# matthewhoung/inference-arena

Measured on AMD Instinct MI355X. Metric: req/sec (whole node) + P50/P99 e2e latency, YOLOv5n→MobileNetV2 at 1/2/4/8 GPU, higher is better.
Workload: dtype fp32

## Files before the change

csrc/bindings.cpp:

```cpp
#include <pybind11/numpy.h>
#include <pybind11/pybind11.h>
#include <pybind11/stl.h>

#include <cstring>
#include <malloc.h>
#include <map>
#include <mutex>

#include "kernels/launch.h"
#include "runtime/executor.h"
#include "runtime/echo_instance.h"
#include "runtime/http_front.h"
#include "runtime/http_loadgen.h"
#include "runtime/ipc_buffer.h"
#include "runtime/peer.h"
#include "runtime/jpeg_decode.h"
#include "runtime/jpeg_ingest.h"
#include "runtime/batcher.h"
#include "runtime/split.h"
#include "runtime/crash_trace.h"

namespace py = pybind11;
using namespace arena;

namespace arena {
void bind_jpeg(py::module& m);
}

namespace {

template <typename T>
T get(const py::dict& d, const char* k, T dflt) {
  if (!d.contains(k)) return dflt;
  py::object o = d[k];
  if (o.is_none()) return dflt;
  return o.cast<T>();
}
template <typename T>
T req(const py::dict& d, const char* k) {
  if (!d.contains(k)) throw std::runtime_error(std::string("missing kernel parameter '") + k + "'");
  return d[k].cast<T>();
}
template <typename P>
P ptr(const py::dict& d, const char* k) {
  return reinterpret_cast<P>(get<uintptr_t>(d, k, 0));
}
hipStream_t stream_of(const py::dict& d) { return reinterpret_cast<hipStream_t>(get<uintptr_t>(d, "stream", 0)); }

void py_conv2d(const py::dict& d) {
  ConvParams p{};
  p.x = ptr<const void*>(d, "x");
  p.B = req<int>(d, "B");
  p.H = req<int>(d, "H");
  p.W = req<int>(d, "W");
  p.xs = req<int>(d, "xs");
  p.Cin = req<int>(d, "Cin");
  p.w = ptr<const void*>(d, "w");
  p.Kpad = req<int>(d, "Kpad");
  p.bias = ptr<const float*>(d, "bias");
  p.y = ptr<void*>(d, "y");
  p.Ho = req<int>(d, "Ho");
  p.Wo = req<int>(d, "Wo");
  p.ys = req<int>(d, "ys");
  p.Cout = req<int>(d, "Cout");
  p.Cout_pad = req<int>(d, "Cout_pad");
  p.KH = req<int>(d, "KH");
  p.KW = req<int>(d, "KW");
  p.stride = get<int>(d, "stride", 1);
  p.pad_t = get<int>(d, "pad_t", 0);
  p.pad_l = get<int>(d, "pad_l", 0);
  p.res = ptr<const void*>(d, "res");
  p.rs = get<int>(d, "rs", 0);
  p.y2 = ptr<void*>(d, "y2");
  p.y2s = get<int>(d, "y2s", 0);
  p.act = get<int>(d, "act", 0);
  p.f32out = get<int>(d, "f32out", 0);
  p.bdev = ptr<const int*>(d, "bdev");
  p.impl = get<int>(d, "impl", 0);
  p.pw_w = ptr<const void*>(d, "pw_w");
  p.pw_bias = ptr<const float*>(d, "pw_bias");
  p.pw_y = ptr<void*>(d, "pw_y");
  p.pw_ys = get<int>(d, "pw_ys", 0);
  p.pw_cout = get<int>(d, "pw_cout", 0);
  p.pw_kpad = get<int>(d, "pw_kpad", 0);
  p.pw_act = get<int>(d, "pw_act", 0);
  p.gate = ptr<const float*>(d, "gate");
  p.gate_n = get<int>(d, "gate_n", 0);
  p.gate_min = get<float>(d, "gate_min", 0.f);
  p.w3 = ptr<const void*>(d, "w3");
  p.sk_ws = ptr<float*>(d, "sk_ws");
  p.sk_ws_bytes = get<int64_t>(d, "sk_ws_bytes", 0);
  prepare_kernels();
  if (get<int>(d, "f32", 0))
    conv2d_f32(p, stream_of(d));
  else
    conv2d(p, stream_of(d));
}

void py_dwconv(const py::dict& d) {
  DwParams p{};
  p.x = ptr<const void*>(d, "x");
  p.B = req<int>(d, "B");
  p.H = req<int>(d, "H");
  p.W = req<int>(d, "W");
  p.xs = req<int>(d, "xs");
  p.C = req<int>(d, "C");
  p.w = ptr<const void*>(d, "w");
  p.bias = ptr<const float*>(d, "bias");
  p.y = ptr<void*>(d, "y");
  p.Ho = req<int>(d, "Ho");
  p.Wo = req<int>(d, "Wo");
  p.ys = req<int>(d, "ys");
  p.stride = get<int>(d, "stride", 1);
  p.act = get<int>(d, "act", 0);
  p.bdev = ptr<const int*>(d, "bdev");
  if (get<int>(d, "f32", 0))
    dwconv3x3_f32(p, stream_of(d));
  else
    dwconv3x3(p, stream_of(d));
}

void py_ir_block(const py::dict& d) {
  IrParams p{};
  p.x = ptr<const void*>(d, "x");
  p.x_cs = req<int>(d, "x_cs");
  p.H = req<int>(d, "H");
  p.W = req<int>(d, "W");
  p.inp = req<int>(d, "inp");
  p.inp_pad = req<int>(d, "inp_pad");
  p.hid_pad = req<int>(d, "hid_pad");
  p.oup = req<int>(d, "oup");
  p.oup_pad = req<int>(d, "oup_pad");
  p.stride = req<int>(d, "stride");
  p.expand = req<int>(d, "expand");
  p.res = get<int>(d, "res", 0);
  p.we = ptr<const void*>(d, "we");
  p.be = ptr<const float*>(d, "be");
  p.wd = ptr<const void*>(d, "wd");
  p.bd = ptr<const float*>(d, "bd");
  p.wp = ptr<const void*>(d, "wp");
  p.bp = ptr<const float*>(d, "bp");
  p.y = ptr<void*>(d, "y");
  p.y_cs = req<int>(d, "y_cs");
  p.Ho = req<int>(d, "Ho");
  p.Wo = req<int>(d, "Wo");
  p.B = req<int>(d, "B");
  p.bdev = ptr<const int*>(d, "bdev");
  p.x3w = get<int>(d, "x3w", 0);
  p.x_parts = get<int>(d, "x_parts", 0);
  p.y_parts = get<int>(d, "y_parts", 0);
  prepare_kernels();
  if (get<int>(d, "f32", 0))
    ir_block_f32(p, stream_of(d));
  else
    ir_block(p, stream_of(d));
}

void py_c3_block(const py::dict& d) {
  C3Params p{};
  p.x = ptr<const void*>(d, "x");
  p.xs = req<int>(d, "xs");
  p.B = req<int>(d, "B");
  p.H = req<int>(d, "H");
  p.W = req<int>(d, "W");
  p.bdev = ptr<const int*>(d, "bdev");
  p.C1 = req<int>(d, "C1");
  p.CH = req<int>(d, "CH");
  p.NB = req<int>(d, "NB");
  p.res = req<int>(d, "res");
  p.w12 = ptr<const void*>(d, "w12");
  p.b12 = ptr<const float*>(d, "b12");
  p.wb1[0] = p.wb1[1] = ptr<const void*>(d, "wb1");
  p.bb1[0] = p.bb1[1] = ptr<const float*>(d, "bb1");
  p.wb2[0] = p.wb2[1] = ptr<const void*>(d, "wb2");
  p.bb2[0] = p.bb2[1] = ptr<const float*>(d, "bb2");
  p.w3 = ptr<const void*>(d, "w3");
  p.b3 = ptr<const float*>(d, "b3");
  p.y = ptr<void*>(d, "y");
  p.ys = req<int>(d, "ys");
  prepare_kernels();
  if (get<int>(d, "f32", 0))
    c3_x3(p, stream_of(d));
  else
    c3_fused(p, stream_of(d));
}

void py_sppf(const py::dict& d) {
  SppfParams p{};
  p.buf = ptr<void*>(d, "buf");
  p.B = req<int>(d, "B");
  p.H = req<int>(d, "H");
  p.W = req<int>(d, "W");
  p.xs = req<int>(d, "xs");
  p.C = req<int>(d, "C");
  p.bdev = ptr<const int*>(d, "bdev");
  if (get<int>(d, "f32", 0))
    sppf_pool_f32(p, stream_of(d));
  else
    sppf_pool(p, stream_of(d));
}

void py_letterbox(const py::dict& d) {
  LetterboxParams p{};
  p.pool = ptr<const uint8_t*>(d, "pool");
  p.meta = ptr<const ImageMeta*>(d, "meta");
  p.ctrl = ptr<const Ctrl*>(d, "ctrl");
  p.out = ptr<void*>(d, "out");
  p.B = req<int>(d, "B");
  p.T = req<int>(d, "T");
  p.f32 = get<int>(d, "f32", 0);
  letterbox_s2d(p, stream_of(d));
}

void py_decode(const py::dict& d) {
  DecodeParams p{};
  auto heads = req<std::vector<uintptr_t>>(d, "head");
  auto hw = req<std::vector<int>>(d, "hw");
  auto xs = req<std::vector<int>>(d, "xs");
  auto st = req<std::vector<float>>(d, "strides");
  for (int l = 0; l < 3; ++l) {
    p.head[l] = (const void*)heads.at(l);
    p.hw[l] = hw.at(l);
    p.xs[l] = xs.at(l);
    p.stride[l] = st.at(l);
  }
  p.B = req<int>(d, "B");
  p.conf_thr = req<float>(d, "conf_thr");
  p.cand = ptr<Candidate*>(d, "cand");
  p.cand_count = ptr<int*>(d, "cand_count");
  p.cand_cap = req<int>(d, "cand_cap");
  p.ctrl = ptr<const Ctrl*>(d, "ctrl");
  p.f32 = get<int>(d, "f32", 0);
  detect_decode(p, stream_of(d));
}

void py_yolo_raw(const py::dict& d) {
  YoloRawParams p{};
  auto heads = req<std::vector<uintptr_t>>(d, "head");
  auto hw = req<std::vector<int>>(d, "hw");
  auto xs = req<std::vector<int>>(d, "xs");
  auto st = req<std::vector<float>>(d, "strides");
  for (int l = 0; l < 3; ++l) {
    p.head[l] = (const void*)heads.at(l);
    p.hw[l] = hw.at(l);
    p.xs[l] = xs.at(l);
    p.stride[l] = st.at(l);
  }
  p.B = req<int>(d, "B");
  p.out = ptr<void*>(d, "out");
// ... 216 lines not shown
      p = std::malloc(bytes);
      if (p == nullptr) throw std::bad_alloc();
    }
    it->coef = (int16_t*)p;
    st = compact ? jpeg_decode_compact((const uint8_t*)data.data(), data.size(), it->info, (uint8_t*)it->coef, err)
                 : jpeg_decode_coefs((const uint8_t*)data.data(), data.size(), it->info, it->coef, err);
    if (st != JpegStatus::Ok) throw py::value_error("JpegSet: entropy decode failed: " + err);
    set->items.push_back(it);
  }
  return set;
}

std::vector<InputImage> images_from(const py::list& imgs, std::vector<py::array>& keep, JpegKeep* jkeep = nullptr) {
  std::vector<InputImage> v;
  v.reserve(imgs.size());
  for (auto h : imgs) {
    if (py::isinstance<py::bytes>(h)) {
      if (jkeep == nullptr) throw std::runtime_error("JPEG inputs are not accepted here");
      const std::string data = h.cast<std::string>();
      auto jh = std::make_shared<JpegHolder>();
      std::string err;
      JpegStatus st = jpeg_parse((const uint8_t*)data.data(), data.size(), jh->info, err);
      if (st == JpegStatus::Ok) {
        jh->coef.assign((size_t)jh->info.coef_count, 0);
        st = jpeg_decode_coefs((const uint8_t*)data.data(), data.size(), jh->info, jh->coef.data(), err);
      }
      if (st != JpegStatus::Ok) throw py::value_error("JPEG input not decodable by the split decoder: " + err);
      InputImage im{(const uint8_t*)jh->coef.data(), jh->info.out_height, jh->info.out_width};
      im.jpeg = &jh->info;
      jkeep->push_back(jh);
      v.push_back(im);
      continue;
    }
    py::array a = py::array::ensure(h, py::array::c_style);
    if (!a) throw std::runtime_error("inputs must be numpy arrays");
    InputImage im;
    if (a.ndim() == 3 && a.shape(2) == 3 && a.itemsize() == 1) {
      im.h = (int)a.shape(0);
      im.w = (int)a.shape(1);
    } else if (a.ndim() == 3 && a.shape(0) == 3 && a.itemsize() == 4 && a.shape(1) == a.shape(2)) {
      im.h = im.w = (int)a.shape(1);
      im.bytes = (int64_t)a.nbytes();
    } else {
      throw std::runtime_error("inputs must be uint8 HxWx3 images or float32 [3,S,S] tensors");
    }
    keep.push_back(a);
    im.data = (const uint8_t*)a.data();
    v.push_back(im);
  }
  return v;
}

py::dict result_to_py(const BatchResult& r, int max_det) {
  py::dict out;
  const int n = r.n_images;
  py::array_t<int32_t> cnt(n);
  std::memcpy(cnt.mutable_data(), r.det_count.data(), sizeof(int) * n);
  py::array_t<float> det({n, max_det, 8});
  static_assert(sizeof(Detection) == 32, "Detection layout");
  if (n) std::memcpy(det.mutable_data(), r.det.data(), sizeof(Detection) * (size_t)n * max_det);
  py::array_t<int32_t> offs(n + 1);
  std::memcpy(offs.mutable_data(), r.crop_offset.data(), sizeof(int) * (n + 1));
  static_assert(sizeof(TopkResult) == 64, "TopkResult layout");
  py::array_t<int32_t> tk_idx({(int)r.topk.size(), 5});
  py::array_t<float> tk_logit({(int)r.topk.size(), 5});
  py::array_t<float> tk_prob({(int)r.topk.size(), 5});
  for (size_t i = 0; i < r.topk.size(); ++i)
    for (int k = 0; k < 5; ++k) {
      tk_idx.mutable_at(i, k) = r.topk[i].idx[k];
      tk_logit.mutable_at(i, k) = r.topk[i].logit[k];
      tk_prob.mutable_at(i, k) = r.topk[i].prob[k];
    }
  out["det_count"] = cnt;
  out["det"] = det;
  out["crop_offset"] = offs;
  out["topk_idx"] = tk_idx;
  out["topk_logit"] = tk_logit;
  out["topk_prob"] = tk_prob;
  out["gpu_ms"] = r.gpu_ms;
  out["detection_ms"] = r.det_ms;
  out["classification_ms"] = r.cls_ms;
  out["bucket"] = r.bucket;
  out["total_crops"] = r.total_crops;
  if (!r.raw.empty()) {
    py::array_t<uint8_t> raw((py::ssize_t)r.raw.size());
    std::memcpy(raw.mutable_data(), r.raw.data(), r.raw.size());
    out["raw"] = raw;
  }
  return out;
}

}

PYBIND11_MODULE(_C, m) {
  m.doc() = "MI355X-native kernels and runtime of inference_arena_amd (gfx950)";
  {
    const char* e = std::getenv("ARENA_CRASH_TRACE");
    if (e == nullptr || std::strcmp(e, "0") != 0) arena::install_crash_trace();
  }
  m.def("install_crash_trace", &arena::install_crash_trace);
  m.def("crash_trace_installed", &arena::crash_trace_installed);
  m.def("dump_thread_stack", &arena::dump_thread_stack, py::arg("tid"));
  m.def("malloc_trim", []() {
    py::gil_scoped_release nogil;
    return malloc_trim(0) != 0;
  });
  m.def("malloc_info", []() {
    const struct mallinfo2 mi = mallinfo2();
    py::dict d;
    d["arena"] = (uint64_t)mi.arena;
    d["mmapped"] = (uint64_t)mi.hblkhd;
    d["in_use"] = (uint64_t)mi.uordblks;
    d["free"] = (uint64_t)mi.fordblks;
    d["releasable"] = (uint64_t)mi.keepcost;
    return d;
  });
  bind_jpeg(m);
  m.def("conv2d", &py_conv2d);
  m.def("set_conv_impl", &set_conv_impl);
  m.def("get_conv_impl", &get_conv_impl);
  m.def("dwconv3x3", &py_dwconv);
  m.def("sppf_pool", &py_sppf);
  m.def("ir_block", &py_ir_block);
  m.def("c3_block", &py_c3_block);
  m.def("set_conv_pw", &set_conv_pw);
  m.def("set_conv_v3", &set_conv_v3);
  m.def("set_ir_wave", &set_ir_wave);
  m.def("set_irx_parts", &set_irx_parts);
  m.def("set_irx_slices_big", &set_irx_slices_big);
  m.def("set_ir_t14", &set_ir_t14);
  m.def("set_ir_crop", &set_ir_crop);
  m.def("set_ir_s2k16", &set_ir_s2k16);
  m.def("set_ir_crop_split", &set_ir_crop_split);
  m.def("set_head_gate", &set_head_gate);
  m.def("get_head_gate", &get_head_gate);
  m.def(
      "head_gate_min",
      [](float conf_thr) -> py::object {
        float g;
        if (!head_gate_min(conf_thr, &g)) return py::none();
        return py::float_(g);
      },
      py::arg("conf_thr"), "the gate's logit threshold for a confidence threshold (float32); None: the gate is off");
  m.def(
      "head_gate_pairs",
      [](py::array_t<int64_t, py::array::c_style> ops) {
        if (ops.ndim() != 2 || ops.shape(1) != kOpFields) throw std::runtime_error("ops must be int64 [n, OP_FIELDS]");
        py::list out;
        for (const HeadGatePair& gp : head_gate_pairs(ops.data(), (int)ops.shape(0), kOpFields))
          out.append(py::make_tuple(gp.box, gp.cls, gp.level));
        return out;
      },
      py::arg("ops"), "[(box conv op, class conv op, level)] of a program's records");
  m.attr("HEAD_BOX_CHANNELS") = kHeadBoxChannels;
  m.attr("HEAD_CLS_CHANNELS") = kHeadClsChannels;
  m.def("letterbox_s2d", &py_letterbox);
  m.def("detect_decode", &py_decode);
  m.def("yolo_raw", &py_yolo_raw);
  m.def("tensor_in_s2d", &py_tensor_in);
  m.def("nms", &py_nms);
  m.def("crop_plan", &py_crop_plan);
  m.def("crop_gather_s2d", &py_crop_gather);
  m.def("global_avgpool", &py_avgpool);
  m.def("head_pool", &py_head_pool);
  m.def("topk_softmax", &py_topk);
  m.attr("SIZEOF_IMAGE_META") = (int)sizeof(ImageMeta);
  m.attr("SIZEOF_CTRL") = (int)sizeof(Ctrl);
  m.attr("SIZEOF_CANDIDATE") = (int)sizeof(Candidate);
  m.attr("SIZEOF_DETECTION") = (int)sizeof(Detection);
  m.attr("SIZEOF_CROPREF") = (int)sizeof(CropRef);
  m.attr("SIZEOF_TOPK") = (int)sizeof(TopkResult);
  m.attr("OP_FIELDS") = kOpFields;

  py::class_<Executor, std::shared_ptr<Executor>>(m, "Executor")
      .def(py::init([](const py::dict& cfg) { return std::make_shared<Executor>(config_from(cfg)); }))
      .def("set_weights",
           [](Executor& e, py::array_t<uint8_t, py::array::c_style> blob) { e.set_weights(blob.data(), blob.size()); })
      .def("set_weights_device",
           [](Executor& e, uintptr_t ptr, size_t bytes) {
             py::gil_scoped_release nogil;
             e.set_weights_device((const void*)ptr, bytes);
           })
      .def("weights_host",
           [](Executor& e) {
             std::vector<uint8_t> v;
             {
               py::gil_scoped_release nogil;
               v = e.weights_host();
             }
             return py::bytes((const char*)v.data(), v.size());
           })
      .def("set_program",
           [](Executor& e, py::array_t<int64_t, py::array::c_style> ops, py::array_t<int64_t, py::array::c_style> cls) {
             if (ops.ndim() != 2 || ops.shape(1) != kOpFields || cls.ndim() != 2 || cls.shape(1) != kOpFields)
               throw std::runtime_error("programs must be int64 [n, OP_FIELDS]");
             e.set_program(ops.data(), (int)ops.shape(0), cls.data(), (int)cls.shape(0));
           })
      .def("add_bucket",
           [](Executor& e, int B, py::array_t<int64_t, py::array::c_style> offs, int64_t arena_bytes,
              py::object impl) {
             if (impl.is_none()) {
               e.add_bucket(B, offs.data(), (int)offs.size(), arena_bytes);
             } else {
               const std::vector<int> v = impl.cast<std::vector<int>>();
               e.add_bucket(B, offs.data(), (int)offs.size(), arena_bytes, &v);
             }
           },
           py::arg("B"), py::arg("offsets"), py::arg("arena_bytes"), py::arg("impl") = py::none())
      .def("buckets", &Executor::buckets)
      .def("crop_cap_for", &Executor::crop_cap_for)
      .def("submit",
           [](Executor& e, const py::list& imgs) {
             std::vector<py::array> keep;
             JpegKeep jkeep;
             auto v = images_from(imgs, keep, &jkeep);
             int slot;
             {
               py::gil_scoped_release nogil;
               slot = e.submit(v);
             }
             if (!jkeep.empty()) {
               std::lock_guard<std::mutex> lk(g_jkeep_mu);
               g_jkeep[{(const void*)&e, slot}] = std::move(jkeep);
             }
             return slot;
           })
      .def("submit_jpeg_set",
           [](Executor& e, std::shared_ptr<JpegSet> set, const std::vector<int>& idx) {
             std::vector<InputImage> v;
             v.reserve(idx.size());
             for (int i : idx) {
               if (i < 0 || i >= (int)set->items.size()) throw py::index_error("submit_jpeg_set: index out of range");
               const auto& it = set->items[i];
               InputImage im{(const uint8_t*)it->coef, it->info.out_height, it->info.out_width};
               im.jpeg = &it->info;
               v.push_back(im);
             }
             int slot;
             {
               py::gil_scoped_release nogil;
               slot = e.submit(v);
             }
             std::lock_guard<std::mutex> lk(g_jkeep_mu);
             g_jset_keep[{(const void*)&e, slot}] = set;
             return slot;
           })
      .def("collect",
           [](Executor& e, int slot) {
             BatchResult r;
             {
               py::gil_scoped_release nogil;
               r = e.collect(slot);
             }
             {
               std::lock_guard<std::mutex> lk(g_jkeep_mu);
               g_jkeep.erase({(const void*)&e, slot});
               g_jset_keep.erase({(const void*)&e, slot});
             }
             return result_to_py(r, e.config().max_det);
           })
      .def("run",
           [](Executor& e, const py::list& imgs) {
             std::vector<py::array> keep;
             JpegKeep jkeep;
             auto v = images_from(imgs, keep, &jkeep);
             BatchResult r;
             {
               py::gil_scoped_release nogil;
               r = e.run(v);
             }
             return result_to_py(r, e.config().max_det);
           })
      .def("replay",
           [](Executor& e, int B, int slot, int iters) {
             py::gil_scoped_release nogil;
             e.replay(B, slot, iters);
           })
      .def("num_slots", &Executor::num_slots)
      .def("synchronize",
           [](Executor& e) {
             py::gil_scoped_release nogil;
             e.synchronize();
           })
      .def("arena_ptr", &Executor::arena_ptr)
      .def("read_arena",
           [](Executor& e, int B, int64_t offset, size_t bytes) {
             py::array_t<uint8_t> out(bytes);
             {
               py::gil_scoped_release nogil;
               e.read_arena(B, offset, out.mutable_data(), bytes);
             }
             return out;
           })
      .def("weights_ptr", &Executor::weights_ptr)
      .def("set_peer_stage", &Executor::set_peer_stage)
      .def("device", &Executor::device)
      .def("submit_peer",
           [](Executor& e, Executor& src, int slot) {
             py::gil_scoped_release nogil;
             return e.submit_peer(src, slot);
           })
      .def("submit_device",
           [](Executor& e, const std::vector<std::tuple<uintptr_t, int, int, int>>& images,
              const std::vector<py::array_t<float, py::array::c_style | py::array::forcecast>>& boxes) {
             if (images.size() != boxes.size()) throw std::runtime_error("submit_device: one box array per image");
             std::vector<Executor::DeviceImage> imgs;
             std::vector<std::vector<Detection>> dets(images.size());
             for (size_t i = 0; i < images.size(); ++i) {
               Executor::DeviceImage d;
               d.ptr = std::get<0>(images[i]);
               d.h = std::get<1>(images[i]);
               d.w = std::get<2>(images[i]);
               d.device = std::get<3>(images[i]);
               imgs.push_back(d);
               const auto& b = boxes[i];
               if (b.size() == 0) continue;
               if (b.ndim() != 2 || b.shape(1) != 6) throw std::runtime_error("submit_device: boxes must be [k, 6]");
               const float* q = b.data();
               for (ssize_t k = 0; k < b.shape(0); ++k, q += 6) {
                 Detection dd{};
                 dd.x1 = q[0];
                 dd.y1 = q[1];
                 dd.x2 = q[2];
                 dd.y2 = q[3];
                 dd.conf = q[4];
                 dd.cls = (int)q[5];
                 dets[i].push_back(dd);
               }
             }
             py::gil_scoped_release nogil;
             return e.submit_device(imgs, dets);
           })
      .def("conv_choices", &Executor::conv_choices)
      .def("exec_order", &Executor::exec_order, py::arg("B"),
           "program op indices in the order bucket B's graphs launch them")
      .def("gated_ops", &Executor::gated_ops, py::arg("B"), "ops of bucket B that run with a tile gate")
      .def("stream", &Executor::stream);

  py::class_<SplitInstance, std::shared_ptr<SplitInstance>>(m, "SplitInstance")
      .def(py::init([](std::shared_ptr<Executor> det, std::shared_ptr<Executor> cls) {
        return std::make_shared<SplitInstance>(det, cls);
      }))
      .def("submit",
           [](SplitInstance& s, const py::list& imgs) {
             std::vector<py::array> keep;
             auto v = images_from(imgs, keep);
             py::gil_scoped_release nogil;
             return s.submit(v);
           })
      .def("collect",
           [](SplitInstance& s, int slot) {
             BatchResult r;
             {
               py::gil_scoped_release nogil;
               r = s.collect(slot);
             }
             return result_to_py(r, s.max_det());
           })
      .def("num_slots", &SplitInstance::num_slots)
      .def("buckets", &SplitInstance::buckets);

  py::class_<JpegSet, std::shared_ptr<JpegSet>>(m, "JpegSet")
      .def(py::init(&make_jpeg_set), py::arg("uploads"), py::arg("pinned") = true,
           "JPEG uploads entropy-decoded once into (pinned) host buffers, for Executor.submit_jpeg_set")
      .def("__len__", [](const JpegSet& s) { return s.items.size(); })
      .def("coef_bytes", [](const JpegSet& s, int i) { return (int64_t)jpeg_payload_bytes(s.items.at(i)->info); })
      .def_property_readonly("pinned", [](const JpegSet& s) {
        for (const auto& it : s.items)
          if (!it->pinned) return false;
        return true;
      });

  py::class_<EchoInstance, std::shared_ptr<EchoInstance>>(m, "EchoInstance")
      .def(py::init<int, int, int, int, int64_t>(), py::arg("slots") = 2, py::arg("max_batch") = 32,
           py::arg("max_det") = 4, py::arg("latency_us") = 0, py::arg("staging_cap") = 0);

  py::class_<DynamicBatcher>(m, "DynamicBatcher")
      .def(py::init([](py::list executors, const py::dict& cfg) {
             std::vector<std::shared_ptr<BatchInstance>> inst;
             for (auto h : executors) {
               if (py::isinstance<SplitInstance>(h))
                 inst.push_back(h.cast<std::shared_ptr<SplitInstance>>());
               else if (py::isinstance<EchoInstance>(h))
                 inst.push_back(h.cast<std::shared_ptr<EchoInstance>>());
               else
                 inst.push_back(h.cast<std::shared_ptr<Executor>>());
             }
             BatcherConfig c;
             c.max_batch = get<int>(cfg, "max_batch", c.max_batch);
             c.preferred = get<std::vector<int>>(cfg, "preferred", {});
             c.max_queue_delay_us = get<int64_t>(cfg, "max_queue_delay_us", c.max_queue_delay_us);
             c.idle_queue_delay_us = get<int64_t>(cfg, "idle_queue_delay_us", c.idle_queue_delay_us);
             c.max_queue_size = get<int64_t>(cfg, "max_queue_size", c.max_queue_size);
             c.overlap = get<int>(cfg, "overlap", c.overlap);
             return new DynamicBatcher(inst, c);
           }),
           py::keep_alive<1, 2>())
      .def("enqueue",
           [](DynamicBatcher& b, py::array img_in, py::function cb, uintptr_t export_to) {
             py::array img = py::array::ensure(img_in, py::array::c_style);
             int h = 0, w = 0;
             int64_t bytes = 0;
             if (img && img.ndim() == 3 && img.shape(2) == 3 && img.itemsize() == 1) {
               h = (int)img.shape(0);
               w = (int)img.shape(1);
             } else if (img && img.ndim() == 3 && img.shape(0) == 3 && img.itemsize() == 4 &&
                        img.shape(1) == img.shape(2)) {
               h = w = (int)img.shape(1);
               bytes = (int64_t)img.nbytes();
             } else {
               throw std::runtime_error("input must be a uint8 HxWx3 image or a float32 [3,S,S] tensor");
             }
             ResultCallback f = py_result_cb(std::move(cb));
             const uint8_t* data = (const uint8_t*)img.data();
             py::gil_scoped_release nogil;
             return b.enqueue(data, h, w, std::move(f), bytes, (uint8_t*)export_to);
           },
           py::arg("img"), py::arg("cb"), py::arg("export_to") = 0)
      .def("stats",
           [](DynamicBatcher& b) {
             BatcherStats s = b.stats();
             py::dict d;
             d["requests"] = s.requests;
             d["batches"] = s.batches;
             d["rejected"] = s.rejected;
             d["failed"] = s.failed;
             d["queue_depth"] = s.queue_depth;
             d["mean_batch"] = s.batches ? s.sum_batch / s.batches : 0.0;
             d["mean_queue_us"] = s.requests ? s.sum_queue_us / s.requests : 0.0;
             d["mean_compute_us"] = s.batches ? s.sum_compute_us / s.batches : 0.0;
             d["batch_hist"] = s.batch_hist;
             d["device_faults"] = s.device_faults;
             d["last_error"] = s.last_error;
             return d;
           })
      .def("shutdown", [](DynamicBatcher& b) {
        py::gil_scoped_release nogil;
        b.shutdown();
      });

  py::class_<JpegIngest>(m, "JpegIngest")
      .def(py::init([](DynamicBatcher& batcher, const py::dict& cfg) {
             IngestConfig c;
             c.threads = get<int>(cfg, "threads", c.threads);
             c.jpeg_device = get<bool>(cfg, "jpeg_device", c.jpeg_device);
             c.max_image_pixels = get<int64_t>(cfg, "max_image_pixels", c.max_image_pixels);
             c.buffer_cap = get<int64_t>(cfg, "buffer_cap", c.buffer_cap);
             int ndev = 0;
             const bool gpu = hipGetDeviceCount(&ndev) == hipSuccess && ndev > 0;
             (void)hipGetLastError();
             if (get<bool>(cfg, "pinned", gpu)) {
               c.host_alloc = [](size_t n) -> void* {
                 void* p = nullptr;
                 if (hipHostMalloc(&p, n, hipHostMallocPortable) != hipSuccess) {
                   (void)hipGetLastError();
                   return nullptr;
                 }
                 return p;
               };
               c.host_free = [](void* p) { (void)hipHostFree(p); };
             }
             py::gil_scoped_release nogil;
             return new JpegIngest(&batcher, c);
           }),
           py::keep_alive<1, 2>())
      .def(
          "submit",
          [](JpegIngest& g, py::bytes upload, py::function done, py::function fallback, uintptr_t export_to) {
            std::string u = upload;
            std::shared_ptr<py::function> fb(new py::function(std::move(fallback)), [](py::function* fn) {
              py::gil_scoped_acquire gil;
              delete fn;
            });
            ResultCallback cb = py_result_cb(std::move(done));
            py::gil_scoped_release nogil;
            g.submit(std::move(u), std::move(cb), [fb](std::string&&) {
              py::gil_scoped_acquire gil;
              try {
                (*fb)();
              } catch (py::error_already_set& e) {
                e.discard_as_unraisable("JpegIngest fallback");
              }
            }, (uint8_t*)export_to);
          },
          py::arg("upload"), py::arg("done"), py::arg("fallback"), py::arg("export_to") = 0,
          "Split-decode `upload` into the batcher: done(result dict) after its batch; fallback() (no arguments) "
          "when the split decoder does not cover the format (the caller decodes and enqueues it itself).")
      .def("stats",
           [](JpegIngest& g) {
// ... 323 lines not shown
```

csrc/kernels/conv_f32.hip:

```cpp
#include <algorithm>
#include <cstdlib>
#include <stdexcept>
#include <string>

#include "common.h"
#include "launch.h"
#include "letterbox.h"

namespace arena {

__device__ __forceinline__ float4 load_f4_or_zero(const float* p, const float* safe, bool ok) {
  const float4 v = *(const float4*)(ok ? p : safe);
  return ok ? v : make_float4(0.f, 0.f, 0.f, 0.f);
}

__device__ __forceinline__ float f4_get(const float4& v, int s) {
  return s == 0 ? v.x : s == 1 ? v.y : s == 2 ? v.z : v.w;
}

__device__ __forceinline__ int xcd_remap(int bx, int nx) {
  const int q = nx / 8, r = nx % 8, x = bx % 8, y = bx / 8;
  return (x < r ? x * (q + 1) : r * (q + 1) + (x - r) * q) + y;
}

// ... 1236 lines not shown
  const int HWo = p.Ho * p.Wo;
  const int M = live_batch(p.B, p.bdev) * HWo;
  const int tiles = (M + 15) / 16;
  int t = blockIdx.x * 4 + wave;
  if (blockIdx.x * 4 >= tiles) return;

  const float* __restrict__ w = (const float*)p.w;
  for (int i = tid; i < BN * K / 4; i += STR_THREADS) {
    const int row = i / (K / 4), k = 4 * (i - row * (K / 4));
    const bool ok = n0 + row < p.Cout_pad && k < p.Kpad;
    *(float4*)&sW[row * WPF + k] = load_f4_or_zero(w + (size_t)(n0 + row) * p.Kpad + k, w, ok);
  }
  float4 bias[NF];
#pragma unroll
  for (int j = 0; j < NF; ++j) {
    const int cb = n0 + j * 16 + 4 * kq;
    bias[j] = cb < p.Cout ? *(const float4*)(p.bias + cb) : make_float4(0.f, 0.f, 0.f, 0.f);
  }
  __syncthreads();

  const float* __restrict__ x = (const float*)p.x;
  const int tstride = gridDim.x * 4;
  int tdy[KC], tdx[KC], tci[KC];
#pragma unroll
  for (int c = 0; c < KC; ++c) {
    const int k0 = c * 16 + kq * 4, tap = k0 / p.Cin;
    const int kh = tap / p.KW;
    tci[c] = k0 - tap * p.Cin;
    tdy[c] = (tap < p.KH * p.KW && k0 < p.Kpad) ? kh - p.pad_t : -(1 << 20);
    tdx[c] = tap - kh * p.KW - p.pad_l;
  }
  float4 bnext[KC];
  auto load_b = [&](int tt) {
    const int pix = tt * 16 + col;
    const int b = pix / HWo, r = pix - b * HWo;
    const int oy = r / p.Wo, ox = r - (r / p.Wo) * p.Wo;
    const float* xb = x + (size_t)b * p.H * p.W * p.xs;
#pragma unroll
    for (int c = 0; c < KC; ++c) {
      const int iy = oy * p.stride + tdy[c], ix = ox * p.stride + tdx[c];
      const bool ok = pix < M && (unsigned)iy < (unsigned)p.H && (unsigned)ix < (unsigned)p.W;
      bnext[c] = load_f4_or_zero(xb + ((size_t)iy * p.W + ix) * p.xs + tci[c], x, ok);
    }
  };
  if (t < tiles) load_b(t);
  for (; t < tiles; t += tstride) {
    float4 bc[KC];
#pragma unroll
    for (int c = 0; c < KC; ++c) bc[c] = bnext[c];
    if (t + tstride < tiles) load_b(t + tstride);
    f32x4 acc[NF];
#pragma unroll
    for (int j = 0; j < NF; ++j) acc[j] = f32x4{0.f, 0.f, 0.f, 0.f};
#pragma unroll
    for (int c = 0; c < KC; ++c) {
#pragma unroll
      for (int j = 0; j < NF; ++j) {
        const float4 a = *(const float4*)&sW[(j * 16 + col) * WPF + c * 16 + kq * 4];
#pragma unroll
        for (int s4 = 0; s4 < 4; ++s4)
          acc[j] = __builtin_amdgcn_mfma_f32_16x16x4f32(f4_get(a, s4), f4_get(bc[c], s4), acc[j], 0, 0, 0);
      }
    }
    const int pix = t * 16 + col;
    if (pix >= M) continue;
#pragma unroll
    for (int j = 0; j < NF; ++j) {
      const int cb = n0 + j * 16 + kq * 4;
      if (cb >= p.Cout) continue;
      float v[4] = {acc[j][0] + bias[j].x, acc[j][1] + bias[j].y, acc[j][2] + bias[j].z, acc[j][3] + bias[j].w};
#pragma unroll
      for (int r = 0; r < 4; ++r) v[r] = apply_act(v[r], p.act);
      if (p.res != nullptr) {
        const float4 rv = *(const float4*)((const float*)p.res + (size_t)pix * p.rs + cb);
        v[0] += rv.x; v[1] += rv.y; v[2] += rv.z; v[3] += rv.w;
      }
      const float4 o = make_float4(v[0], v[1], v[2], v[3]);
      *(float4*)((float*)p.y + (size_t)pix * p.ys + cb) = o;
      if (p.y2 != nullptr) {
        const int b = pix / HWo;
        const int r = pix - b * HWo;
        const int oy = r / p.Wo, ox = r - (r / p.Wo) * p.Wo;
        const int W2 = 2 * p.Wo;
        float* y2 = (float*)p.y2;
        const size_t base = ((size_t)(b * 2 * p.Ho + 2 * oy) * W2 + 2 * ox);
        *(float4*)(y2 + base * p.y2s + cb) = o;
        *(float4*)(y2 + (base + 1) * p.y2s + cb) = o;
        *(float4*)(y2 + (base + W2) * p.y2s + cb) = o;
        *(float4*)(y2 + (base + W2 + 1) * p.y2s + cb) = o;
      }
    }
  }
}

template <int NF, int KC>
static void launch_stream_exact(const ConvParams& p, hipStream_t s) {
  constexpr int BN = NF * 16;
  const int ny = (p.Cout_pad + BN - 1) / BN;
  const long tiles = ((long)p.B * p.Ho * p.Wo + 15) / 16;
  const long gx = std::max(1L, std::min((tiles + 3) / 4, (long)std::max(1, 1024 / ny)));
  hipLaunchKernelGGL((conv_f32_stream_kernel<NF, KC>), dim3((unsigned)gx, (unsigned)ny), dim3(STR_THREADS), 0, s, p);
}

template <int NF>
static bool launch_stream_exact_k(const ConvParams& p, hipStream_t s) {
  const int kc = p.Kpad / 16;
  if (kc <= 1) launch_stream_exact<NF, 1>(p, s);
  else if (kc <= 2) launch_stream_exact<NF, 2>(p, s);
  else if (kc <= 4) launch_stream_exact<NF, 4>(p, s);
  else if (kc <= 6) launch_stream_exact<NF, 6>(p, s);
  else if (kc <= 8) launch_stream_exact<NF, 8>(p, s);
  else if (kc <= 10) launch_stream_exact<NF, 10>(p, s);
  else if (kc <= 12) launch_stream_exact<NF, 12>(p, s);
  else return false;
  return true;
}

static bool f32_stream(const ConvParams& p, hipStream_t s) {
  if (p.Cin % 4 != 0 || p.Kpad > 192 || p.Kpad % 16 != 0 || p.Kpad < p.KH * p.KW * p.Cin || p.xs % 4 != 0)
    return false;
  const int ncf = p.Cout_pad / 16;
  const int nf = ncf <= 5 ? ncf : ncf % 4 == 0 ? 4 : ncf % 3 == 0 ? 3 : ncf % 5 == 0 ? 5 : ncf % 2 == 0 ? 2 : 1;
  switch (nf) {
    case 1: return launch_stream_exact_k<1>(p, s);
    case 2: return launch_stream_exact_k<2>(p, s);
    case 3: return launch_stream_exact_k<3>(p, s);
    case 4: return launch_stream_exact_k<4>(p, s);
    case 5: return launch_stream_exact_k<5>(p, s);
    default: return false;
  }
}

static bool x3_stream(const ConvParams& p, hipStream_t s, int nf_force) {
  if (p.Cin % 8 != 0 || p.Kpad > 192 || p.Kpad < p.KH * p.KW * p.Cin || p.xs % 4 != 0) return false;
  const int ncf = p.Cout_pad / 16;
  const int nf = nf_force ? nf_force
                          : ncf <= 5 ? ncf : ncf % 4 == 0 ? 4 : ncf % 3 == 0 ? 3 : ncf % 5 == 0 ? 5 : ncf % 2 == 0 ? 2 : 1;
  switch (nf) {
    case 1: return launch_stream_k<1>(p, s);
    case 2: return launch_stream_k<2>(p, s);
    case 3: return launch_stream_k<3>(p, s);
    case 4: return launch_stream_k<4>(p, s);
    case 5: return launch_stream_k<5>(p, s);
    default: return false;
  }
}

void conv2d_f32(const ConvParams& p, hipStream_t s) {
  if (p.Cin % 4 != 0 || p.xs % 4 != 0 || p.Kpad % 16 != 0 || p.Cout_pad % 16 != 0 || p.Cout % 4 != 0 ||
      p.Cout > p.Cout_pad || p.ys % 4 != 0)
    throw std::runtime_error("conv2d_f32: unsupported geometry (Cin/xs/ys %4, Kpad %16, Cout_pad %16, Cout %4)");
  if (p.Cin < 16) throw std::runtime_error("conv2d_f32: Cin must be >= 16");
  if (p.Kpad < p.KH * p.KW * p.Cin) throw std::runtime_error("conv2d_f32: Kpad < KH*KW*Cin");
  if (p.pw_w != nullptr) {
    if (p.impl >= kF32X3HRPw && p.impl < kF32X3HRPw + kF32X3HRPwVariants) {
      if (!conv_x3hr_pw(p, s, p.impl - kF32X3HRPw))
        throw std::runtime_error("conv2d_f32: a fused pointwise epilogue needs an x3hr-pw variant that fits the conv");
      return;
    }
    const int v = p.impl >= kF32X3HGPw && p.impl < kF32X3HGPw + kF32X3HGPwVariants ? p.impl - kF32X3HGPw
                  : p.impl >= kF32X3HGPwSmall && p.impl < kF32X3HGPwSmall + kF32X3HGPwSmallVariants
                      ? kF32X3HGPwVariants + p.impl - kF32X3HGPwSmall
                  : p.impl == 0 ? (p.Cout_pad <= 64 ? 0 : 2)
                                : -1;
    if (v < 0 || !conv_x3hg_pw(p, s, v))
      throw std::runtime_error("conv2d_f32: a fused pointwise epilogue needs an x3hg-pw variant that fits the conv");
    return;
  }
  if (p.res != nullptr && p.rs % 4 != 0) throw std::runtime_error("conv2d_f32: residual stride % 4");
  if (p.y2 != nullptr && p.y2s % 4 != 0) throw std::runtime_error("conv2d_f32: upsampled stride % 4");
  const long M = (long)p.B * p.Ho * p.Wo;
  if (M <= 0) return;
  if (M > 0x7fffffffL || (long)p.B * p.H * p.W * p.xs > 0x7fffffffL) throw std::runtime_error("conv2d_f32: too large");
  const int ncf = p.Cout_pad / 16;
  if (p.lb_meta != nullptr) {
    if (p.lb_pool == nullptr || !x3_h16(p, s))
      throw std::runtime_error("conv2d_f32: a letterbox-source conv must be a 3x3 s1 pad-1 conv over 16 channels");
    return;
  }
  if (p.impl >= 10) {
    if (p.impl >= kF32X3G && p.impl < kF32X3G + kF32X3GVariants) {
      if (!conv_x3g(p, s, p.impl - kF32X3G))
        throw std::runtime_error("conv2d_f32: not an x3g-eligible conv (needs pre-split weights)");
      return;
    }
    if (p.impl >= kF32X3GSK && p.impl < kF32X3GSK + kF32X3GSKVariants) {
      if (!conv_x3g_sk(p, s, p.impl - kF32X3GSK))
        throw std::runtime_error("conv2d_f32: not a split-K x3g-eligible conv (pre-split weights, workspace)");
      return;
    }
    if (p.impl >= kF32X3HG && p.impl < kF32X3HG + kF32X3HGVariants) {
      if (!conv_x3hg(p, s, p.impl - kF32X3HG))
        throw std::runtime_error("conv2d_f32: not an x3hg-eligible conv (3x3 s1 with pre-split weights)");
      return;
    }
    if (p.impl >= kF32X3HR && p.impl < kF32X3HR + kF32X3HRVariants) {
      if (!conv_x3hr(p, s, p.impl - kF32X3HR))
        throw std::runtime_error("conv2d_f32: not an x3hr-eligible conv (3x3 s1 with pre-split weights)");
      return;
    }
    if (p.impl >= kF32X3HP && p.impl < kF32X3HP + kF32X3HPVariants) {
      if (!conv_x3hp(p, s, p.impl - kF32X3HP))
        throw std::runtime_error("conv2d_f32: not an x3hp-eligible conv (3x3 s1 with pre-split weights)");
      return;
    }
    if (p.impl == kF32X3H16) {
      if (!x3_h16(p, s)) throw std::runtime_error("conv2d_f32: not an x3-h16-eligible conv (3x3 s1 over 16 channels)");
      return;
    }
    if (p.impl == kF32Fc) {
      if (!conv_fc_f32(p, s)) throw std::runtime_error("conv2d_f32: not an FC-eligible conv (1x1 map, Kpad 1280)");
      return;
    }
    if (p.impl == kF32StreamExact) {
      if (!f32_stream(p, s)) throw std::runtime_error("conv2d_f32: not a stream-eligible conv (Cin % 4, Kpad <= 192)");
      return;
    }
    if (p.impl == kF32Stream || p.impl == kF32StreamN2) {
      if (!x3_stream(p, s, p.impl == kF32StreamN2 ? 2 : 0))
        throw std::runtime_error("conv2d_f32: not a stream-eligible conv (Cin % 8, Kpad <= 192)");
      return;
    }
    if (p.impl == kF32X3Halo || p.impl == kF32X3HaloN3 || p.impl == kF32X3HaloN2 || p.impl == kF32X3Halo16 ||
        p.impl == kF32X3Halo16N3) {
      const int nf = (p.impl == kF32X3HaloN3 || p.impl == kF32X3Halo16N3) ? 3 : p.impl == kF32X3HaloN2 ? 2 : 0;
      const int th = (p.impl == kF32X3Halo16 || p.impl == kF32X3Halo16N3) ? 16 : 8;
      if (!x3_halo(p, s, nf, th)) throw std::runtime_error("conv2d_f32: not an x3-halo-eligible conv");
      return;
    }
    if (p.impl == kF32Halo) {
      if (!halo_f32(p, s, true)) throw std::runtime_error("conv2d_f32: not a halo-eligible conv");
      return;
    }
    if (p.impl >= kF32X3) {
      if (p.impl >= kF32X3 + kF32X3Variants || !launch_x3_variant(p, s, M, p.impl - kF32X3))
        throw std::runtime_error("conv2d_f32: unknown x3 variant");
      return;
    }
    if (p.impl >= 10 + kF32Variants || !launch_lds_variant(p, s, M, p.impl - 10)) throw std::runtime_error("conv2d_f32: unknown variant");
    return;
  }
  if (p.impl == 0 && conv_fc_f32(p, s)) return;
  const int impl = p.impl == 1 ? 1 : p.impl >= 2 ? 2 : f32_conv_family();
  if (impl == 2 && halo_f32(p, s)) return;
  if (impl == 2) {
    if (ncf == 1)
      launch_lds_m<1, 4, 1>(p, s, M);
    else if (ncf == 2)
      launch_lds_m<2, 4, 1>(p, s, M);
    else if (ncf == 3 || ncf == 9)
      launch_lds_m<3, 4, 1>(p, s, M);
    else if (ncf == 5)
      launch_lds_m<5, 4, 1>(p, s, M);
    else if (ncf == 6)
      launch_lds_m<3, 2, 2>(p, s, M);
    else
      launch_lds_m<2, 2, 2>(p, s, M);
    return;
  }
  if (ncf % 4 == 0 || ncf > 12)
    launch_f32_wc<4>(p, s, M);
  else if (ncf % 3 == 0)
    launch_f32_wc<3>(p, s, M);
  else if (ncf % 2 == 0)
    launch_f32_wc<2>(p, s, M);
  else if (ncf == 5)
    launch_f32_wc<5>(p, s, M);
  else
    launch_f32_wc<1>(p, s, M);
}

template <int R, int S, int CX>
__global__ __launch_bounds__(256) void dwconv_f32_kernel(const DwParams p) {
  const int B = live_batch(p.B, p.bdev);
  const int cg = p.C >> 2;
  const int strips = (p.Ho + R - 1) / R;
  const int colb = (p.Wo + CX - 1) / CX;
  const int total = B * strips * colb * cg;
  const int tid = blockIdx.x * blockDim.x + threadIdx.x;
  if (tid >= total) return;
  const int g = tid % cg;
  int t = tid / cg;
  const int ox0 = (t % colb) * CX;
  t /= colb;
  const int st = t % strips;
  const int b = t / strips;
  const int c0 = g * 4;
  const int oy0 = st * R;
  const float* x = (const float*)p.x + (size_t)b * p.H * p.W * p.xs + c0;
  const float* w = (const float*)p.w + c0;
  float4 wt[9];
#pragma unroll
  for (int k = 0; k < 9; ++k) wt[k] = *(const float4*)(w + k * p.C);
  const float4 bias = *(const float4*)(p.bias + c0);
  float4 acc[R][CX];
#pragma unroll
  for (int r = 0; r < R; ++r)
#pragma unroll
    for (int c = 0; c < CX; ++c) acc[r][c] = bias;
  constexpr int NIN = (R - 1) * S + 3, NCOL = (CX - 1) * S + 3;
  const int iy0 = oy0 * S - 1, ix0 = ox0 * S - 1;
#pragma unroll
  for (int ri = 0; ri < NIN; ++ri) {
    const int iy = iy0 + ri;
    if ((unsigned)iy >= (unsigned)p.H) continue;
    const float* row = x + (size_t)iy * p.W * p.xs;
    float4 v[NCOL];
#pragma unroll
    for (int q = 0; q < NCOL; ++q)
      v[q] = load_f4_or_zero(row + (ix0 + q) * p.xs, x, (unsigned)(ix0 + q) < (unsigned)p.W);
#pragma unroll
    for (int r = 0; r < R; ++r) {
      const int ky = ri - r * S;
      if (ky < 0 || ky > 2) continue;
#pragma unroll
      for (int c = 0; c < CX; ++c)
#pragma unroll
// ... 120 lines not shown
```

csrc/kernels/halo_x3g.hip:

```cpp
#include <stdexcept>
#include <string>

#include "common.h"
#include "launch.h"

namespace arena {

namespace {

typedef float f32x16 __attribute__((ext_vector_type(16)));
typedef unsigned u32x4 __attribute__((ext_vector_type(4)));

constexpr int HG_P = 56;
constexpr int HG_GATE_MAX_N = 80;

__host__ __device__ constexpr int hg_th(int TW, int WM, int TM) { return WM * TM * (32 / TW); }
__host__ __device__ constexpr int hg_lds_bytes(int TW, int WM, int WN, int TM, int TN) {
  return ((hg_th(TW, WM, TM) + 2) * (TW + 2) + 2 * WN * TN * 32) * HG_P * 2;
}
__host__ __device__ constexpr int hr_lds_bytes(int TW, int WM, int TM) {
  return (hg_th(TW, WM, TM) + 2) * (TW + 2) * HG_P * 2;
}

__device__ __forceinline__ int hg_xcd_remap(int bx, int nx) {
// ... 404 lines not shown
#pragma unroll
      for (int pl = 0; pl < 3; ++pl) w[tn][pl] = __builtin_amdgcn_raw_buffer_load_b128(wr, w_off[tn], step + 64 * pl, 0);
  };

  f32x16 acc[TM][TN];
#pragma unroll
  for (int a = 0; a < TM; ++a)
#pragma unroll
    for (int c = 0; c < TN; ++c)
#pragma unroll
      for (int r = 0; r < 16; ++r) acc[a][c][r] = 0.f;

  int xpix[TM];
#pragma unroll
  for (int tm = 0; tm < TM; ++tm) {
    const int r = (wm * TM + tm) * RF + fr / TW, c = fr % TW;
    xpix[tm] = r * HC + c;
  }
  auto compute = [&](const u32x4 (&w)[TN][3], int tap) {
    const int ky = tap / 3, kx = tap - ky * 3;
    const int toff = ky * HC + kx;
    bf16x8 xh[TM], xm[TM], xl[TM];
#pragma unroll
    for (int tm = 0; tm < TM; ++tm) {
      const bf16* r = sX + (xpix[tm] + toff) * HG_P + fk;
      xh[tm] = *(const bf16x8*)r;
      xm[tm] = *(const bf16x8*)(r + 16);
      xl[tm] = *(const bf16x8*)(r + 32);
    }
#pragma unroll
    for (int tn = 0; tn < TN; ++tn) {
      const bf16x8 wh = __builtin_bit_cast(bf16x8, w[tn][0]), wmid = __builtin_bit_cast(bf16x8, w[tn][1]),
                   wl = __builtin_bit_cast(bf16x8, w[tn][2]);
#pragma unroll
      for (int tm = 0; tm < TM; ++tm) acc[tm][tn] = hg_mfma_x3(wh, wmid, wl, xh[tm], xm[tm], xl[tm], acc[tm][tn]);
    }
  };

  const int nc = (Cin + 15) >> 4;
  u32x4 wa[TN][3], wb[TN][3];
#pragma unroll
  for (int piece = 0; piece < 8; ++piece) load_x_piece(0, piece);
  load_w(0, wa);
  store_x();
  __syncthreads();
  auto chunk = [&](int cc, u32x4 (&w0)[TN][3], u32x4 (&w1)[TN][3]) {
    const bool more = cc + 1 < nc;
#pragma unroll
    for (int tap = 0; tap < 9; ++tap) {
      const int st = cc * 9 + tap;
      if (tap % 2 == 0) load_w(st + 1, w1);
      else load_w(st + 1, w0);
      if (more && tap < 8) load_x_piece(cc + 1, tap);
      if (tap % 2 == 0) compute(w0, tap);
      else compute(w1, tap);
    }
    if (more) {
      __syncthreads();
      store_x();
      __syncthreads();
    }
  };
  for (int cc = 0; cc < nc; ++cc) {
    if ((cc & 1) == 0) chunk(cc, wa, wb);
    else chunk(cc, wb, wa);
  }

  hg_epilogue<TW, WM, WN, TM, TN, PWN>(p, acc, b, oy0, ox0, n0, wm, wn, lane);
}

namespace {

template <int TW, int WM, int WN, int TM, int TN, int PWN = 0>
void hg_launch(const ConvParams& p, hipStream_t s) {
  constexpr int TH = hg_th(TW, WM, TM), BN = WN * TN * 32;
  const long tiles = (long)p.B * ((p.Ho + TH - 1) / TH) * ((p.Wo + TW - 1) / TW) * ((p.Cout_pad + BN - 1) / BN);
  hipLaunchKernelGGL((conv_x3hg_kernel<TW, WM, WN, TM, TN, PWN>), dim3((unsigned)tiles), dim3(WM * WN * 64),
                     hg_lds_bytes(TW, WM, WN, TM, TN), s, p);
}

template <int TW, int WM, int WN, int TM, int TN, int PWN = 0>
void hr_launch(const ConvParams& p, hipStream_t s) {
  constexpr int TH = hg_th(TW, WM, TM), BN = WN * TN * 32;
  const long tiles = (long)p.B * ((p.Ho + TH - 1) / TH) * ((p.Wo + TW - 1) / TW) * ((p.Cout_pad + BN - 1) / BN);
  hipLaunchKernelGGL((conv_x3hr_kernel<TW, WM, WN, TM, TN, PWN>), dim3((unsigned)tiles), dim3(WM * WN * 64),
                     hr_lds_bytes(TW, WM, TM), s, p);
}

#define HG_VARIANTS(X) \
  X(0, 16, 4, 1, 2, 2)   \
  X(1, 16, 4, 1, 1, 2)   \
  X(2, 16, 2, 2, 2, 1)   \
  X(3, 16, 4, 1, 2, 3)   \
  X(4, 16, 4, 1, 1, 3)   \
  X(5, 16, 4, 1, 2, 5)   \
  X(6, 16, 4, 1, 1, 5)   \
  X(7, 8, 2, 2, 1, 1)    \
  X(8, 8, 4, 1, 1, 2)    \
  X(9, 8, 4, 1, 1, 5)    \
  X(10, 8, 4, 1, 1, 3)   \
  X(11, 16, 8, 1, 1, 5)  \
  X(12, 8, 2, 2, 1, 2)   \
  X(13, 8, 2, 1, 1, 5)

#define HG_PW_VARIANTS(X) \
  X(0, 16, 4, 1, 2, 2)   \
  X(1, 16, 4, 2, 2, 2)   \
  X(2, 16, 4, 1, 3, 3)   \
  X(3, 16, 4, 2, 3, 3)   \
  X(4, 8, 4, 1, 2, 2)    \
  X(5, 8, 4, 1, 3, 3)    \
  X(6, 8, 2, 1, 2, 2)    \
  X(7, 8, 2, 1, 3, 3)

#define HR_VARIANTS(X) \
  X(0, 16, 4, 1, 2, 2)   \
  X(1, 16, 4, 1, 1, 2)   \
  X(2, 16, 4, 1, 2, 3)   \
  X(3, 16, 4, 1, 1, 3)   \
  X(4, 16, 4, 1, 1, 5)   \
  X(5, 16, 8, 1, 1, 5)   \
  X(6, 8, 4, 1, 1, 2)    \
  X(7, 8, 4, 1, 1, 5)    \
  X(8, 16, 2, 2, 2, 1)   \
  X(9, 8, 4, 1, 1, 3)

#define HR_PW_VARIANTS(X) \
  X(0, 16, 4, 1, 2, 2)  \
  X(1, 16, 4, 2, 2, 2)  \
  X(2, 16, 4, 1, 3, 3)  \
  X(3, 16, 4, 2, 3, 3)  \
  X(4, 8, 4, 1, 2, 2)   \
  X(5, 8, 4, 1, 3, 3)

}

bool x3hg_supported(const ConvParams& p) {
  const size_t x_bytes = (size_t)p.B * p.H * p.W * p.xs * 4;
  const size_t w_bytes = (size_t)9 * ((p.Cin + 31) / 32) * p.Cout_pad * 192;
  return p.w3 != nullptr && p.KH == 3 && p.KW == 3 && p.stride == 1 && p.Cin % 4 == 0 && p.xs % 4 == 0 &&
         x_bytes < (1u << 31) - (1u << 20) && w_bytes < (1u << 31) - (1u << 20) && p.Cout % 4 == 0 &&
         p.ys % 4 == 0 && (p.res == nullptr || p.rs % 4 == 0) && (p.y2 == nullptr || p.y2s % 4 == 0) &&
         p.lb_meta == nullptr && p.pw_w == nullptr;
}

bool x3hg_pw_supported(const ConvParams& p, int bn, int pwn) {
  return p.w3 != nullptr && p.KH == 3 && p.KW == 3 && p.stride == 1 && p.Cin % 4 == 0 && p.xs % 4 == 0 &&
         (size_t)p.B * p.H * p.W * p.xs * 4 < (1u << 31) - (1u << 20) && p.Cout % 4 == 0 && p.Cout_pad <= bn &&
         p.res == nullptr && p.y2 == nullptr && p.lb_meta == nullptr && p.pw_w != nullptr && p.pw_y != nullptr &&
         p.pw_kpad == bn && p.pw_cout % 4 == 0 && p.pw_cout <= 32 * pwn && p.pw_ys % 4 == 0 &&
         (p.gate == nullptr ||
          (p.gate_n > 0 && p.gate_n <= HG_GATE_MAX_N && p.gate_n % 4 == 0 && p.gate_n <= p.pw_ys &&
           (uintptr_t)p.gate % 16 == 0));
}

bool conv_x3hg_pw(const ConvParams& p, hipStream_t s, int v) {
  switch (v) {
#define HG_PW_CASE(V, TW, WM, TM, TN, PWN) \
  case V:                                 \
    if (!x3hg_pw_supported(p, TN * 32, PWN)) return false; \
    hg_launch<TW, WM, 1, TM, TN, PWN>(p, s);                \
    return true;
    HG_PW_VARIANTS(HG_PW_CASE)
#undef HG_PW_CASE
    default: return false;
  }
}

bool conv_x3hg(const ConvParams& p, hipStream_t s, int v) {
  if (!x3hg_supported(p)) return false;
  switch (v) {
#define HG_CASE(V, TW, WM, WN, TM, TN) \
  case V: hg_launch<TW, WM, WN, TM, TN>(p, s); return true;
    HG_VARIANTS(HG_CASE)
#undef HG_CASE
    default: return false;
  }
}

bool conv_x3hr(const ConvParams& p, hipStream_t s, int v) {
  if (!x3hg_supported(p)) return false;
  switch (v) {
#define HR_CASE(V, TW, WM, WN, TM, TN) \
  case V: hr_launch<TW, WM, WN, TM, TN>(p, s); return true;
    HR_VARIANTS(HR_CASE)
#undef HR_CASE
    default: return false;
  }
}

bool conv_x3hr_pw(const ConvParams& p, hipStream_t s, int v) {
  switch (v) {
#define HR_PW_CASE(V, TW, WM, TM, TN, PWN) \
  case V:                                 \
    if (!x3hg_pw_supported(p, TN * 32, PWN)) return false; \
    hr_launch<TW, WM, 1, TM, TN, PWN>(p, s);                \
    return true;
    HR_PW_VARIANTS(HR_PW_CASE)
#undef HR_PW_CASE
    default: return false;
  }
}

void x3hg_prepare() {
#define HG_ATTR(V, TW, WM, WN, TM, TN)                                                            \
  ARENA_HIP_CHECK(hipFuncSetAttribute((const void*)conv_x3hg_kernel<TW, WM, WN, TM, TN>,           \
                                      hipFuncAttributeMaxDynamicSharedMemorySize,                  \
                                      hg_lds_bytes(TW, WM, WN, TM, TN)));
  HG_VARIANTS(HG_ATTR)
#undef HG_ATTR
#define HG_PW_ATTR(V, TW, WM, TM, TN, PWN)                                                         \
  ARENA_HIP_CHECK(hipFuncSetAttribute((const void*)conv_x3hg_kernel<TW, WM, 1, TM, TN, PWN>,         \
                                      hipFuncAttributeMaxDynamicSharedMemorySize,                  \
                                      hg_lds_bytes(TW, WM, 1, TM, TN)));
  HG_PW_VARIANTS(HG_PW_ATTR)
#undef HG_PW_ATTR
#define HR_ATTR(V, TW, WM, WN, TM, TN)                                                            \
  ARENA_HIP_CHECK(hipFuncSetAttribute((const void*)conv_x3hr_kernel<TW, WM, WN, TM, TN>,           \
                                      hipFuncAttributeMaxDynamicSharedMemorySize, hr_lds_bytes(TW, WM, TM)));
  HR_VARIANTS(HR_ATTR)
#undef HR_ATTR
#define HR_PW_ATTR(V, TW, WM, TM, TN, PWN)                                                         \
  ARENA_HIP_CHECK(hipFuncSetAttribute((const void*)conv_x3hr_kernel<TW, WM, 1, TM, TN, PWN>,         \
                                      hipFuncAttributeMaxDynamicSharedMemorySize, hr_lds_bytes(TW, WM, TM)));
  HR_PW_VARIANTS(HR_PW_ATTR)
#undef HR_PW_ATTR
}

}
```

csrc/kernels/halo_x3p.hip:

```cpp
#include <stdexcept>
#include <string>

#include "common.h"
#include "launch.h"

namespace arena {

namespace {

typedef unsigned u32x4 __attribute__((ext_vector_type(4)));

constexpr int HP_TW = 16, HP_HC = HP_TW + 2;
constexpr int HP_XP = 3 * 32 + 16;
__host__ __device__ constexpr int hp_wp(int TS) { return TS * 96 + 16; }
__host__ __device__ constexpr int hp_lds_bytes(int NF, int TH, int TS) {
  return ((TH + 2) * HP_HC * HP_XP + NF * 16 * hp_wp(TS)) * 2;
}

__device__ __forceinline__ int hp_xcd_remap(int bx, int nx) {
  const int q = nx / 8, r = nx % 8, x = bx % 8, y = bx / 8;
  return (x < r ? x * (q + 1) : r * (q + 1) + (x - r) * q) + y;
}

}

template <int NF, int TH, int TS>
__global__ __launch_bounds__(TH * 32) void conv_x3hp_kernel(const ConvParams p) {
  static_assert(TS == 1 || TS == 3, "a weight stage is one tap or one kernel row");
  constexpr int NT = TH * 32, NW = TH / 2;
  constexpr int HR = TH + 2, HPIX = HR * HP_HC;
  constexpr int XI = (HPIX * 8 + NT - 1) / NT;
  constexpr int BN = NF * 16, MF = 2;
  constexpr int WP = hp_wp(TS);
  constexpr int WPC = TS * BN * 12;
  constexpr int WI = (WPC + NT - 1) / NT;
  constexpr int SPC = 9 / TS;
  extern __shared__ __attribute__((aligned(16))) bf16 hp_lds[];
  bf16* sX = hp_lds;
  bf16* sW = hp_lds + HPIX * HP_XP;

  const int tid = threadIdx.x, lane = tid & 63, wave = tid >> 6;
  const int col = lane & 15, kq = lane >> 4;
  const int tiles_x = (p.Wo + HP_TW - 1) / HP_TW, tiles_y = (p.Ho + TH - 1) / TH;
  const int tiles = tiles_x * tiles_y;
  const int bx = hp_xcd_remap(blockIdx.x, gridDim.x);
  const int b = bx / tiles;
  if (b >= live_batch(p.B, p.bdev)) return;
  const int t = bx - b * tiles;
  const int ty = t / tiles_x, tx = t - ty * tiles_x;
  const int oy0 = ty * TH, ox0 = tx * HP_TW;
  const int iy0 = oy0 - p.pad_t, ix0 = ox0 - p.pad_l;
  const int n0 = blockIdx.y * BN;
  const int H = p.H, W = p.W, Cin = p.Cin;

  const __amdgpu_buffer_rsrc_t xr = __builtin_amdgcn_make_buffer_rsrc(
      const_cast<void*>(p.x), (short)0, (int)((size_t)p.B * H * W * p.xs * 4), 0x00020000);
  const int cin32 = (Cin + 31) >> 5;
  const __amdgpu_buffer_rsrc_t wr = __builtin_amdgcn_make_buffer_rsrc(
      const_cast<void*>(p.w3), (short)0, (int)((size_t)9 * cin32 * p.Cout_pad * 192), 0x00020000);
  constexpr int kOob = 0x7fffffff & ~15;

  int x_off[XI];
  const size_t img = (size_t)b * H * W;
#pragma unroll
  for (int j = 0; j < XI; ++j) {
    const int i = tid + NT * j;
    const int px = i >> 3, g = i & 7;
    const int hy = px / HP_HC, hx = px - hy * HP_HC;
    const int iy = iy0 + hy, ix = ix0 + hx;
    const bool in = i < HPIX * 8 && (unsigned)iy < (unsigned)H && (unsigned)ix < (unsigned)W;
    x_off[j] = in ? (int)(((img + (size_t)iy * W + ix) * p.xs + 4 * g) * 4) : kOob;
  }
  int w_off[WI], w_dst[WI];
  const int tap_bytes = cin32 * p.Cout_pad * 192;
#pragma unroll
  for (int j = 0; j < WI; ++j) {
    const int i = tid + NT * j;
    const int kxl = i / (BN * 12), r = i - kxl * (BN * 12);
    const int row = r / 12, piece = r - row * 12;
    const int n = n0 + row;
    w_off[j] = (i < WPC && n < p.Cout_pad) ? kxl * tap_bytes + n * 192 + piece * 16 : kOob;
    w_dst[j] = row * WP + kxl * 96 + piece * 8;
  }

  f32x4 rx[XI];
  u32x4 rw[WI];
  auto load_x = [&](int c0) {
#pragma unroll
    for (int j = 0; j < XI; ++j) {
      const int c = c0 + 4 * ((tid + NT * j) & 7);
      const int o = (x_off[j] != kOob && c < Cin) ? x_off[j] + 4 * c0 : kOob;
      rx[j] = __builtin_bit_cast(f32x4, __builtin_amdgcn_raw_buffer_load_b128(xr, o, 0, 0));
    }
  };
  auto store_x = [&]() {
#pragma unroll
    for (int j = 0; j < XI; ++j) {
      const int i = tid + NT * j;
      if (HPIX * 8 % NT == 0 || i < HPIX * 8) {
        bf16x2 h0, m0, l0, h1, m1, l1;
        split_bf16x3_pair(f32x2{rx[j][0], rx[j][1]}, h0, m0, l0);
        split_bf16x3_pair(f32x2{rx[j][2], rx[j][3]}, h1, m1, l1);
        bf16* d = sX + (i >> 3) * HP_XP + 4 * (i & 7);
        *(bf16x4*)d = __builtin_shufflevector(h0, h1, 0, 1, 2, 3);
        *(bf16x4*)(d + 32) = __builtin_shufflevector(m0, m1, 0, 1, 2, 3);
        *(bf16x4*)(d + 64) = __builtin_shufflevector(l0, l1, 0, 1, 2, 3);
      }
    }
  };
  auto load_w = [&](int st) {
    const int chunk = st / SPC, s = st - chunk * SPC;
    const int step = (s * TS * cin32 + chunk) * p.Cout_pad * 192;
#pragma unroll
    for (int j = 0; j < WI; ++j) rw[j] = __builtin_amdgcn_raw_buffer_load_b128(wr, w_off[j], step, 0);
  };
  auto store_w = [&]() {
#pragma unroll
    for (int j = 0; j < WI; ++j)
      if (WPC % NT == 0 || tid + NT * j < WPC) *(u32x4*)(sW + w_dst[j]) = rw[j];
  };

  f32x4 acc[MF][NF];
#pragma unroll
  for (int f = 0; f < MF; ++f)
#pragma unroll
    for (int j = 0; j < NF; ++j) acc[f][j] = f32x4{0.f, 0.f, 0.f, 0.f};

  const int nstage = cin32 * SPC;
  load_x(0);
  load_w(0);
  for (int st = 0; st < nstage; ++st) {
    const int chunk = st / SPC, s = st - chunk * SPC;
    if (s == 0) store_x();
    store_w();
    __syncthreads();
    if (st + 1 < nstage) {
      if (s == SPC - 1) load_x((chunk + 1) * 32);
      load_w(st + 1);
    }
    const int ky = TS == 3 ? s : s / 3;
#pragma unroll
    for (int kxl = 0; kxl < TS; ++kxl) {
      const int kx = TS == 3 ? kxl : s - ky * 3;
      bf16x8 bh[MF], bm[MF], bl[MF];
#pragma unroll
      for (int f = 0; f < MF; ++f) {
        const int oy = wave + NW * f;
        const bf16* r = &sX[((oy + ky) * HP_HC + col + kx) * HP_XP + 8 * kq];
        bh[f] = *(const bf16x8*)r;
        bm[f] = *(const bf16x8*)(r + 32);
        bl[f] = *(const bf16x8*)(r + 64);
      }
#pragma unroll
      for (int j = 0; j < NF; ++j) {
        const bf16* r = &sW[(j * 16 + col) * WP + kxl * 96 + 8 * kq];
        const bf16x8 ah = *(const bf16x8*)r;
        const bf16x8 am = *(const bf16x8*)(r + 32);
        const bf16x8 al = *(const bf16x8*)(r + 64);
#pragma unroll
        for (int f = 0; f < MF; ++f) {
          f32x4 c = acc[f][j];
          c = __builtin_amdgcn_mfma_f32_16x16x32_bf16(am, bm[f], c, 0, 0, 0);
          c = __builtin_amdgcn_mfma_f32_16x16x32_bf16(al, bh[f], c, 0, 0, 0);
          c = __builtin_amdgcn_mfma_f32_16x16x32_bf16(ah, bl[f], c, 0, 0, 0);
          c = __builtin_amdgcn_mfma_f32_16x16x32_bf16(am, bh[f], c, 0, 0, 0);
          c = __builtin_amdgcn_mfma_f32_16x16x32_bf16(ah, bm[f], c, 0, 0, 0);
          acc[f][j] = __builtin_amdgcn_mfma_f32_16x16x32_bf16(ah, bh[f], c, 0, 0, 0);
        }
      }
    }
    __syncthreads();
  }

  const int HWo = p.Ho * p.Wo;
#pragma unroll
  for (int j = 0; j < NF; ++j) {
    const int cb = n0 + j * 16 + kq * 4;
    if (cb >= p.Cout) continue;
    const float4 bias = *(const float4*)(p.bias + cb);
#pragma unroll
    for (int f = 0; f < MF; ++f) {
      const int oy = oy0 + wave + NW * f, ox = ox0 + col;
      if (oy >= p.Ho || ox >= p.Wo) continue;
      const size_t pix = (size_t)b * HWo + (size_t)oy * p.Wo + ox;
      float v[4] = {acc[f][j][0] + bias.x, acc[f][j][1] + bias.y, acc[f][j][2] + bias.z, acc[f][j][3] + bias.w};
#pragma unroll
      for (int r = 0; r < 4; ++r) v[r] = apply_act(v[r], p.act);
      if (p.res != nullptr) {
        const float4 rv = *(const float4*)((const float*)p.res + pix * p.rs + cb);
        v[0] += rv.x; v[1] += rv.y; v[2] += rv.z; v[3] += rv.w;
      }
      const float4 o = make_float4(v[0], v[1], v[2], v[3]);
      *(float4*)((float*)p.y + pix * p.ys + cb) = o;
      if (p.y2 != nullptr) {
        const int W2 = 2 * p.Wo;
        float* y2 = (float*)p.y2;
        const size_t base = ((size_t)(b * 2 * p.Ho + 2 * oy) * W2 + 2 * ox);
        *(float4*)(y2 + base * p.y2s + cb) = o;
        *(float4*)(y2 + (base + 1) * p.y2s + cb) = o;
        *(float4*)(y2 + (base + W2) * p.y2s + cb) = o;
        *(float4*)(y2 + (base + W2 + 1) * p.y2s + cb) = o;
      }
    }
  }
}

namespace {

template <int NF, int TH, int TS>
void hp_launch(const ConvParams& p, hipStream_t s) {
  constexpr int BN = NF * 16;
  const int tiles = ((p.Wo + HP_TW - 1) / HP_TW) * ((p.Ho + TH - 1) / TH);
  dim3 grid((unsigned)(p.B * tiles), (unsigned)((p.Cout_pad + BN - 1) / BN));
  hipLaunchKernelGGL((conv_x3hp_kernel<NF, TH, TS>), grid, dim3(TH * 32), hp_lds_bytes(NF, TH, TS), s, p);
}

#define HP_VARIANTS(X) \
  X(0, 2, 8, 3)    \
  X(1, 3, 8, 3)    \
  X(2, 4, 8, 3)    \
  X(3, 5, 8, 3)    \
  X(4, 2, 16, 3)   \
  X(5, 3, 16, 3)   \
  X(6, 4, 16, 3)   \
  X(7, 9, 8, 1)    \
  X(8, 9, 16, 1)

}

bool x3hp_supported(const ConvParams& p) {
  const size_t x_bytes = (size_t)p.B * p.H * p.W * p.xs * 4;
  const size_t w_bytes = (size_t)9 * ((p.Cin + 31) / 32) * p.Cout_pad * 192;
  return p.w3 != nullptr && p.KH == 3 && p.KW == 3 && p.stride == 1 && p.Cin % 4 == 0 && p.xs % 4 == 0 &&
         x_bytes < (1u << 31) - (1u << 20) && w_bytes < (1u << 31) - (1u << 20) && p.Cout % 4 == 0 &&
         p.Cout_pad % 16 == 0 && p.ys % 4 == 0 && (p.res == nullptr || p.rs % 4 == 0) &&
         (p.y2 == nullptr || p.y2s % 4 == 0) && p.lb_meta == nullptr && p.pw_w == nullptr;
}

bool conv_x3hp(const ConvParams& p, hipStream_t s, int v) {
  if (!x3hp_supported(p)) return false;
  switch (v) {
#define HP_CASE(V, NF, TH, TS) \
  case V: hp_launch<NF, TH, TS>(p, s); return true;
    HP_VARIANTS(HP_CASE)
#undef HP_CASE
    default: return false;
  }
}

void x3hp_prepare() {
#define HP_ATTR(V, NF, TH, TS)                                                                      \
  ARENA_HIP_CHECK(hipFuncSetAttribute((const void*)conv_x3hp_kernel<NF, TH, TS>,                     \
                                      hipFuncAttributeMaxDynamicSharedMemorySize, hp_lds_bytes(NF, TH, TS)));
  HP_VARIANTS(HP_ATTR)
#undef HP_ATTR
}

}
```

csrc/kernels/launch.h:

```cpp
#pragma once
#include <hip/hip_runtime.h>
#include <stdint.h>
#include <stdexcept>
#include <string>

namespace arena {

struct ImageMeta;
struct CropRef;
struct Ctrl;
struct ConvParams {
  const void* x;
  int B, H, W;
  int xs;
  int Cin;
  const void* w;
  int Kpad;
  const float* bias;
  void* y;
  int Ho, Wo, ys;
  int Cout;
  int Cout_pad;
  int KH, KW, stride, pad_t, pad_l;
  const void* res;
  int rs;
  void* y2;
  int y2s;
  int act;
  int f32out;
  const int* bdev;
  int impl;
  const void* pw_w;
  const float* pw_bias;
  void* pw_y;
  int pw_ys, pw_cout, pw_kpad, pw_act;
  const float* gate;
  int gate_n;
  float gate_min;
  const uint8_t* lb_pool;
  const ImageMeta* lb_meta;
  const void* w3;
  float* sk_ws;
  int64_t sk_ws_bytes;
  int sk_splits;
};
void conv2d(const ConvParams& p, hipStream_t s);
void conv_igemm(const ConvParams& p, hipStream_t s);
bool conv_pw(const ConvParams& p, hipStream_t s);
void set_conv_pw(bool v);
bool conv3x3_v3(const ConvParams& p, hipStream_t s);
bool conv_fc(const ConvParams& p, hipStream_t s);
void set_conv_v3(bool v);
void set_conv_impl(int v);
int get_conv_impl();

constexpr int kF32Variants = 16;
constexpr int kF32X3 = 40;
constexpr int kF32X3Variants = 12;
constexpr int kF32Halo = 100;
constexpr int kF32X3Halo = 101;
constexpr int kF32X3HaloN3 = 102;
constexpr int kF32X3HaloN2 = 103;
constexpr int kF32Stream = 104;
constexpr int kF32StreamN2 = 105;
constexpr int kF32Fc = 106;
constexpr int kF32StreamExact = 107;
constexpr int kF32X3Halo16 = 108;
constexpr int kF32X3Halo16N3 = 109;
constexpr int kF32X3H16 = 110;
constexpr int kF32X3G = 111;
constexpr int kF32X3GVariants = 20;
void x3_halo_prepare();
bool x3g_supported(const ConvParams& p);
bool conv_x3g(const ConvParams& p, hipStream_t s, int v);
constexpr int kF32X3GSK = 171;
constexpr int kF32X3GSKVariants = 9;
bool conv_x3g_sk(const ConvParams& p, hipStream_t s, int v);
void x3g_prepare();
constexpr int kF32X3HG = 131;
constexpr int kF32X3HGVariants = 14;
bool x3hg_supported(const ConvParams& p);
bool conv_x3hg(const ConvParams& p, hipStream_t s, int v);
void x3hg_prepare();
constexpr int kF32X3HGPw = 145;
constexpr int kF32X3HGPwVariants = 6;
constexpr int kF32X3HGPwSmall = 181;
constexpr int kF32X3HGPwSmallVariants = 2;
bool conv_x3hg_pw(const ConvParams& p, hipStream_t s, int v);
constexpr int kF32X3HR = 151;
constexpr int kF32X3HRVariants = 10;
constexpr int kF32X3HRPw = 161;
constexpr int kF32X3HRPwVariants = 6;
constexpr int kF32X3HP = 191;
constexpr int kF32X3HPVariants = 9;
bool x3hp_supported(const ConvParams& p);
bool conv_x3hp(const ConvParams& p, hipStream_t s, int v);
void x3hp_prepare();
bool conv_x3hr(const ConvParams& p, hipStream_t s, int v);
bool conv_x3hr_pw(const ConvParams& p, hipStream_t s, int v);
bool conv_fc_f32(const ConvParams& p, hipStream_t s);
void conv2d_f32(const ConvParams& p, hipStream_t s);

struct DwParams {
  const void* x;
  int B, H, W, xs, C;
  const void* w;
  const float* bias;
  void* y;
  int Ho, Wo, ys, stride, act;
  const int* bdev;
};
void dwconv3x3(const DwParams& p, hipStream_t s);
void dwconv3x3_f32(const DwParams& p, hipStream_t s);

struct IrParams {
  const void* x;
  int x_cs, H, W;
  int inp, inp_pad;
  int hid_pad;
  int oup, oup_pad;
  int stride, expand, res;
  const void* we;
  const float* be;
  const void* wd;
  const float* bd;
  const void* wp;
  const float* bp;
  void* y;
  int y_cs, Ho, Wo;
  int B;
  const int* bdev;
  int x3w;
  int x_parts, y_parts;
  int stem;
  const uint8_t* st_pool;
  const ImageMeta* st_meta;
  const CropRef* st_crops;
  const Ctrl* st_ctrl;
  int st_S;
  float st_mean[3], st_inv_std[3];
  const float* st_w;
  const float* st_b;
};
void ir_block(const IrParams& p, hipStream_t s);
void ir_block_f32(const IrParams& p, hipStream_t s);
bool ir_block_f32_supported(int stride, int inp_pad, int hid_pad, int oup_pad, int expand);
bool ir_block_crop_f32(const IrParams& p, hipStream_t s);
bool ir_block_crop_f32_supported(int H, int stride, int inp_pad, int hid_pad, int oup_pad, int expand);
bool ir_tile_x3(const IrParams& p, hipStream_t s);
bool ir_tile_x3_supported(int stride, int inp_pad, int hid_pad, int oup_pad, int expand);
void ir_tile_x3_prepare();
bool ir_stem_x3(const IrParams& p, hipStream_t s);
bool ir_s2k16_x3(const IrParams& p, hipStream_t s);
void set_ir_s2k16(bool v);
void ir_prepare();
void set_ir_t14(bool v);
void set_ir_crop(bool v);
void set_ir_crop_split(int v);
void set_ir_wave(bool v);
void set_irx_slices_big(int n);
void set_irx_parts(int n);

struct C3Params {
  const void* x;
  int xs;
  int B, H, W;
  const int* bdev;
  int C1, CH, NB, res;
  const void* w12;
  const float* b12;
  const void* wb1[2];
  const float* bb1[2];
  const void* wb2[2];
  const float* bb2[2];
  const void* w3;
  const float* b3;
  void* y;
  int ys;
};
bool c3_fused_supported(int C1, int CH, int NB, bool res, int H, int W);
bool c3_x3_supported(int C1, int CH, int NB, bool res, int H, int W);
void c3_x3(const C3Params& p, hipStream_t s);
void c3_x3_prepare();
void c3_fused(const C3Params& p, hipStream_t s);

struct SppfParams {
  void* buf;
  int B, H, W, xs, C;
  const int* bdev;
};
void sppf_pool(const SppfParams& p, hipStream_t s);
void sppf_pool_f32(const SppfParams& p, hipStream_t s);

struct ImageMeta {
  int64_t offset;
  int h, w;
  int new_w, new_h;
  int pad_w, pad_h;
  float scale;
  float pad_[3];
};
static_assert(sizeof(ImageMeta) == 48, "ImageMeta layout");

struct Ctrl {
  int n_images;
  int n_crops;
  int crop_base;
  int total_crops;
  int pad_[12];
};

struct LetterboxParams {
  const uint8_t* pool;
  const ImageMeta* meta;
  const Ctrl* ctrl;
  void* out;
  int B, T;
  int f32;
};
void letterbox_s2d(const LetterboxParams& p, hipStream_t s);

struct TensorInParams {
  const uint8_t* pool;
  const ImageMeta* meta;
  const Ctrl* ctrl;
  void* out;
  int B, S;
  int f32;
};
void tensor_in_s2d(const TensorInParams& p, hipStream_t s);

struct Candidate {
  float x1, y1, x2, y2;
  float score;
  int cls;
  int anchor;
  int pad_;
};
struct DecodeParams {
  const void* head[3];
  int hw[3];
  int xs[3];
  float stride[3];
  int B;
  float conf_thr;
  Candidate* cand;
  int* cand_count;
  int cand_cap;
  const Ctrl* ctrl;
  int f32;
// ... 157 lines not shown
```

csrc/runtime/executor.cpp:

```cpp
#include "executor.h"
#include "peer.h"

#include <pthread.h>
#include <sys/prctl.h>

#include <algorithm>
#include <chrono>
#include <cmath>
#include <cstdio>
#include <cstdlib>
#include <cstring>
#include <thread>
#include <stdexcept>
#include <string>

#include "../kernels/common.h"
#include "../kernels/jpeg_desc.h"
#include "jpeg_decode.h"
#include "trace.h"

namespace arena {

namespace {
float bits_to_float(int64_t v) {
  uint32_t u = (uint32_t)v;
  float f;
  std::memcpy(&f, &u, 4);
  return f;
}
size_t align_up(size_t v, size_t a) { return (v + a - 1) / a * a; }
constexpr size_t kCtrlBytes = 256;
static_assert(kHgOpConv == OP_CONV && kHgOpDecode == OP_DECODE && kHgDtypeField == kDtypeField &&
                  sizeof(OpRecord) == sizeof(int64_t) * kOpFields,
              "head_gate.h reads the executor's op records");
bool g_head_gate = [] {
  const char* e = std::getenv("ARENA_HEAD_GATE");
  return e == nullptr || std::atoi(e) != 0;
}();
}

void set_head_gate(bool v) { g_head_gate = v; }
bool get_head_gate() { return g_head_gate; }

Executor::Executor(const ExecutorConfig& cfg) : cfg_(cfg) {
  if (cfg_.max_batch <= 0 || cfg_.max_batch > 1024) throw std::runtime_error("Executor: max_batch out of range");
  if (cfg_.cand_cap > 16384) throw std::runtime_error("Executor: cand_cap > 16384");
  ARENA_HIP_CHECK(hipSetDevice(cfg_.device));
  prepare_kernels();
  max_B_ = cfg_.max_batch;
  {
    int khz = 0;
    if (hipDeviceGetAttribute(&khz, hipDeviceAttributeWallClockRate, cfg_.device) == hipSuccess && khz > 0)
      wall_khz_ = (double)khz;
  }
  {
    const char* e = std::getenv("ARENA_DEBUG_SYNC");
    debug_sync_ = e != nullptr ? std::atoi(e) : 0;
    const char* at = std::getenv("ARENA_AUTOTUNE");
    autotune_ = at != nullptr ? std::atoi(at) : 1;
    const char* c = std::getenv("ARENA_COPY_MODE");
    copy_mode_ = c != nullptr && std::atoi(c) == 2 ? 2 : 0;
    const char* cc = std::getenv("ARENA_CONCURRENT");
    concurrent_ = cc != nullptr ? std::atoi(cc) : 1;
    if (debug_sync_) concurrent_ = 0;
    const char* ns = std::getenv("ARENA_SLOTS");
    n_slots_ = concurrent_ ? std::min(kMaxSlots, std::max(2, ns != nullptr ? std::atoi(ns) : 4)) : 2;
    const char* nc = std::getenv("ARENA_CONCURRENCY");
    n_streams_ = concurrent_ ? std::min(n_slots_, std::max(1, nc != nullptr ? std::atoi(nc) : 3)) : 1;
    const char* sg = std::getenv("ARENA_STAGGER");
    if (concurrent_ && n_streams_ > 1) {
      std::string spec = sg != nullptr ? sg : "0.25";
      for (size_t a = 0; a < spec.size();) {
        size_t e = spec.find(',', a);
        if (e == std::string::npos) e = spec.size();
        const double f = std::atof(spec.substr(a, e - a).c_str());
        if (f > 0.0 && f < 1.0 && (int)stagger_.size() < kMaxStaggerParts - 1) stagger_.push_back(f);
        a = e + 1;
      }
      std::sort(stagger_.begin(), stagger_.end());
    }
    const char* sm = std::getenv("ARENA_STAGGER_MIN_BATCH");
    stagger_min_batch_ = sm != nullptr ? std::max(1, std::atoi(sm)) : 32;
  }
  ARENA_HIP_CHECK(hipStreamCreateWithFlags(&compute_, hipStreamNonBlocking));
  ARENA_HIP_CHECK(hipStreamCreateWithFlags(&copy_, hipStreamNonBlocking));
  streams_[0] = compute_;
  for (int i = 1; i < n_streams_; ++i) ARENA_HIP_CHECK(hipStreamCreateWithFlags(&streams_[i], hipStreamNonBlocking));
  for (int s = 0; s < n_slots_; ++s) {
    slots_[s].idx = s;
    slots_[s].stream = streams_[s % n_streams_];
  }
  alloc_slots();
  const int nthreads = std::max(1, cfg_.host_threads);
  for (int t = 0; t < nthreads; ++t) {
    workers_.emplace_back([this]() {
      pthread_setname_np(pthread_self(), "arena-pack");
      uint64_t seen = 0;
      for (;;) {
        std::vector<std::function<void()>>* jobs;
        {
          std::unique_lock<std::mutex> lk(pool_mu_);
          pool_cv_.wait(lk, [&] { return pool_stop_ || pool_gen_ != seen; });
          if (pool_stop_) return;
          seen = pool_gen_;
          jobs = pool_jobs_;
          if (jobs == nullptr) continue;
          ++pool_active_;
        }
        for (;;) {
          const int i = pool_next_.fetch_add(1);
          if (i >= (int)jobs->size()) break;
          (*jobs)[i]();
        }
        std::lock_guard<std::mutex> lk(pool_mu_);
        if (--pool_active_ == 0) pool_done_cv_.notify_all();
      }
    });
  }
}

Executor::~Executor() {
  {
    std::lock_guard<std::mutex> lk(pool_mu_);
    pool_stop_ = true;
  }
  pool_cv_.notify_all();
  for (auto& t : workers_) t.join();
  hipSetDevice(cfg_.device);
  for (int i = 0; i < n_streams_; ++i)
    if (streams_[i]) hipStreamSynchronize(streams_[i]);
  if (copy_) hipStreamSynchronize(copy_);
  for (auto& kv : buckets_) {
    for (int s = 0; s < n_slots_; ++s) destroy_graphs(kv.second, s);
    free_arenas(kv.second);
  }
  for (int i = 1; i < n_streams_; ++i)
    if (streams_[i]) hipStreamDestroy(streams_[i]);
  for (int s = 0; s < n_slots_; ++s) {
    Slot& sl = slots_[s];
    if (sl.d_in) hipFree(sl.d_in);
    if (sl.d_out) hipFree(sl.d_out);
    if (sl.sk_ws) hipFree(sl.sk_ws);
    if (sl.h_in) hipHostFree(sl.h_in);
    if (sl.h_out) hipHostFree(sl.h_out);
  }
  for (uint8_t* p : retired_h_in_) hipHostFree(p);
  retired_h_in_.clear();
  for (int s = 0; s < n_slots_; ++s) {
    Slot& sl = slots_[s];
    if (sl.copied) hipEventDestroy(sl.copied);
    if (sl.started) hipEventDestroy(sl.started);
    if (sl.done) hipEventDestroy(sl.done);
    if (sl.fork_ev) hipEventDestroy(sl.fork_ev);
    for (hipEvent_t& e : sl.phase)
      if (e) hipEventDestroy(e);
    for (int l = 0; l < kMaxLanes; ++l) {
      if (sl.lane_ev[l]) hipEventDestroy(sl.lane_ev[l]);
      if (sl.lane_stream[l]) hipStreamDestroy(sl.lane_stream[l]);
    }
  }
  if (d_weights_) hipFree(d_weights_);
  if (compute_) hipStreamDestroy(compute_);
  if (copy_) hipStreamDestroy(copy_);
}

size_t Executor::jpeg_desc_off() const { return kCtrlBytes + align_up(sizeof(ImageMeta) * (size_t)max_B_, 256); }
size_t Executor::in_bytes_meta() const { return jpeg_desc_off() + align_up(sizeof(JpegDesc) * (size_t)max_B_, 256); }
size_t Executor::pool_cap() const {
  return align_up((size_t)cfg_.pool_bytes_per_image * (size_t)std::max(1, cfg_.pool_factor) * max_B_, 256);
}
size_t Executor::in_bytes_total() const { return in_bytes_meta() + pool_cap(); }
size_t Executor::out_off_det() const { return align_up(sizeof(int) * (size_t)max_B_, 256); }
size_t Executor::out_off_topk() const {
  return out_off_det() + align_up(sizeof(Detection) * (size_t)max_B_ * cfg_.max_det, 256);
}
size_t Executor::out_off_raw() const {
  return align_up(out_off_topk() + sizeof(TopkResult) * (size_t)max_B_ * cfg_.max_det, 256);
}
size_t Executor::out_off_xcrops() const { return align_up(out_off_raw() + (size_t)cfg_.raw_out_bytes * max_B_, 256); }
size_t Executor::out_off_stamps() const {
  return align_up(out_off_xcrops() + sizeof(CropRef) * (size_t)max_B_ * cfg_.max_det, 256);
}
size_t Executor::out_bytes_total() const { return out_off_stamps() + 4 * sizeof(uint64_t); }

void Executor::sync_slots() {
  for (int i = 0; i < n_streams_; ++i) ARENA_HIP_CHECK(hipStreamSynchronize(streams_[i]));
}

void Executor::free_arenas(Bucket& bk) {
  for (int s = 0; s < n_slots_; ++s) {
    if (bk.d_arena[s] == nullptr) continue;
    bool first = true;
    for (int t = 0; t < s; ++t) first &= bk.d_arena[t] != bk.d_arena[s];
    if (first) hipFree(bk.d_arena[s]);
  }
  for (int s = 0; s < kMaxSlots; ++s) bk.d_arena[s] = nullptr;
}

void Executor::alloc_slots() {
  for (int s = 0; s < n_slots_; ++s) {
    Slot& sl = slots_[s];
    ARENA_HIP_CHECK(hipMalloc(&sl.d_in, in_bytes_total() + 256));
    ARENA_HIP_CHECK(hipMalloc(&sl.d_out, out_bytes_total()));
    ARENA_HIP_CHECK(hipMalloc(&sl.sk_ws, (size_t)sk_lane_bytes() * (kMaxLanes + 1)));
    sl.h_cap = in_bytes_meta() + align_up((size_t)cfg_.pool_bytes_per_image * max_B_, 256);
    ARENA_HIP_CHECK(hipHostMalloc(&sl.h_in, sl.h_cap, hipHostMallocDefault));
    ARENA_HIP_CHECK(hipHostMalloc(&sl.h_out, out_bytes_total(), hipHostMallocDefault));
    ARENA_HIP_CHECK(hipMemset(sl.d_in, 0, in_bytes_total()));
    ARENA_HIP_CHECK(hipMemset(sl.d_out, 0, out_bytes_total()));
    std::memset(sl.h_in, 0, in_bytes_meta());
    ARENA_HIP_CHECK(hipEventCreateWithFlags(&sl.copied, hipEventDisableTiming));
    for (hipEvent_t& e : sl.phase) ARENA_HIP_CHECK(hipEventCreateWithFlags(&e, hipEventDisableTiming));
    ARENA_HIP_CHECK(hipEventCreate(&sl.started));
    static const bool blocking = [] {
      const char* e = std::getenv("ARENA_SYNC");
      return e != nullptr && std::string(e) == "blocking";
    }();
    ARENA_HIP_CHECK(hipEventCreateWithFlags(&sl.done, blocking ? hipEventBlockingSync : hipEventDefault));
  }
}

void Executor::ensure_lanes(Slot& sl) {
  if (sl.fork_ev != nullptr) return;
  bool lanes = false;
  for (const OpRecord& r : prog_) lanes |= r[kLaneField] > 0;
  if (!lanes) return;
  for (int l = 0; l < kMaxLanes; ++l) {
    ARENA_HIP_CHECK(hipStreamCreateWithFlags(&sl.lane_stream[l], hipStreamNonBlocking));
    ARENA_HIP_CHECK(hipEventCreateWithFlags(&sl.lane_ev[l], hipEventDisableTiming));
  }
  ARENA_HIP_CHECK(hipEventCreateWithFlags(&sl.fork_ev, hipEventDisableTiming));
}

void Executor::set_weights(const void* host, size_t bytes) {
  ARENA_HIP_CHECK(hipSetDevice(cfg_.device));
  if (d_weights_ != nullptr && bytes != weights_bytes_) {
    if (!buckets_.empty()) throw std::runtime_error("set_weights: size change after buckets were captured");
    ARENA_HIP_CHECK(hipFree(d_weights_));
    d_weights_ = nullptr;
  }
  if (d_weights_ == nullptr) ARENA_HIP_CHECK(hipMalloc(&d_weights_, bytes));
  sync_slots();
  ARENA_HIP_CHECK(hipMemcpy(d_weights_, host, bytes, hipMemcpyHostToDevice));
  weights_bytes_ = bytes;
}

void Executor::set_weights_device(const void* dev, size_t bytes) {
  ARENA_HIP_CHECK(hipSetDevice(cfg_.device));
  if (d_weights_ == nullptr || bytes != weights_bytes_)
    throw std::runtime_error("set_weights_device: only a same-size update of uploaded weights is supported");
  sync_slots();
  ARENA_HIP_CHECK(hipMemcpy(d_weights_, dev, bytes, hipMemcpyDeviceToDevice));
}

std::vector<uint8_t> Executor::weights_host() {
  std::vector<uint8_t> out(weights_bytes_);
  if (d_weights_ == nullptr || weights_bytes_ == 0) return out;
  ARENA_HIP_CHECK(hipSetDevice(cfg_.device));
  sync_slots();
  ARENA_HIP_CHECK(hipMemcpy(out.data(), d_weights_, weights_bytes_, hipMemcpyDeviceToHost));
  return out;
}

void Executor::set_program(const int64_t* ops, int n_ops, const int64_t* cls_ops, int n_cls_ops) {
  prog_.resize(n_ops);
  for (int i = 0; i < n_ops; ++i) std::memcpy(prog_[i].data(), ops + (size_t)i * kOpFields, sizeof(OpRecord));
  cls_prog_.resize(n_cls_ops);
  for (int i = 0; i < n_cls_ops; ++i)
    std::memcpy(cls_prog_[i].data(), cls_ops + (size_t)i * kOpFields, sizeof(OpRecord));
  has_topk_ = has_det_ = has_raw_ = has_stamps_ = false;
  for (const auto& r : prog_) {
    has_topk_ |= r[0] == OP_TOPK;
    has_stamps_ |= r[0] == OP_STAMP;
    has_det_ |= r[0] == OP_NMS || r[0] == OP_CROPPLAN;
    for (int f = 1; f < kOpFields; ++f) has_raw_ |= r[f] == BUF_RAWOUT && (r[0] == OP_YOLORAW || r[0] == OP_CONV);
  }
  if (has_raw_ && cfg_.raw_out_bytes <= 0) throw std::runtime_error("program exports raw outputs: raw_out_bytes = 0");
  gate_pairs_ = head_gate_pairs(prog_.empty() ? nullptr : prog_[0].data(), n_ops, kOpFields);
}

int Executor::crop_cap_for(int B) const { return std::max(cfg_.min_crop_cap, B * cfg_.crop_cap_per_image); }

std::vector<int> Executor::buckets() const {
  std::vector<int> r;
  for (auto& kv : buckets_) r.push_back(kv.first);
  return r;
}

uintptr_t Executor::arena_ptr(int B) const {
  auto it = buckets_.find(B);
  return it == buckets_.end() ? 0 : (uintptr_t)it->second.d_arena[0];
}

void Executor::read_arena(int B, int64_t offset, void* dst, size_t bytes) {
  auto it = buckets_.find(B);
  if (it == buckets_.end()) throw std::runtime_error("read_arena: unknown bucket");
  if (offset < 0 || offset + (int64_t)bytes > it->second.info.arena_bytes)
    throw std::runtime_error("read_arena: range outside the arena");
  ARENA_HIP_CHECK(hipSetDevice(cfg_.device));
  sync_slots();
  ARENA_HIP_CHECK(hipMemcpy(dst, it->second.d_arena[it->second.last_slot] + offset, bytes, hipMemcpyDeviceToHost));
}

void Executor::add_bucket(int B, const int64_t* offsets, int n_buffers, int64_t arena_bytes,
                          const std::vector<int>* impl) {
  if (B <= 0 || B > max_B_) throw std::runtime_error("add_bucket: B outside (0, max_batch]");
  if (prog_.empty()) throw std::runtime_error("add_bucket: set_program first");
  if (d_weights_ == nullptr) throw std::runtime_error("add_bucket: set_weights first");
  ARENA_HIP_CHECK(hipSetDevice(cfg_.device));
  Bucket& bk = buckets_[B];
  bk.info.B = B;
  bk.info.crop_cap = crop_cap_for(B);
  bk.info.offsets.assign(offsets, offsets + n_buffers);
  bk.info.arena_bytes = arena_bytes;
  sync_slots();
  free_arenas(bk);
  const size_t abytes = (size_t)std::max<int64_t>(arena_bytes, 256);
  for (int s = 0; s < n_slots_; ++s) {
    ARENA_HIP_CHECK(hipMalloc(&bk.d_arena[s], abytes));
    ARENA_HIP_CHECK(hipMemset(bk.d_arena[s], 0, abytes));
  }
  bk.impl.assign(prog_.size(), 0);
  if (impl != nullptr) {
    if (impl->size() != prog_.size()) throw std::runtime_error("add_bucket: tuning table does not match the program");
    for (size_t i = 0; i < prog_.size(); ++i) {
      const int v = (*impl)[i];
      const bool f32 = prog_[i][kDtypeField] == 1;
      const bool ok = f32 ? (v >= 0 && v <= 2) || (v >= 10 && v < 10 + kF32Variants) ||
                                (v >= kF32X3 && v < kF32X3 + kF32X3Variants) || v == kF32Halo || v == kF32X3Halo ||
                                v == kF32X3HaloN3 || v == kF32X3HaloN2 || v == kF32Stream || v == kF32StreamN2 ||
                                v == kF32Fc || v == kF32StreamExact || v == kF32X3Halo16 || v == kF32X3Halo16N3 ||
                                v == kF32X3H16 || (v >= kF32X3G && v < kF32X3G + kF32X3GVariants) ||
                                (v >= kF32X3HG && v < kF32X3HG + kF32X3HGVariants) ||
                                (v >= kF32X3HGPw && v < kF32X3HGPw + kF32X3HGPwVariants) ||
                                (v >= kF32X3HGPwSmall && v < kF32X3HGPwSmall + kF32X3HGPwSmallVariants) ||
                                (v >= kF32X3HR && v < kF32X3HR + kF32X3HRVariants) ||
                                (v >= kF32X3HRPw && v < kF32X3HRPw + kF32X3HRPwVariants) ||
                                (v >= kF32X3HP && v < kF32X3HP + kF32X3HPVariants) ||
                                (v >= kF32X3GSK && v < kF32X3GSK + kF32X3GSKVariants)
                          : v >= 0 && v <= 3;
      if (!ok || (v != 0 && prog_[i][0] != OP_CONV)) throw std::runtime_error("add_bucket: bad tuning entry");
      bk.impl[i] = (int16_t)v;
    }
  } else if (autotune_) {
    autotune(bk);
  }
  for (int s = 0; s < n_slots_; ++s) capture(bk, s);
  if (debug_sync_ || std::getenv("ARENA_DEBUG_ALLOC")) {
    fprintf(stderr, "[arena alloc] bucket %d arena %p..%p (%lld B)\n", B, (void*)bk.d_arena[0],
            (void*)(bk.d_arena[0] + arena_bytes), (long long)arena_bytes);
    for (int s = 0; s < n_slots_; ++s)
      fprintf(stderr, "[arena alloc] slot %d in %p..%p out %p..%p\n", s, (void*)slots_[s].d_in,
              (void*)(slots_[s].d_in + in_bytes_total()), (void*)slots_[s].d_out,
              (void*)(slots_[s].d_out + out_bytes_total()));
    fprintf(stderr, "[arena alloc] weights %p..%p\n", (void*)d_weights_, (void*)(d_weights_ + weights_bytes_));
  }
}

void Executor::autotune(Bucket& bk) {
  Slot& sl = slots_[0];
  Ctrl c{};
  c.n_images = bk.info.B;
  c.n_crops = bk.info.crop_cap;
  ARENA_HIP_CHECK(hipStreamSynchronize(compute_));
  ARENA_HIP_CHECK(hipMemcpy(sl.d_in, &c, sizeof(Ctrl), hipMemcpyHostToDevice));
  hipEvent_t e0, e1;
  ARENA_HIP_CHECK(hipEventCreate(&e0));
  ARENA_HIP_CHECK(hipEventCreate(&e1));
  static const int kF32Candidates[] = {0,      12,     13,     14,     17,     19,     20,         21,
                                       23,     24,     kF32Halo, kF32X3, kF32X3 + 1, kF32X3 + 4, kF32X3 + 5,
                                       kF32X3 + 6, kF32X3 + 7, kF32X3 + 8, kF32X3Halo, kF32X3HaloN3,
                                       kF32X3HaloN2, kF32Stream, kF32StreamN2, kF32Fc, kF32StreamExact,
                                       kF32X3Halo16, kF32X3Halo16N3, kF32X3H16,
                                       kF32X3G + 5, kF32X3G + 6, kF32X3G + 7, kF32X3G + 9, kF32X3G + 15,
                                       kF32X3G + 16, kF32X3G + 17, kF32X3G + 19,
                                       kF32X3HG + 0, kF32X3HG + 1, kF32X3HG + 2, kF32X3HG + 4, kF32X3HG + 6,
                                       kF32X3HG + 7, kF32X3HG + 8, kF32X3HG + 9, kF32X3HG + 10,
                                       kF32X3HGPw + 0, kF32X3HGPw + 1, kF32X3HGPw + 2, kF32X3HGPw + 3,
                                       kF32X3HGPw + 4, kF32X3HGPw + 5, kF32X3HGPwSmall + 0, kF32X3HGPwSmall + 1,
                                       kF32X3HR + 0, kF32X3HR + 1, kF32X3HR + 2, kF32X3HR + 3, kF32X3HR + 4,
                                       kF32X3HR + 5, kF32X3HR + 6, kF32X3HR + 7, kF32X3HR + 8, kF32X3HR + 9,
                                       kF32X3HRPw + 0, kF32X3HRPw + 1, kF32X3HRPw + 2, kF32X3HRPw + 3,
                                       kF32X3HRPw + 4, kF32X3HRPw + 5,
                                       kF32X3HP + 0, kF32X3HP + 1, kF32X3HP + 2, kF32X3HP + 3, kF32X3HP + 4,
                                       kF32X3HP + 5, kF32X3HP + 6, kF32X3HP + 7, kF32X3HP + 8,
                                       kF32X3GSK + 0, kF32X3GSK + 1, kF32X3GSK + 2, kF32X3GSK + 3, kF32X3GSK + 4,
                                       kF32X3GSK + 5, kF32X3GSK + 6, kF32X3GSK + 7, kF32X3GSK + 8};
  static const int kBf16Candidates[] = {1, 2, 3};
  for (size_t i = 0; i < prog_.size(); ++i) {
    if (prog_[i][0] != OP_CONV) continue;
    const bool f32 = prog_[i][kDtypeField] == 1;
    if (prog_[i][1] == BUF_POOL) {
      bk.impl[i] = kF32X3H16;
      continue;
    }
    if (!f32 && prog_[i][34] > 0) {
      bk.impl[i] = 2;
      continue;
    }
    const int reps = f32 ? 5 : 3;
    std::vector<OpRecord> one(1, prog_[i]);
    float best = 1e30f;
    int best_impl = -1;
    const int* cand = f32 ? kF32Candidates : kBf16Candidates;
    const int n_cand = f32 ? (int)(sizeof(kF32Candidates) / sizeof(int)) : 3;
    for (int ci = 0; ci < n_cand; ++ci) {
      const int impl = cand[ci];
      try {
        enqueue_program(one, bk, sl, compute_, (int)i, impl);
      } catch (const std::runtime_error&) {
        continue;
      }
      ARENA_HIP_CHECK(hipEventRecord(e0, compute_));
      for (int k = 0; k < reps; ++k) enqueue_program(one, bk, sl, compute_, (int)i, impl);
      ARENA_HIP_CHECK(hipEventRecord(e1, compute_));
      ARENA_HIP_CHECK(hipEventSynchronize(e1));
      float ms = 0.f;
      ARENA_HIP_CHECK(hipEventElapsedTime(&ms, e0, e1));
      if (best_impl < 0 || ms < best * 0.97f) {
        best = ms;
        best_impl = impl;
      }
    }
    bk.impl[i] = (int16_t)std::max(best_impl, 0);
    if (autotune_ > 1)
      fprintf(stderr, "[arena autotune] B=%d op %zu -> impl %d (%.1f us)\n", bk.info.B, i, best_impl,
              best * 1e3f / reps);
  }
  ARENA_HIP_CHECK(hipEventDestroy(e0));
  ARENA_HIP_CHECK(hipEventDestroy(e1));
  ARENA_HIP_CHECK(hipMemset(bk.d_arena[0], 0, std::max<int64_t>(bk.info.arena_bytes, 256)));
}

static int lanes_max_batch() {
  static const int v = [] {
    const char* e = std::getenv("ARENA_LANES_MAX_BATCH");
    return e != nullptr ? std::atoi(e) : 2;
  }();
  return v;
}

bool Executor::lanes_for(const Bucket& bk) const {
  if (bk.info.B > lanes_max_batch()) return false;
  for (const OpRecord& r : prog_)
    if (r[kLaneField] >= 1 && r[kLaneField] <= kMaxLanes) return true;
  return false;
}

int64_t Executor::sk_lane_bytes() {
  static const int64_t v = [] {
    const char* e = std::getenv("ARENA_SPLITK_WS_MB");
    return (int64_t)std::max(1, e != nullptr ? std::atoi(e) : 16) << 20;
  }();
  return v;
}

void Executor::destroy_graphs(Bucket& bk, int s) {
  if (bk.graph[s]) hipGraphExecDestroy(bk.graph[s]);
  bk.graph[s] = nullptr;
  for (hipGraphExec_t g : bk.parts[s])
    if (g) hipGraphExecDestroy(g);
  bk.parts[s].clear();
  for (auto& sg : bk.segs[s])
    if (sg.g) hipGraphExecDestroy(sg.g);
  bk.segs[s].clear();
}

void Executor::capture(Bucket& bk, int s) {
  Slot& sl = slots_[s];
  hipStream_t st = sl.stream;
  ARENA_HIP_CHECK(hipStreamSynchronize(st));
  destroy_graphs(bk, s);
  if (s == 0) {
    bk.exec_order.clear();
    bk.gated.clear();
  }
  auto capture_range = [&](size_t a, size_t b) {
    std::vector<OpRecord> part(prog_.begin() + a, prog_.begin() + b);
    if (s == 0) {
      std::vector<const HeadGatePair*> gate;
      const std::vector<size_t> order = exec_plan(part, bk, (int)a, 0, gate);
      for (size_t k = 0; k < order.size(); ++k) {
        bk.exec_order.push_back((int)(a + order[k]));
        if (gate[k] != nullptr) bk.gated.push_back((int)(a + order[k]));
      }
    }
    hipGraph_t g = nullptr;
    hipGraphExec_t ge = nullptr;
    ARENA_HIP_CHECK(hipStreamBeginCapture(st, hipStreamCaptureModeThreadLocal));
    try {
      enqueue_program(part, bk, sl, st, (int)a);
    } catch (...) {
      hipStreamEndCapture(st, &g);
      if (g) hipGraphDestroy(g);
      throw;
    }
    ARENA_HIP_CHECK(hipStreamEndCapture(st, &g));
    ARENA_HIP_CHECK(hipGraphInstantiate(&ge, g, nullptr, nullptr, 0));
    ARENA_HIP_CHECK(hipGraphDestroy(g));
    return ge;
  };
  if (!lanes_for(bk)) {
    std::vector<size_t> cuts{0};
    if (bk.info.B >= 16)
      for (double f : stagger_) {
        const size_t k = (size_t)std::lround(f * (double)prog_.size());
        if (k > cuts.back() && k < prog_.size()) cuts.push_back(k);
      }
    if (cuts.size() > 1) {
      cuts.push_back(prog_.size());
      for (size_t i = 0; i + 1 < cuts.size(); ++i) bk.parts[s].push_back(capture_range(cuts[i], cuts[i + 1]));
    } else {
      bk.graph[s] = capture_range(0, prog_.size());
    }
    return;
  }
  ensure_lanes(sl);
  auto lane_of = [&](size_t i) {
    const int64_t l = prog_[i][kLaneField];
    return l >= 1 && l <= kMaxLanes ? (int)l : 0;
  };
  for (size_t a = 0; a < prog_.size();) {
    size_t b = a + 1;
    while (b < prog_.size() && lane_of(b) == lane_of(a)) ++b;
    Bucket::Seg sg;
    sg.lane = lane_of(a);
    sg.g = capture_range(a, b);
    bk.segs[s].push_back(sg);
    a = b;
  }
}

void Executor::launch_graph(Bucket& bk, int s, hipStream_t st, int n_live) {
  if (bk.segs[s].empty()) {
    if (!bk.parts[s].empty()) {
      int others = 0;
      for (int k = 0; k < n_slots_; ++k) others += k != s && slots_[k].busy ? 1 : 0;
      const bool gate = n_live < 0 || (n_live >= std::min(stagger_min_batch_, bk.info.B) && others >= 2);
      const Slot* prev = gate && last_launched_ >= 0 && last_launched_ != s ? &slots_[last_launched_] : nullptr;
      const size_t np = bk.parts[s].size();
      for (size_t i = 0; i < np; ++i) {
        if (prev && i + 1 < np) ARENA_HIP_CHECK(hipStreamWaitEvent(st, prev->phase[i], 0));
        ARENA_HIP_CHECK(hipGraphLaunch(bk.parts[s][i], st));
        ARENA_HIP_CHECK(hipEventRecord(slots_[s].phase[i], st));
      }
      last_launched_ = s;
      return;
    }
    ARENA_HIP_CHECK(hipGraphLaunch(bk.graph[s], st));
    return;
  }
  Slot& sl = slots_[s];
  bool forked[kMaxLanes] = {};
  bool fork_recorded = false;
  auto join = [&]() {
    for (int l = 0; l < kMaxLanes; ++l)
      if (forked[l]) {
        ARENA_HIP_CHECK(hipEventRecord(sl.lane_ev[l], sl.lane_stream[l]));
        ARENA_HIP_CHECK(hipStreamWaitEvent(st, sl.lane_ev[l], 0));
        forked[l] = false;
      }
    fork_recorded = false;
  };
  for (const Bucket::Seg& sg : bk.segs[s]) {
    if (sg.lane == 0) {
      join();
      ARENA_HIP_CHECK(hipGraphLaunch(sg.g, st));
      continue;
    }
    const int l = sg.lane - 1;
    if (!forked[l]) {
      if (!fork_recorded) {
        ARENA_HIP_CHECK(hipEventRecord(sl.fork_ev, st));
        fork_recorded = true;
      }
      ARENA_HIP_CHECK(hipStreamWaitEvent(sl.lane_stream[l], sl.fork_ev, 0));
      forked[l] = true;
    }
    ARENA_HIP_CHECK(hipGraphLaunch(sg.g, sl.lane_stream[l]));
  }
  join();
}

uint8_t* Executor::resolve(Bucket& bk, Slot& sl, int64_t buf, int64_t coff, int eb) {
  uint8_t* base = nullptr;
  switch (buf) {
    case BUF_NONE: return nullptr;
    case BUF_CTRL: base = sl.d_in; break;
    case BUF_META: base = sl.d_in + kCtrlBytes; break;
    case BUF_POOL: base = sl.d_in + in_bytes_meta(); break;
    case BUF_DETCOUNT: base = sl.d_out; break;
    case BUF_DET: base = sl.d_out + out_off_det(); break;
    case BUF_TOPK: base = sl.d_out + out_off_topk(); break;
    case BUF_RAWOUT: base = sl.d_out + out_off_raw(); break;
    case BUF_XCROPS: base = sl.d_out + out_off_xcrops(); break;
    default:
      if (buf < 0 || buf >= (int64_t)bk.info.offsets.size())
        throw std::runtime_error("program references unknown buffer " + std::to_string(buf));
      base = bk.d_arena[sl.idx] + bk.info.offsets[buf];
  }
  return base + coff * eb;
}

std::vector<size_t> Executor::exec_plan(const std::vector<OpRecord>& prog, const Bucket& bk, int op_offset,
                                        int force_impl, std::vector<const HeadGatePair*>& gate) const {
  std::vector<size_t> order(prog.size());
  for (size_t k = 0; k < order.size(); ++k) order[k] = k;
  gate.assign(prog.size(), nullptr);
  if (!g_head_gate || force_impl != 0) return order;
  for (const HeadGatePair& gp : gate_pairs_) {
    const long li = (long)gp.box - op_offset;
    float gm;
    if (li < 0 || li + 1 >= (long)prog.size() || gp.cls >= (int)prog_.size()) continue;
    if (!head_gate_min(gp.conf_thr, &gm)) continue;
    if (prog[li] != prog_[gp.box] || prog[li + 1] != prog_[gp.cls]) continue;
    const int impl = gp.box < (int)bk.impl.size() ? bk.impl[gp.box] : 0;
    const bool x3hg_pw = impl == 0 || (impl >= kF32X3HGPw && impl < kF32X3HGPw + kF32X3HGPwVariants) ||
                         (impl >= kF32X3HGPwSmall && impl < kF32X3HGPwSmall + kF32X3HGPwSmallVariants);
    if (!x3hg_pw) continue;
    order[li] = (size_t)li + 1;
    order[li + 1] = (size_t)li;
    gate[li + 1] = &gp;
  }
  return order;
}

void Executor::enqueue_program(const std::vector<OpRecord>& prog, Bucket& bk, Slot& sl, hipStream_t s_main,
                               int op_offset, int force_impl) {
  Ctrl* ctrl = (Ctrl*)resolve(bk, sl, BUF_CTRL, 0, 1);
  const ImageMeta* meta = (const ImageMeta*)resolve(bk, sl, BUF_META, 0, 1);
  const uint8_t* pool = resolve(bk, sl, BUF_POOL, 0, 1);
  const int B = bk.info.B, CC = bk.info.crop_cap;
  auto batch = [&](int64_t kind) { return kind == BATCH_CROPS ? CC : B; };
  auto bdev = [&](int64_t kind) -> const int* { return kind == BATCH_CROPS ? &ctrl->n_crops : &ctrl->n_images; };
  const uint8_t* W = d_weights_;

  std::vector<const HeadGatePair*> gate;
  const std::vector<size_t> order = exec_plan(prog, bk, op_offset, force_impl, gate);
  for (size_t k = 0; k < prog.size(); ++k) {
    const size_t oi = order[k];
    const OpRecord& r = prog[oi];
    hipStream_t s = s_main;
    const bool f32 = r[kDtypeField] == 1;
    const int eb = f32 ? 4 : 2;
    switch (r[0]) {
      case OP_CONV: {
        ConvParams p{};
        const size_t gi = (size_t)op_offset + oi;
        p.impl = force_impl ? force_impl : (gi < bk.impl.size() ? bk.impl[gi] : 0);
        p.x = resolve(bk, sl, r[1], r[2], eb);
        p.xs = (int)r[3];
        p.H = (int)r[4];
        p.W = (int)r[5];
        p.Cin = (int)r[6];
        p.w = W + r[7];
        p.Kpad = (int)r[8];
        p.bias = (const float*)(W + r[9]);
        p.f32out = (int)r[29];
        p.y = resolve(bk, sl, r[10], r[11], p.f32out ? 4 : eb);
        p.ys = (int)r[12];
        p.Ho = (int)r[13];
        p.Wo = (int)r[14];
        p.Cout = (int)r[15];
        p.Cout_pad = (int)r[16];
        p.KH = (int)r[17];
        p.KW = (int)r[18];
        p.stride = (int)r[19];
        p.pad_t = (int)r[20];
        p.pad_l = (int)r[21];
        p.res = resolve(bk, sl, r[22], r[23], eb);
        p.rs = (int)r[24];
        p.y2 = resolve(bk, sl, r[25], r[26], eb);
        p.y2s = (int)r[27];
        p.act = (int)r[28];
        p.B = batch(r[30]);
        p.bdev = bdev(r[30]);
        if (r[41] != 0) p.w3 = W + r[40];
        {
          const int64_t ln = r[kLaneField];
          const int li = ln >= 1 && ln <= kMaxLanes ? (int)ln : 0;
          p.sk_ws = (float*)((uint8_t*)sl.sk_ws + (size_t)li * sk_lane_bytes());
          p.sk_ws_bytes = sk_lane_bytes();
        }
        if (r[1] == BUF_POOL) {
          if (!f32 || r[30] != 0) throw std::runtime_error("executor: letterbox-source conv must be fp32 over images");
          p.x = nullptr;
          p.lb_pool = pool;
          p.lb_meta = meta;
          p.impl = kF32X3H16;
        }
        if (r[34] > 0) {
          p.pw_w = W + r[31];
          p.pw_kpad = (int)r[32];
          p.pw_bias = (const float*)(W + r[33]);
          p.pw_cout = (int)r[34];
          p.pw_y = resolve(bk, sl, r[36], r[37], eb);
          p.pw_ys = (int)r[38];
          p.pw_act = (int)r[39];
          if (!f32) p.impl = 2;
          if (gate[k] != nullptr) {
            p.gate = (const float*)resolve(bk, sl, r[36], r[37] + kHeadBoxChannels, eb);
            p.gate_n = kHeadClsChannels;
            head_gate_min(gate[k]->conf_thr, &p.gate_min);
          }
        }
        if (f32)
          conv2d_f32(p, s);
        else
          conv2d(p, s);
        break;
      }
      case OP_DWCONV: {
        DwParams p{};
        p.x = resolve(bk, sl, r[1], r[2], eb);
        p.xs = (int)r[3];
        p.H = (int)r[4];
        p.W = (int)r[5];
        p.C = (int)r[6];
        p.w = W + r[7];
        p.bias = (const float*)(W + r[8]);
        p.y = resolve(bk, sl, r[9], r[10], eb);
        p.ys = (int)r[11];
        p.Ho = (int)r[12];
        p.Wo = (int)r[13];
        p.stride = (int)r[14];
        p.act = (int)r[15];
        p.B = batch(r[16]);
        p.bdev = bdev(r[16]);
        if (f32)
          dwconv3x3_f32(p, s);
        else
          dwconv3x3(p, s);
        break;
      }
      case OP_IRBLOCK: {
        IrParams p{};
        p.x = resolve(bk, sl, r[1], r[2], eb);
        p.x_cs = (int)r[3];
        p.H = (int)r[4];
        p.W = (int)r[5];
        p.inp = (int)r[6];
        p.inp_pad = (int)r[7];
        p.hid_pad = (int)r[8];
        p.oup = (int)r[9];
        p.oup_pad = (int)r[10];
        p.stride = (int)r[11];
        p.expand = (int)r[12];
        p.res = (int)r[13];
        p.we = W + r[14];
        p.be = (const float*)(W + r[15]);
        p.wd = W + r[16];
        p.bd = (const float*)(W + r[17]);
        p.wp = W + r[18];
        p.bp = (const float*)(W + r[19]);
        p.y = resolve(bk, sl, r[20], r[21], eb);
        p.y_cs = (int)r[22];
        p.Ho = (int)r[23];
        p.Wo = (int)r[24];
        p.B = batch(r[25]);
        p.bdev = bdev(r[25]);
        p.x3w = (int)r[26];
        p.x_parts = (int)r[27];
        p.y_parts = (int)r[28];
        if (!f32 && (p.x_parts > 1 || p.y_parts > 1))
          throw std::runtime_error("executor: partial-sum ir_block tensors are fp32-only");
        p.stem = (int)r[31];
        if (p.stem) {
          p.st_pool = pool;
          p.st_meta = meta;
          p.st_crops = (const CropRef*)resolve(bk, sl, r[32], 0, 1);
          p.st_ctrl = ctrl;
          p.st_S = (int)r[33];
          for (int c = 0; c < 3; ++c) {
            p.st_mean[c] = bits_to_float(r[34 + c]);
            p.st_inv_std[c] = bits_to_float(r[37 + c]);
          }
          p.st_w = (const float*)(W + r[40]);
          p.st_b = (const float*)(W + r[41]);
        }
        if (f32)
          ir_block_f32(p, s);
        else
          ir_block(p, s);
        break;
      }
      case OP_SPPF: {
        SppfParams p{};
        p.buf = resolve(bk, sl, r[1], r[2], eb);
        p.xs = (int)r[3];
        p.H = (int)r[4];
        p.W = (int)r[5];
        p.C = (int)r[6];
        p.B = batch(r[7]);
        p.bdev = bdev(r[7]);
        if (f32)
          sppf_pool_f32(p, s);
        else
          sppf_pool(p, s);
        break;
      }
      case OP_LETTERBOX: {
        LetterboxParams p{};
        p.pool = pool;
        p.meta = meta;
        p.ctrl = ctrl;
        p.out = resolve(bk, sl, r[1], 0, eb);
        p.B = B;
        p.T = (int)r[2];
        p.f32 = f32;
        letterbox_s2d(p, s);
        break;
      }
      case OP_STAMP: {
        if (r[1] < 0 || r[1] >= 4) throw std::runtime_error("OP_STAMP: stamp index out of range");
        stamp(sl.d_out + out_off_stamps() + sizeof(uint64_t) * (size_t)r[1], s);
        break;
      }
      case OP_ZERO: {
        uint8_t* ptr = resolve(bk, sl, r[1], 0, 1);
        const size_t bytes = (size_t)r[2] * batch(r[3]);
        zero_fill(ptr, bytes, s);
        break;
      }
      case OP_DECODE: {
        DecodeParams p{};
        for (int l = 0; l < 3; ++l) {
          p.head[l] = resolve(bk, sl, r[1 + 4 * l], r[2 + 4 * l], eb);
          p.xs[l] = (int)r[3 + 4 * l];
          p.hw[l] = (int)r[4 + 4 * l];
          p.stride[l] = (float)r[13 + l];
        }
        p.cand = (Candidate*)resolve(bk, sl, r[16], 0, 1);
        p.cand_count = (int*)resolve(bk, sl, r[17], 0, 1);
        p.conf_thr = bits_to_float(r[18]);
        p.cand_cap = cfg_.cand_cap;
        p.B = B;
        p.ctrl = ctrl;
        p.f32 = f32;
        detect_decode(p, s);
        break;
      }
      case OP_NMS: {
        NmsParams p{};
        p.cand = (const Candidate*)resolve(bk, sl, r[1], 0, 1);
        p.cand_count = (const int*)resolve(bk, sl, r[2], 0, 1);
        p.cand_cap = cfg_.cand_cap;
        p.meta = meta;
        p.B = B;
        p.det = (Detection*)resolve(bk, sl, r[3], 0, 1);
        p.det_count = (int*)resolve(bk, sl, r[4], 0, 1);
        p.max_det = cfg_.max_det;
        p.iou_thr = bits_to_float(r[5]);
        p.ctrl = ctrl;
        nms(p, s);
        break;
      }
      case OP_CROPPLAN: {
// ... 748 lines not shown
```

csrc/runtime/executor.h:

```cpp
#pragma once
#include <chrono>
#include <hip/hip_runtime.h>

#include <array>
#include <atomic>
#include <condition_variable>
#include <cstdint>
#include <functional>
#include <map>
#include <mutex>
#include <thread>
#include <vector>

#include "../kernels/launch.h"
#include "head_gate.h"
#include "instance.h"

namespace arena {

constexpr int kOpFields = 48;
constexpr int kDtypeField = 47;
constexpr int kLaneField = 46;
constexpr int kMaxLanes = 3;
constexpr int kMaxSlots = 6;
constexpr int kMaxStaggerParts = 5;
constexpr int kMaxEstBuckets = 257;
using OpRecord = std::array<int64_t, kOpFields>;

void set_head_gate(bool v);
bool get_head_gate();

enum OpType : int64_t {
  OP_CONV = 1,
  OP_DWCONV = 2,
  OP_SPPF = 3,
  OP_LETTERBOX = 4,
  OP_ZERO = 5,
  OP_DECODE = 6,
  OP_NMS = 7,
  OP_CROPPLAN = 8,
  OP_CROPGATHER = 9,
  OP_AVGPOOL = 10,
  OP_TOPK = 11,
  OP_TENSORIN = 12,
  OP_YOLORAW = 13,
  OP_IRBLOCK = 14,
  OP_STEMFUSED = 15,
  OP_C3FUSED = 16,
  OP_HEADPOOL = 17,
  OP_STAMP = 18,
};

enum ReservedBuf : int64_t {
  BUF_NONE = -1,
  BUF_CTRL = -10,
  BUF_META = -11,
  BUF_POOL = -12,
  BUF_DET = -13,
  BUF_DETCOUNT = -14,
  BUF_TOPK = -15,
  BUF_RAWOUT = -16,
  BUF_XCROPS = -17,
};

enum BatchKind : int64_t { BATCH_IMAGES = 0, BATCH_CROPS = 1 };

struct ExecutorConfig {
  int device = 0;
  int max_batch = 32;
  int max_det = 300;
  int cand_cap = 8400;
  int crop_cap_per_image = 6;
  int min_crop_cap = 16;
  int64_t pool_bytes_per_image = 640LL * 640 * 3;
  int pool_factor = 3;
  int det_size = 640;
  int cls_size = 224;
  int host_threads = 8;
  int64_t raw_out_bytes = 0;
};

struct BucketInfo {
  int B = 0;
  int crop_cap = 0;
  std::vector<int64_t> offsets;
  int64_t arena_bytes = 0;
};

class Executor : public BatchInstance {
 public:
  explicit Executor(const ExecutorConfig& cfg);
  ~Executor() override;
  Executor(const Executor&) = delete;
  Executor& operator=(const Executor&) = delete;

  void set_weights(const void* host, size_t bytes);
  void set_weights_device(const void* dev, size_t bytes);
  std::vector<uint8_t> weights_host();
  void set_program(const int64_t* ops, int n_ops, const int64_t* cls_ops, int n_cls_ops);
  void add_bucket(int B, const int64_t* offsets, int n_buffers, int64_t arena_bytes,
                  const std::vector<int>* impl = nullptr);
  std::vector<int> buckets() const override;
  int crop_cap_for(int B) const;
  const ExecutorConfig& config() const { return cfg_; }
  int max_det() const override { return cfg_.max_det; }
  int64_t raw_out_bytes() const override { return cfg_.raw_out_bytes; }
  int64_t staging_bytes() const override { return (int64_t)pool_cap(); }

  int submit(const std::vector<InputImage>& imgs) override;
  BatchResult collect(int slot) override;
  int ready(int slot) override;
  double remaining_us(int slot) override;
  BatchResult run(const std::vector<InputImage>& imgs);

  int submit_peer(Executor& src, int src_slot);
  struct DeviceImage {
    uintptr_t ptr = 0;
    int h = 0, w = 0;
    int device = -1;
  };
  int submit_device(const std::vector<DeviceImage>& imgs, const std::vector<std::vector<Detection>>& dets);
  void set_peer_stage(bool v) { peer_stage_ = v; }
  bool peer_stage() const { return peer_stage_; }
  int device() const { return cfg_.device; }

  void replay(int B, int slot, int iters);
  void synchronize();
  int num_slots() const override { return n_slots_; }

  uintptr_t arena_ptr(int B) const;
  void read_arena(int B, int64_t offset, void* dst, size_t bytes);
  uintptr_t weights_ptr() const { return (uintptr_t)d_weights_; }
  uintptr_t stream() const { return (uintptr_t)compute_; }

 private:
  std::vector<uint8_t*> retired_h_in_;
  int64_t staging_growths_ = 0;

 public:
  int64_t staging_growths() const { return staging_growths_; }

 private:
  struct Slot {
    uint8_t* d_in = nullptr;
    uint8_t* d_out = nullptr;
    float* sk_ws = nullptr;
    uint8_t* h_in = nullptr;
    size_t h_cap = 0;
    uint8_t* h_out = nullptr;
    hipEvent_t copied = nullptr, started = nullptr, done = nullptr;
    hipEvent_t phase[kMaxStaggerParts] = {};
    hipStream_t stream = nullptr;
    hipStream_t lane_stream[kMaxLanes] = {};
    hipEvent_t fork_ev = nullptr, lane_ev[kMaxLanes] = {};
    int idx = 0;
    std::chrono::steady_clock::time_point t_submit{};
    bool polled = false;
    std::chrono::steady_clock::time_point t_poll{};
    bool busy = false;
    int bucket = 0;
    int n_images = 0;
    size_t in_used = 0;
  };
  struct Bucket {
    BucketInfo info;
    uint8_t* d_arena[kMaxSlots] = {};
    int last_slot = 0;
    hipGraphExec_t graph[kMaxSlots] = {};
    std::vector<hipGraphExec_t> parts[kMaxSlots];
    struct Seg {
      int lane = 0;
      hipGraphExec_t g = nullptr;
    };
    std::vector<Seg> segs[kMaxSlots];
    std::vector<int16_t> impl;
    std::vector<int> exec_order, gated;
  };

  void alloc_slots();
  void ensure_lanes(Slot& sl);
  void sync_slots();
  void free_arenas(Bucket& bk);
  void capture(Bucket& bk, int slot);
  void wait_done(Slot& sl);
  void note_done(Slot& sl);
  void release_copy(Slot& sl);
  static int64_t sk_lane_bytes();
  uint64_t copy_release_n_ = 0;
  void launch_graph(Bucket& bk, int slot, hipStream_t st, int n_live = -1);
  void destroy_graphs(Bucket& bk, int slot);
  bool lanes_for(const Bucket& bk) const;
  void enqueue_program(const std::vector<OpRecord>& prog, Bucket& bk, Slot& sl, hipStream_t s,
                       int op_offset = 0, int force_impl = 0);
  void autotune(Bucket& bk);
  std::vector<size_t> exec_plan(const std::vector<OpRecord>& prog, const Bucket& bk, int op_offset, int force_impl,
                                std::vector<const HeadGatePair*>& gate) const;

 public:
  std::vector<int> exec_order(int B) const {
    auto it = buckets_.find(B);
    return it == buckets_.end() ? std::vector<int>{} : it->second.exec_order;
  }
  std::vector<int> gated_ops(int B) const {
    auto it = buckets_.find(B);
    return it == buckets_.end() ? std::vector<int>{} : it->second.gated;
  }
  std::vector<int> conv_choices(int B) const {
    auto it = buckets_.find(B);
    if (it == buckets_.end()) return {};
    return std::vector<int>(it->second.impl.begin(), it->second.impl.end());
  }

 private:
  void enqueue_results_d2h(Bucket& bk, Slot& sl, int n);
  uint8_t* resolve(Bucket& bk, Slot& sl, int64_t buf, int64_t coff_elems, int elem_bytes);
  int pick_bucket(int n) const;
  size_t in_bytes_meta() const;
  size_t jpeg_desc_off() const;
  size_t pool_cap() const;
  size_t in_bytes_total() const;
  size_t out_off_det() const;
  size_t out_off_topk() const;
  size_t out_bytes_total() const;
  size_t out_off_raw() const;
  size_t out_off_xcrops() const;
  size_t out_off_stamps() const;
  int acquire_slot();
  void parallel_copy(std::vector<std::function<void()>>& jobs);

  ExecutorConfig cfg_;
  int max_B_ = 0;
  hipStream_t compute_ = nullptr, copy_ = nullptr;
  uint8_t* d_weights_ = nullptr;
  size_t weights_bytes_ = 0;
  std::vector<OpRecord> prog_, cls_prog_;
  std::vector<HeadGatePair> gate_pairs_;
  std::map<int, Bucket> buckets_;
  Slot slots_[kMaxSlots];
  int n_slots_ = 2;
  int next_slot_ = 0;
  hipStream_t streams_[kMaxSlots] = {};
  int n_streams_ = 1;
  uint64_t seq_ = 0;
  std::vector<double> stagger_;
  int stagger_min_batch_ = 32;
  int last_launched_ = -1;
  bool has_topk_ = false, has_det_ = false, has_raw_ = false, has_stamps_ = false;
  double wall_khz_ = 100000.0;
  bool peer_stage_ = false;
  std::vector<int> peer_enabled_;
  void enable_peer(int src, const char* what);
  int copy_mode_ = 0;
  int concurrent_ = 1;
  int autotune_ = 1;
  int debug_sync_ = 0;
  std::mutex mu_;
  std::vector<std::thread> workers_;
  std::mutex pool_mu_;
  std::condition_variable pool_cv_, pool_done_cv_;
  std::vector<std::function<void()>>* pool_jobs_ = nullptr;
  std::atomic<int> pool_next_{0};
  std::atomic<float> wall_est_us_[kMaxEstBuckets] = {};
  int pool_active_ = 0;
  uint64_t pool_gen_ = 0;
  bool pool_stop_ = false;
};

}
```

csrc/runtime/head_gate.h:

```cpp
#pragma once
#include <cmath>
#include <cstdint>
#include <cstring>
#include <vector>

namespace arena {

constexpr int kHeadBoxChannels = 64;
constexpr int kHeadClsChannels = 80;

constexpr double kHeadGateMargin = 1.0 / 64.0;
constexpr float kHeadGateThrMin = 1e-3f;
constexpr float kHeadGateThrMax = 0.999f;

inline bool head_gate_min(float conf_thr, float* gate_min) {
  if (!(conf_thr >= kHeadGateThrMin && conf_thr <= kHeadGateThrMax)) return false;
  const double t = (double)conf_thr;
  const double g = std::log(t / (1.0 - t)) - kHeadGateMargin;
  float f = (float)g;
  if ((double)f > g) f = std::nextafterf(f, -INFINITY);
  *gate_min = f;
  return true;
}

constexpr int64_t kHgOpConv = 1, kHgOpDecode = 6;
constexpr int kHgDtypeField = 47;

struct HeadGatePair {
  int box;
  int cls;
  int level;
  float conf_thr;
};

inline std::vector<HeadGatePair> head_gate_pairs(const int64_t* ops, int n, int fields) {
  std::vector<HeadGatePair> out;
  if (ops == nullptr || fields <= kHgDtypeField) return out;
  auto rec = [&](int i) { return ops + (size_t)i * fields; };
  for (int d = 0; d < n; ++d) {
    const int64_t* dr = rec(d);
    if (dr[0] != kHgOpDecode || dr[kHgDtypeField] != 1) continue;
    uint32_t bits = (uint32_t)dr[18];
    float thr;
    std::memcpy(&thr, &bits, 4);
    for (int l = 0; l < 3; ++l) {
      const int64_t buf = dr[1 + 4 * l], coff = dr[2 + 4 * l], cs = dr[3 + 4 * l], hw = dr[4 + 4 * l];
      if (buf < 0) continue;
      for (int i = 0; i + 1 < d; ++i) {
        const int64_t* a = rec(i);
        const int64_t* c = rec(i + 1);
        if (a[0] != kHgOpConv || a[kHgDtypeField] != 1 || c[0] != kHgOpConv || c[kHgDtypeField] != 1) continue;
        if (!(a[34] == kHeadBoxChannels && a[36] == buf && a[37] == coff && a[38] == cs && a[13] == hw && a[14] == hw))
          continue;
        const bool c_pw = c[34] > 0;
        const int64_t cb = c_pw ? c[36] : c[10], cc = c_pw ? c[37] : c[11], cst = c_pw ? c[38] : c[12];
        const int64_t cn = c_pw ? c[34] : c[15];
        if (!(cn == kHeadClsChannels && cb == buf && cc == coff + kHeadBoxChannels && cst == cs && c[13] == hw &&
              c[14] == hw && c[30] == a[30]))
          continue;
        const bool disjoint = a[1] != c[1] || a[2] + a[6] <= c[2] || c[2] + c[6] <= a[2];
        if (!disjoint || a[1] == buf || c[1] == buf || a[22] >= 0 || c[22] >= 0) continue;
        out.push_back(HeadGatePair{i, i + 1, l, thr});
        break;
      }
    }
  }
  return out;
}

}
```

inference_arena_amd/engine/plans.py:

```python
from __future__ import annotations

import os

import torch

from ..models.common import fold, fold_conv_bn
from ..models.mobilenetv2 import MobileNetV2
from ..models.yolov5nu import STRIDES, YOLOv5nu
from .planner import BUF_NONE, BUF_RAWOUT, BUF_XCROPS, CROPS, IMAGES, Program, ProgramBuilder, Reserved, View

CAND_BYTES = 32
CROPREF_BYTES = 32


def s2d_stem_6x6(w: torch.Tensor) -> torch.Tensor:
    co = w.shape[0]
    out = torch.zeros(co, 16, 3, 3)
    for a in range(3):
        for b in range(3):
            for p in range(2):
                for q in range(2):
                    for c in range(3):
                        out[:, (p * 2 + q) * 3 + c, a, b] = w[:, c, 2 * a + p, 2 * b + q]
    return out
# ... 13 lines not shown
C3_FUSED = {(32, 16, 1, True), (64, 32, 2, True), (128, 32, 1, False)}
C3_FUSED_AUTO = {(32, 16, 1, True)}


def fuse_c3_policy() -> str:
    v = os.environ.get("ARENA_FUSE_C3", "auto").lower()
    return {"0": "none", "false": "none", "off": "none", "1": "auto", "true": "auto"}.get(v, v)


def fuse_c3_f32() -> bool:
    return os.environ.get("ARENA_FUSE_C3_F32", "1").lower() not in ("0", "false", "no", "off")


def _c3(pb: ProgramBuilder, m, src: View, dst: View, H: int, W: int, name: str) -> None:
    c_ = m.c_
    res = bool(m.m[0].add)
    if pb.f32:
        allowed = {(32, 16, 1, True)} if fuse_c3_f32() and fuse_c3_policy() != "none" else set()
    else:
        policy = fuse_c3_policy()
        allowed = C3_FUSED if policy == "all" else C3_FUSED_AUTO if policy == "auto" else set()
    if ((src.C, c_, len(m.m), res) in allowed and H % 8 == 0 and W % 16 == 0
            and all(bool(bn.add) == res for bn in m.m)):
        w1, b1 = fold(m.cv1)
        w2, b2 = fold(m.cv2)
        pb.c3_fused(src, dst, H, W, (torch.cat([w1, w2]), torch.cat([b1, b2])),
                    [(fold(bn.cv1), fold(bn.cv2)) for bn in m.m], fold(m.cv3), res=res)
        return
    T = pb.tensor(f"{name}.T", H, W, 2 * c_)
    U = pb.tensor(f"{name}.U", H, W, c_)
    w1, b1 = fold(m.cv1)
    w2, b2 = fold(m.cv2)
    pb.conv(src, View(T, 0, 2 * c_), torch.cat([w1, w2]), torch.cat([b1, b2]))
    for bn in m.m:
        wa, ba = fold(bn.cv1)
        pb.conv(View(T, 0, c_), View(U, 0, c_), wa, ba)
        wb, bb = fold(bn.cv2)
        pb.conv(View(U, 0, c_), View(T, 0, c_), wb, bb, res=View(T, 0, c_) if bn.add else None)
    w3, b3 = fold(m.cv3)
    pb.conv(View(T, 0, 2 * c_), dst, w3, b3)


def fuse_stem_default() -> bool:
    return os.environ.get("ARENA_FUSE_STEM", "1").lower() not in ("0", "false", "no", "off")


def fuse_stem2_default() -> bool:
    return os.environ.get("ARENA_FUSE_STEM2", "1").lower() not in ("0", "false", "no", "off")


def fuse_stem_ir_default() -> bool:
    return os.environ.get("ARENA_FUSE_STEM_IR", "1").lower() not in ("0", "false", "no", "off")


def fuse_head_pool_default() -> bool:
    return os.environ.get("ARENA_FUSE_POOL", "1").lower() not in ("0", "false", "no", "off")


def fuse_letterbox_f32_default() -> bool:
    return os.environ.get("ARENA_F32_LB_STEM", "1").lower() not in ("0", "false", "no", "off")


def fuse_stem_s2_f32_default() -> bool:
    return os.environ.get("ARENA_F32_STEM_S2", "1").lower() not in ("0", "false", "no", "off")


def plan_yolo(pb: ProgramBuilder, y: YOLOv5nu, T: int = 640, tensor_input: bool = False,
              fuse_stem: bool | None = None):
    h = T // 2
    w, b = fold(y.b0)
    if fuse_stem is None:
        fuse_stem = fuse_stem_default()
    fuse_stem = fuse_stem and (not pb.f32 or fuse_stem_s2_f32_default())
    A1 = pb.tensor("b1", h // 2, h // 2, 32)
    if fuse_stem and not tensor_input and (fuse_stem2_default() or pb.f32) and T % 64 == 0:
        w1, b1 = fold(y.b1)
        pb.stem_fused(View(A1, 0, 32), s2d_stem_6x6(w), b, S=T, act="silu", second=(w1, b1, "silu"))
    elif fuse_stem and not tensor_input and not pb.f32:
        A0 = pb.tensor("b0", h, h, 16)
        pb.stem_fused(View(A0, 0, 16), s2d_stem_6x6(w), b, S=T, act="silu")
        pb.conv(View(A0, 0, 16), View(A1, 0, 32), *fold(y.b1), stride=2)
    elif pb.f32 and not tensor_input and fuse_letterbox_f32_default():
        A0 = pb.tensor("b0", h, h, 16)
        pb.letterbox_conv(View(A0, 0, 16), s2d_stem_6x6(w), b, T=T)
        pb.conv(View(A0, 0, 16), View(A1, 0, 32), *fold(y.b1), stride=2)
    else:
        A0 = pb.tensor("b0", h, h, 16)
        X0 = pb.tensor("x_s2d", h, h, 16)
        if tensor_input:
            pb.tensor_in(X0, T)
        else:
            pb.letterbox(X0, T)
        pb.conv(View(X0, 0, 16), View(A0, 0, 16), s2d_stem_6x6(w), b)
        pb.conv(View(A0, 0, 16), View(A1, 0, 32), *fold(y.b1), stride=2)
    A2 = pb.tensor("b2", h // 2, h // 2, 32)
    _c3(pb, y.b2, View(A1, 0, 32), View(A2, 0, 32), h // 2, h // 2, "b2")
    s8 = T // 8
    A3 = pb.tensor("b3", s8, s8, 64)
    pb.conv(View(A2, 0, 32), View(A3, 0, 64), *fold(y.b3), stride=2)
    CAT16 = pb.tensor("cat16", s8, s8, 128)
    _c3(pb, y.b4, View(A3, 0, 64), View(CAT16, 64, 64), s8, s8, "b4")
    s16 = T // 16
    A5 = pb.tensor("b5", s16, s16, 128)
    pb.conv(View(CAT16, 64, 64), View(A5, 0, 128), *fold(y.b5), stride=2, src_hw=(s8, s8))
    CAT12 = pb.tensor("cat12", s16, s16, 256)
    _c3(pb, y.b6, View(A5, 0, 128), View(CAT12, 128, 128), s16, s16, "b6")
    s32 = T // 32
    A7 = pb.tensor("b7", s32, s32, 256)
    pb.conv(View(CAT12, 128, 128), View(A7, 0, 256), *fold(y.b7), stride=2)
    A8 = pb.tensor("b8", s32, s32, 256)
    _c3(pb, y.b8, View(A7, 0, 256), View(A8, 0, 256), s32, s32, "b8")
    S9 = pb.tensor("sppf", s32, s32, 512)
    c_ = y.b9.c_
    pb.conv(View(A8, 0, 256), View(S9, 0, c_), *fold(y.b9.cv1))
    pb.sppf(S9, c_)
    A9 = pb.tensor("b9", s32, s32, 256)
    pb.conv(View(S9, 0, 4 * c_), View(A9, 0, 256), *fold(y.b9.cv2))
    CAT22 = pb.tensor("cat22", s32, s32, 256)
    pb.conv(View(A9, 0, 256), View(CAT22, 128, 128), *fold(y.h10), dst2=View(CAT12, 0, 128))
    A13 = pb.tensor("h13", s16, s16, 128)
    _c3(pb, y.h13, View(CAT12, 0, 256), View(A13, 0, 128), s16, s16, "h13")
    CAT19 = pb.tensor("cat19", s16, s16, 128)
    pb.conv(View(A13, 0, 128), View(CAT19, 64, 64), *fold(y.h14), dst2=View(CAT16, 0, 64))
    P3 = pb.tensor("p3", s8, s8, 64)
    _c3(pb, y.h17, View(CAT16, 0, 128), View(P3, 0, 64), s8, s8, "h17")
    pb.conv(View(P3, 0, 64), View(CAT19, 0, 64), *fold(y.h18), stride=2)
    P4 = pb.tensor("p4", s16, s16, 128)
    _c3(pb, y.h20, View(CAT19, 0, 128), View(P4, 0, 128), s16, s16, "h20")
    pb.conv(View(P4, 0, 128), View(CAT22, 0, 128), *fold(y.h21), stride=2)
    P5 = pb.tensor("p5", s32, s32, 256)
    _c3(pb, y.h23, View(CAT22, 0, 256), View(P5, 0, 256), s32, s32, "h23")

    d = y.detect
    c2, c3, nc = d.c2, d.c3, d.nc
    fuse_head = os.environ.get("ARENA_FUSE_HEAD", "1").lower() not in ("0", "false", "no", "off")
    ch = c2 + c3
    heads = []
    lanes = head_lanes()
    region = pb.parallel()
    lane = region.__enter__()
    for lvl, (P, cin, s) in enumerate(((P3, 64, s8), (P4, 128, s16), (P5, 256, s32))):
        lane(lvl + 1 if lanes else 0)
        H1 = pb.tensor(f"det{lvl}.h1", s, s, ch)
        H2 = pb.tensor(f"det{lvl}.h2", s, s, ch)
        D = pb.tensor(f"det{lvl}.out", s, s, 4 * d.reg_max + nc)
        wa, ba = fold(d.cv2[lvl][0])
        wc, bc = fold(d.cv3[lvl][0])
        pb.conv(View(P, 0, cin), View(H1, 0, ch), torch.cat([wa, wc]), torch.cat([ba, bc]))
        if fuse_head and c2 in (64, 80) and c3 in (64, 80) and (not pb.f32 or s >= 40):
            pb.conv(View(H1, 0, c2), View(BUF_NONE, 0, c2), *fold(d.cv2[lvl][1]),
                    pw=(*fold_conv_bn(d.cv2[lvl][2], None), View(D, 0, 4 * d.reg_max), None))
            pb.conv(View(H1, c2, c3), View(BUF_NONE, 0, c3), *fold(d.cv3[lvl][1]),
                    pw=(*fold_conv_bn(d.cv3[lvl][2], None), View(D, 4 * d.reg_max, nc), None))
        else:
            pb.conv(View(H1, 0, c2), View(H2, 0, c2), *fold(d.cv2[lvl][1]))
            pb.conv(View(H1, c2, c3), View(H2, c2, c3), *fold(d.cv3[lvl][1]))
            pb.conv(View(H2, 0, c2), View(D, 0, 4 * d.reg_max), *fold_conv_bn(d.cv2[lvl][2], None), act=None)
            pb.conv(View(H2, c2, c3), View(D, 4 * d.reg_max, nc), *fold_conv_bn(d.cv3[lvl][2], None), act=None)
        heads.append(View(D, 0, 4 * d.reg_max + nc))
    region.__exit__(None, None, None)
    return heads


def head_lanes() -> bool:
    return os.environ.get("ARENA_HEAD_LANES", "0").lower() not in ("0", "false", "no", "off")


def fuse_ir_default() -> str:
    v = os.environ.get("ARENA_FUSE_IR", "auto").lower()
    return {"0": "none", "1": "all", "false": "none", "true": "all"}.get(v, v)


def ir_crop_default() -> bool:
    return os.environ.get("ARENA_IR_CROP", "1").lower() not in ("0", "false", "no", "off")


def fuse_block_f32(blk, H: int) -> bool:
    from .planner import ir_crop_f32_planned
    from .validate import ir_f32_supported

    inp_pad = (blk.inp + 15) // 16 * 16
    hid_pad = inp_pad if blk.expand is None else (blk.hidden + 31) // 32 * 32
    oup_pad = (blk.oup + 15) // 16 * 16
    expand = int(blk.expand is not None)
    if H >= 28:
        return ir_f32_supported(blk.stride, inp_pad, hid_pad, oup_pad, expand)
    return ir_crop_f32_planned(H, blk.stride, inp_pad, hid_pad, oup_pad, expand)


def irx_slices() -> int:
    try:
        return max(1, min(8, int(os.environ.get("ARENA_IRX_SLICES", "6"))))
    except ValueError:
        return 6


def _sliceable_f32(blk, H: int) -> bool:
    from .planner import ir_crop_f32_planned

    if H not in (14, 7) or blk.expand is None or blk.inp % 4 or blk.oup % 4:
        return False
    inp_pad = (blk.inp + 15) // 16 * 16
    hid_pad = (blk.hidden + 31) // 32 * 32
    oup_pad = (blk.oup + 15) // 16 * 16
    return hid_pad // 32 >= irx_slices() and ir_crop_f32_planned(H, blk.stride, inp_pad, hid_pad, oup_pad, 1)


def fuse_stem_ir_f32_default() -> bool:
    return os.environ.get("ARENA_F32_STEM_IR", "1").lower() not in ("0", "false", "no", "off")


def fuse_block(blk, H: int, policy) -> bool:
    if policy == "f32":
        return fuse_block_f32(blk, H)
    """``auto``: fuse where the tile kernel wins on MI355X — blocks at >= 28x28 input and the stride-1
    14x14 blocks (hid 576: 46 us fused vs 28 + 18 + 17 us as expand / depthwise / project ops;
    profiles/r1_irpolicy14_ops.md).  The 14 -> 7 stride-2 block and the 7x7 blocks have one
    output tile per crop and a 18-30 chunk serial loop in the tile kernel: unless the whole-crop
    kernel takes them (``ARENA_IR_CROP``, default 1: csrc/kernels/ir_crop.hip, waves split the hidden
    channels; <= 160 or 320 output channels) they run as batched 1x1 GEMMs + depthwise over all crops."""
    if policy in (True, "all"):
        return True
    if policy in (False, None, "none"):
        return False
    if H >= 28 or (H >= 14 and blk.stride == 1):
        return True
    Ho = (H + 2 - 3) // blk.stride + 1
    return ir_crop_default() and Ho == 7 and blk.expand is not None and (blk.oup <= 160 or blk.oup == 320)


def plan_mobilenet(pb: ProgramBuilder, m: MobileNetV2, crops, S: int, mean, std, *, kind: int = CROPS,
                   raw_logits: bool = False, fuse_ir: bool | str | None = None, fuse_stem: bool | None = None):
    CROPS_ = kind
    if fuse_ir is None:
        fuse_ir = fuse_ir_default()
    h = S // 2
    if fuse_stem is None:
        fuse_stem = fuse_stem_default()
    if pb.f32:
        fuse_stem = False
        fuse_ir = "f32" if fuse_ir in ("auto", True, "all", "f32") else "none"
    w, b = fold(m.stem)
    b0 = m.blocks[0]
    first_fused = (fuse_stem and crops is not None and fuse_stem_ir_default() and S % 32 == 0
                   and b0.expand is None and b0.stride == 1 and not b0.use_res and b0.inp == 32 and b0.oup == 16
                   and fuse_block(b0, h, fuse_ir))
    first_fused_f32 = (pb.f32 and crops is not None and fuse_stem_ir_f32_default() and S % 2 == 0
                       and b0.expand is None and b0.stride == 1 and not b0.use_res and b0.inp == 32
                       and b0.oup <= 16 and h >= 16)
    if first_fused:
        O0 = pb.tensor("m0.out", h, h, b0.oup, kind=CROPS_)
        pb.stem_fused(View(O0, 0, b0.oup), s2d_stem_3x3(w), b, S=S, act="relu6", crops=crops, mean=mean, std=std,
                      kind=CROPS_, ir=(fold(b0.dw), fold(b0.project)))
        F = O0
    elif first_fused_f32:
        O0 = pb.tensor("m0.out", h, h, b0.oup, kind=CROPS_)
        pb.ir_block_stem(crops, View(O0, 0, b0.oup), (s2d_stem_3x3(w), b), fold(b0.dw), fold(b0.project), S=S,
                         mean=mean, std=std, kind=CROPS_)
        F = O0
        first_fused = True
    elif fuse_stem and crops is not None:
        F = pb.tensor("m.stem", h, h, 32, kind=CROPS_)
        pb.stem_fused(View(F, 0, 32), s2d_stem_3x3(w), b, S=S, act="relu6", crops=crops, mean=mean, std=std,
                      kind=CROPS_)
    else:
        F = pb.tensor("m.stem", h, h, 32, kind=CROPS_)
        X = pb.tensor("crop_s2d", h, h, 16, kind=CROPS_)
        if crops is None:
            pb.tensor_in(X, S)
        else:
            pb.crop_gather(crops, X, S, mean, std)
        pb.conv(View(X, 0, 16), View(F, 0, 32), s2d_stem_3x3(w), b, pad=(1, 1), act="relu6", kind=CROPS_,
                out_hw=(h, h))
    cur, H = F, h
    parts = 1
    slices = irx_slices() if pb.f32 and fuse_ir == "f32" else 1
    for i, blk in enumerate(m.blocks):
        if i == 0 and first_fused:
            continue
        Ho = (H + 2 - 3) // blk.stride + 1
        if fuse_block(blk, H, fuse_ir):
            nxt = m.blocks[i + 1] if i + 1 < len(m.blocks) else None
            yp = slices if (slices > 1 and _sliceable_f32(blk, H) and nxt is not None
                            and fuse_block(nxt, Ho, fuse_ir) and _sliceable_f32(nxt, Ho)) else 1
            O = pb.tensor(f"m{i}.out", Ho, Ho, blk.oup * yp, kind=CROPS_)
            pb.ir_block(View(cur, 0, blk.inp * parts), View(O, 0, blk.oup * yp),
                        fold(blk.expand) if blk.expand is not None else None, fold(blk.dw), fold(blk.project),
                        stride=blk.stride, res=blk.use_res, kind=CROPS_, x_parts=parts, y_parts=yp)
            cur, H, parts = O, Ho, yp
            continue
        if parts != 1:
            raise AssertionError("partial-sum tensor feeds an unfused block")
        if blk.expand is not None:
            E = pb.tensor(f"m{i}.exp", H, H, blk.hidden, kind=CROPS_)
            pb.conv(View(cur, 0, blk.inp), View(E, 0, blk.hidden), *fold(blk.expand), act="relu6", kind=CROPS_)
        else:
            E = cur
        Dw = pb.tensor(f"m{i}.dw", Ho, Ho, blk.hidden, kind=CROPS_)
        wd, bd = fold(blk.dw)
        pb.dwconv(View(E, 0, blk.hidden), View(Dw, 0, blk.hidden), wd, bd, stride=blk.stride, kind=CROPS_)
        O = pb.tensor(f"m{i}.out", Ho, Ho, blk.oup, kind=CROPS_)
        pb.conv(View(Dw, 0, blk.hidden), View(O, 0, blk.oup), *fold(blk.project), act=None,
                res=View(cur, 0, blk.inp) if blk.use_res else None, kind=CROPS_)
        cur, H = O, Ho
    PO = pb.tensor("m.pool", 1, 1, 1280, kind=CROPS_)
    if fuse_head_pool_default() and H * H <= 64 and cur.C == 320:
# ... 101 lines not shown
```

inference_arena_amd/ops/functional.py:

```python
from __future__ import annotations

import ctypes
import struct

import numpy as np
import torch

from ..engine.planner import ACT, pack_conv_weight, pack_conv_weight_x3
from . import native

IMAGE_META = struct.Struct("<qiiiiiif12x")


def _stream() -> int:
    return torch.cuda.current_stream().cuda_stream


def _ptr(t: torch.Tensor | None, elem_off: int = 0) -> int:
    if t is None:
        return 0
    return t.data_ptr() + elem_off * t.element_size()


def pack_weights(w: torch.Tensor, b: torch.Tensor, device, dtype: str = "bf16"):
    wb, bb, kpad, cpad = pack_conv_weight(w.detach().cpu().float(), b.detach().cpu().float(), dtype)
    wt = torch.frombuffer(bytearray(wb), dtype=torch.float32 if dtype == "fp32" else torch.bfloat16).to(device)
    bt = torch.frombuffer(bytearray(bb), dtype=torch.float32).to(device)
    w3 = None
    if dtype == "fp32":
        w3 = torch.frombuffer(bytearray(pack_conv_weight_x3(w.detach().cpu().float())), dtype=torch.int16).to(device)
    return wt, bt, kpad, cpad, w3


def conv2d_nhwc(x: torch.Tensor, w: torch.Tensor, b: torch.Tensor, *, stride: int = 1, pad=None, act=None,
                x_coff: int = 0, cin: int | None = None, out: torch.Tensor | None = None, out_coff: int = 0,
                res: torch.Tensor | None = None, res_coff: int = 0, out2: torch.Tensor | None = None,
                out2_coff: int = 0, f32out: bool = False, out_hw=None, bdev: torch.Tensor | None = None,
                packed=None, impl: int = 0, pw=None, pw_out: torch.Tensor | None = None, pw_out_coff: int = 0,
                gate=None) -> torch.Tensor:
    f32 = x.dtype == torch.float32
    B, H, W, Cx = x.shape
    cout, cin_w, kh, kw = w.shape
    cin = cin or cin_w
    if pad is None:
        pad = (kh // 2, kw // 2)
    if isinstance(pad, int):
        pad = (pad, pad)
    if out_hw is None:
        Ho = (H + 2 * pad[0] - kh) // stride + 1
        Wo = (W + 2 * pad[1] - kw) // stride + 1
    else:
        Ho, Wo = out_hw
    if out is None:
        out = torch.empty(B, Ho, Wo, cout, dtype=torch.float32 if (f32out or f32) else torch.bfloat16, device=x.device)
    wt, bt, kpad, cpad, w3 = packed if packed is not None else pack_weights(w, b, x.device, "fp32" if f32 else "bf16")
    pwd = {}
    if pw is not None:
        from ..engine.planner import pack_pw_weight_x3

        if not f32:
            raise ValueError("conv2d_nhwc: the functional fused pointwise path is fp32-only")
        w2, b2 = pw
        co2 = w2.shape[0]
        k2 = (cout + 31) // 32 * 32
        w2p = torch.frombuffer(bytearray(pack_pw_weight_x3(w2.detach().cpu().float(), k2)),
                               dtype=torch.int16).to(x.device)
        b2p = torch.zeros((co2 + 15) // 16 * 16)
        b2p[:co2] = b2.detach().float()
        b2p = b2p.to(x.device)
        if pw_out is None:
            out = torch.empty(B, Ho, Wo, co2, dtype=torch.float32, device=x.device)
            pw_out_coff = 0
        else:
            out = pw_out
            if (out.shape[:3] != (B, Ho, Wo) or out.shape[3] < pw_out_coff + co2 or out.dtype != torch.float32
                    or out.device != x.device or not out.is_contiguous()):
                raise ValueError(f"conv2d_nhwc: pw_out {tuple(out.shape)} {out.dtype} does not fit the 1x1 output")
        pwd = {"pw_w": _ptr(w2p), "pw_bias": _ptr(b2p), "pw_y": _ptr(out, pw_out_coff), "pw_ys": out.shape[-1],
               "pw_cout": co2, "pw_kpad": k2, "pw_act": 0}
        if gate is not None:
            gt, gcoff, gn, gmin = gate
            if (gt.shape != out.shape or gt.dtype != torch.float32 or gt.device != x.device or not gt.is_contiguous()
                    or gcoff < 0 or gn <= 0 or gcoff + gn > gt.shape[3]):
                raise ValueError("conv2d_nhwc: the gate logits must match the 1x1 output tensor's shape and stride")
            pwd.update({"gate": _ptr(gt, gcoff), "gate_n": int(gn), "gate_min": float(gmin)})
    elif gate is not None or pw_out is not None:
        raise ValueError("conv2d_nhwc: gate / pw_out need pw")
    skd = {}
    if 171 <= int(impl) < 180:
        ws = torch.empty(8 * B * Ho * Wo * cpad, dtype=torch.float32, device=x.device)
        skd = {"sk_ws": _ptr(ws), "sk_ws_bytes": ws.numel() * 4}
    native().conv2d({
        "x": _ptr(x, x_coff), "B": B, "H": H, "W": W, "xs": Cx, "Cin": cin,
        "w": _ptr(wt), "Kpad": kpad, "bias": _ptr(bt),
        "y": _ptr(out, out_coff), "Ho": Ho, "Wo": Wo, "ys": out.shape[-1], "Cout": cout, "Cout_pad": cpad,
        "KH": kh, "KW": kw, "stride": stride, "pad_t": pad[0], "pad_l": pad[1],
        "res": _ptr(res, res_coff), "rs": res.shape[-1] if res is not None else 0,
        "y2": _ptr(out2, out2_coff), "y2s": out2.shape[-1] if out2 is not None else 0,
        "act": ACT[act], "f32out": int(f32out), "bdev": _ptr(bdev), "stream": _stream(), "f32": int(f32),
        "impl": int(impl), "w3": _ptr(w3), **pwd, **skd,
    })
    if pw is not None:
        torch.cuda.synchronize(x.device)
    return out


def dwconv3x3_nhwc(x: torch.Tensor, w: torch.Tensor, b: torch.Tensor, *, stride: int = 1, act="relu6",
                   bdev: torch.Tensor | None = None) -> torch.Tensor:
    B, H, W, C = x.shape
    f32 = x.dtype == torch.float32
    Ho, Wo = (H - 1) // stride + 1, (W - 1) // stride + 1
    y = torch.empty(B, Ho, Wo, C, dtype=x.dtype, device=x.device)
    wt = w.detach().float().reshape(C, 9).t().contiguous().to(x.dtype).to(x.device)
    bt = b.detach().float().contiguous().to(x.device)
    native().dwconv3x3({"x": _ptr(x), "B": B, "H": H, "W": W, "xs": C, "C": C, "w": _ptr(wt), "bias": _ptr(bt),
                        "y": _ptr(y), "Ho": Ho, "Wo": Wo, "ys": C, "stride": stride, "act": ACT[act],
                        "bdev": _ptr(bdev), "stream": _stream(), "f32": int(f32)})
    return y


def ir_block_nhwc(x: torch.Tensor, expand, dw, project, *, stride: int, res: bool = False,
                  bdev: torch.Tensor | None = None, x_parts: int = 1, y_parts: int = 1,
                  out: torch.Tensor | None = None) -> torch.Tensor:
    from ..engine.planner import ir_x3_plan, pack_ir_weights, split_bf16x3

    B, H, W, Ct = x.shape
    C = Ct // x_parts
    f32 = x.dtype == torch.float32
    pk = pack_ir_weights(expand, dw, project, C, k_align=16 if f32 else 32)
    x3w = 0
    if f32:
        x3w, inp_x3 = ir_x3_plan(H, W, stride, C, pk["hid_pad"], pk["oup_pad"], int(expand is not None))
        if x3w and inp_x3 != pk["inp_pad"]:
            pk = pack_ir_weights(expand, dw, project, C, k_align=32)
    Ho, Wo = (H - 1) // stride + 1, (W - 1) // stride + 1
    y = out if out is not None else torch.empty(B, Ho, Wo, pk["oup"] * y_parts, dtype=x.dtype, device=x.device)
    if (y.shape[:3] != (B, Ho, Wo) or y.shape[3] < pk["oup"] * y_parts or y.dtype != x.dtype or y.device != x.device
            or not y.is_contiguous()):
        raise ValueError(f"ir_block_nhwc: out {tuple(y.shape)} {y.dtype} does not fit the block's output")
    mat = torch.float32 if f32 else torch.bfloat16
    dev = {k: (pk[k].to(mat) if k in ("we", "wd", "wp") else pk[k].float()).contiguous().to(x.device)
           for k in ("we", "be", "wd", "bd", "wp", "bp")}
    if x3w:
        dev["we"] = split_bf16x3(pk["we"]).to(x.device)
        dev["wp"] = split_bf16x3(pk["wp"]).to(x.device)
    native().ir_block({"x": _ptr(x), "x_cs": Ct, "H": H, "W": W, "inp": C, "inp_pad": pk["inp_pad"],
                       "hid_pad": pk["hid_pad"], "oup": pk["oup"], "oup_pad": pk["oup_pad"], "stride": stride,
                       "expand": int(expand is not None), "res": int(res),
                       **{k: _ptr(v) for k, v in dev.items()}, "y": _ptr(y), "y_cs": y.shape[3], "Ho": Ho,
                       "Wo": Wo, "B": B, "bdev": _ptr(bdev), "stream": _stream(), "f32": int(f32), "x3w": x3w,
                       "x_parts": x_parts, "y_parts": y_parts})
    torch.cuda.synchronize(x.device)
    return y


def c3_x3_nhwc(x: torch.Tensor, cv12, bottleneck, cv3) -> torch.Tensor:
    from ..engine.planner import split_bf16x3

    B, H, W, C = x.shape
    (w1, b1), (w2, b2) = bottleneck
    w2k = torch.zeros(16, 160)
    w2k[:, :144] = w2.detach().float().permute(0, 2, 3, 1).reshape(16, 144)
    dev = {"w12": split_bf16x3(cv12[0].reshape(32, 32)), "b12": cv12[1].float(),
           "wb1": split_bf16x3(w1.reshape(16, 16)), "bb1": b1.float(), "wb2": split_bf16x3(w2k), "bb2": b2.float(),
           "w3": split_bf16x3(cv3[0].reshape(32, 32)), "b3": cv3[1].float()}
    dev = {k: v.contiguous().to(x.device) for k, v in dev.items()}
    y = torch.empty(B, H, W, 32, dtype=torch.float32, device=x.device)
    native().c3_block({"x": _ptr(x), "xs": C, "B": B, "H": H, "W": W, "bdev": 0, "C1": 32, "CH": 16, "NB": 1,
                       "res": 1, **{k: _ptr(v) for k, v in dev.items()}, "y": _ptr(y), "ys": 32,
                       "stream": _stream(), "f32": 1})
    torch.cuda.synchronize(x.device)
    return y


def sppf_nhwc(buf: torch.Tensor, C: int) -> torch.Tensor:
    B, H, W, Ct = buf.shape
    native().sppf_pool({"buf": _ptr(buf), "B": B, "H": H, "W": W, "xs": Ct, "C": C, "stream": _stream(),
                        "f32": int(buf.dtype == torch.float32)})
    return buf


def image_meta_bytes(images: list[np.ndarray], T: int) -> tuple[bytes, np.ndarray]:
    from ..processing.transforms import letterbox_geometry

    metas, chunks, off = [], [], 0
    for im in images:
        h, w = im.shape[:2]
        scale, nw, nh, pw, ph = letterbox_geometry(h, w, T)
        metas.append(IMAGE_META.pack(off, h, w, nw, nh, pw, ph, scale))
        data = np.ascontiguousarray(im, np.uint8).tobytes()
        pad = (-len(data)) % 256
        chunks.append(data + b"\0" * pad)
        off += len(data) + pad
    return b"".join(metas), np.frombuffer(b"".join(chunks), dtype=np.uint8)


def ctrl_tensor(n_images: int, device, n_crops: int = 0, crop_base: int = 0) -> torch.Tensor:
    c = torch.zeros(16, dtype=torch.int32)
    c[0], c[1], c[2] = n_images, n_crops, crop_base
    return c.to(device)


def letterbox_s2d(images: list[np.ndarray], T: int, device, dtype=torch.bfloat16) -> torch.Tensor:
    meta, pool = image_meta_bytes(images, T)
    meta_t = torch.frombuffer(bytearray(meta), dtype=torch.uint8).to(device)
    pool_t = torch.from_numpy(pool.copy()).to(device)
    ctrl = ctrl_tensor(len(images), device)
    out = torch.empty(len(images), T // 2, T // 2, 16, dtype=dtype, device=device)
    native().letterbox_s2d({"pool": _ptr(pool_t), "meta": _ptr(meta_t), "ctrl": _ptr(ctrl), "out": _ptr(out),
                            "B": len(images), "T": T, "stream": _stream(), "f32": int(dtype == torch.float32)})
    torch.cuda.current_stream().synchronize()
    return out


def s2d_to_nchw(x: torch.Tensor) -> torch.Tensor:
    B, h, w, _ = x.shape
    y = x[..., :12].float().reshape(B, h, w, 2, 2, 3)
    return y.permute(0, 5, 1, 3, 2, 4).reshape(B, 3, 2 * h, 2 * w)


def avgpool_nhwc(x: torch.Tensor) -> torch.Tensor:
    B, H, W, C = x.shape
    y = torch.empty(B, C, dtype=x.dtype, device=x.device)
    native().global_avgpool({"x": _ptr(x), "B": B, "HW": H * W, "C": C, "y": _ptr(y), "stream": _stream(),
                             "f32": int(x.dtype == torch.float32)})
    return y


def head_pool_nhwc(x: torch.Tensor, w: torch.Tensor, b: torch.Tensor, act: str | None = "relu6",
                   bdev: torch.Tensor | None = None) -> torch.Tensor:
    from ..engine.planner import ACT, pack_conv_weight

    B, H, W, C = x.shape
    N = w.shape[0]
    f32 = x.dtype == torch.float32
    wb, bb, kpad, npad = pack_conv_weight(w, b, "fp32" if f32 else "bf16")
    wd = torch.frombuffer(bytearray(wb), dtype=torch.float32 if f32 else torch.bfloat16).to(x.device)
    bd = torch.frombuffer(bytearray(bb), dtype=torch.float32).to(x.device)
    y = torch.empty(B, N, dtype=x.dtype, device=x.device)
    native().head_pool({"x": _ptr(x), "xs": C, "HW": H * W, "K": C, "w": _ptr(wd), "Kpad": kpad, "bias": _ptr(bd),
                        "N": N, "Npad": npad, "y": _ptr(y), "ys": N, "act": ACT[act], "B": B, "bdev": _ptr(bdev),
                        "stream": _stream(), "f32": int(f32)})
    torch.cuda.synchronize(x.device)
    return y


def topk_softmax(logits: torch.Tensor):
    B, N = logits.shape
    out = torch.empty(B, 16, dtype=torch.int32, device=logits.device)
    native().topk_softmax({"logits": _ptr(logits), "B": B, "N": N, "ld": logits.stride(0), "out": _ptr(out),
                           "stream": _stream()})
    torch.cuda.current_stream().synchronize()
    o = out.cpu()
    return o[:, 0:5].clone(), o[:, 5:10].view(torch.float32).clone(), o[:, 10:15].view(torch.float32).clone()
```

inference_arena_amd/utils/settings.py:

```python
from __future__ import annotations

import functools
import os
from pathlib import Path

from pydantic import BaseModel


def _read_dotenv(path: Path) -> dict[str, str]:
    out: dict[str, str] = {}
    if not path.exists():
        return out
    for line in path.read_text(encoding="utf-8").splitlines():
        line = line.strip()
        if not line or line.startswith("#") or "=" not in line:
            continue
        k, v = line.split("=", 1)
        v = v.strip()
        if v[:1] in ("'", '"') and v[0] in v[1:]:
            v = v[1:v.index(v[0], 1)]
        else:
            v = v.split(" #", 1)[0].split("\t#", 1)[0].strip()
        out[k.strip()] = v
    return out


class Settings(BaseModel):
    LOG_LEVEL: str = "INFO"
    PORT: int = 8100
    HOST: str = "0.0.0.0"
    MODELS_DIR: str = "model_repository"
    LABELS_FILE: str = ""
    CLASSIFICATION_GRPC_ENDPOINT: str = "127.0.0.1:8201"
    TRITON_GRPC_ENDPOINT: str = "127.0.0.1:8001"
    TRITON_HTTP_ENDPOINT: str = "127.0.0.1:8000"
    TRITON_TIMEOUT_SECONDS: float = 60.0
    ARENA_DEVICE: str = "gpu"
    ARENA_GPU: int = 0
    ARENA_GPUS: str = ""
    ARENA_CLS_GPU: int = -1
    ARENA_MAX_BATCH: int = 32
    ARENA_QUEUE_DELAY_US: int = 500
    ARENA_DECODE_THREADS: int = 8
    ARENA_CONFIDENCE: str = ""
    ARENA_CROP_TRANSPORT: str = "jpeg"
    ARENA_DEVICE_RING_SLOTS: int = 512
    ARENA_CROP_ENCODE: str = "pil"
    ARENA_FANOUT: str = "parallel"
    ARENA_GATEWAY_MODE: str = "pipeline"
    ARENA_INSTANCES: int = 1
    ARENA_WEIGHT_SEED: int = 0
    ARENA_FAULT_EVERY: int = 0
    ARENA_INFER_SERVICE: int = 0
    ARENA_IR_S2K16: int = 1
    ARENA_HEAD_GATE: int = 1

    @classmethod
    def from_env(cls, env_file: str | Path = ".env", **overrides) -> "Settings":
        vals: dict[str, str] = _read_dotenv(Path(env_file))
        for k in cls.model_fields:
            if k in os.environ:
                vals[k] = os.environ[k]
        vals.update({k: v for k, v in overrides.items() if v is not None})
        return cls(**vals)


@functools.lru_cache
def get_settings() -> Settings:
    return Settings.from_env()
```

Baseline: 10960.

## Split first detect-head conv into class/box windows and gate box tiles by class marks

Splits the first 3x3 conv of each detection head into a class-channel launch and a box-channel launch using an output-channel window in the x3hp kernel. A new head_mark kernel scans class logits per 8x8 cell and marks cells above the gate threshold. The box-side conv then skips producer tiles whose consumer region has no marked cell. This is meant to avoid computing box features where no detection can survive, at the cost of extra launches, a mark pass and arena space for the marks.

```diff
diff --git a/csrc/bindings.cpp b/csrc/bindings.cpp
--- a/csrc/bindings.cpp
+++ b/csrc/bindings.cpp
@@ -87,6 +87,12 @@
   p.gate = ptr<const float*>(d, "gate");
   p.gate_n = get<int>(d, "gate_n", 0);
   p.gate_min = get<float>(d, "gate_min", 0.f);
+  p.n_lo = get<int>(d, "n_lo", 0);
+  p.n_hi = get<int>(d, "n_hi", 0);
+  p.marks = ptr<const int*>(d, "marks");
+  p.mark_uh = get<int>(d, "mark_uh", 0);
+  p.mark_uw = get<int>(d, "mark_uw", 0);
+  p.mark_halo = get<int>(d, "mark_halo", 0);
   p.w3 = ptr<const void*>(d, "w3");
   p.sk_ws = ptr<float*>(d, "sk_ws");
   p.sk_ws_bytes = get<int64_t>(d, "sk_ws_bytes", 0);
@@ -95,6 +101,30 @@
     conv2d_f32(p, stream_of(d));
   else
     conv2d(p, stream_of(d));
+}
+
+void py_head_mark(const py::dict& d) {
+  HeadMarkParams p{};
+  const std::vector<uintptr_t> logits = req<std::vector<uintptr_t>>(d, "logits");
+  const std::vector<uintptr_t> marks = req<std::vector<uintptr_t>>(d, "marks");
+  const std::vector<int> H = req<std::vector<int>>(d, "H"), W = req<std::vector<int>>(d, "W");
+  const std::vector<int> ps = req<std::vector<int>>(d, "ps");
+  const size_t n = logits.size();
+  if (n < 1 || n > (size_t)kMarkMaxLevels || marks.size() != n || H.size() != n || W.size() != n || ps.size() != n)
+    throw std::runtime_error("head_mark: 1..3 levels, one entry per level in every list");
+  p.n_levels = (int)n;
+  for (size_t l = 0; l < n; ++l) {
+    p.logits[l] = reinterpret_cast<const float*>(logits[l]);
+    p.marks[l] = reinterpret_cast<int*>(marks[l]);
+    p.H[l] = H[l];
+    p.W[l] = W[l];
+    p.ps[l] = ps[l];
+  }
+  p.n = req<int>(d, "n");
+  p.gate_min = req<float>(d, "gate_min");
+  p.B = req<int>(d, "B");
+  p.bdev = ptr<const int*>(d, "bdev");
+  head_mark(p, stream_of(d));
 }
 
 void py_dwconv(const py::dict& d) {
@@ -617,6 +647,42 @@
         return out;
       },
       py::arg("ops"), "[(box conv op, class conv op, level)] of a program's records");
+  m.def("set_head_split", &set_head_split);
+  m.def("get_head_split", &get_head_split);
+  m.attr("HEAD_SPLIT_MIN_BUCKET") = kHeadSplitMinBucket;
+  m.attr("HEAD_SPLIT_BOX_IMPL") = kF32X3HP + kHeadSplitBoxVariant;
+  m.attr("HEAD_SPLIT_CLS_IMPL") = kF32X3HP + kHeadSplitClsVariant;
+  m.attr("MARK_CELL") = kMarkCell;
+  m.def("head_mark", &py_head_mark);
+  m.def(
+      "head_gate_first_convs",
+      [](py::array_t<int64_t, py::array::c_style> ops) {
+        if (ops.ndim() != 2 || ops.shape(1) != kOpFields) throw std::runtime_error("ops must be int64 [n, OP_FIELDS]");
+        py::list out;
+        for (const HeadGatePair& gp : head_gate_pairs(ops.data(), (int)ops.shape(0), kOpFields))
+          out.append(head_gate_first_conv(ops.data(), (int)ops.shape(0), kOpFields, gp));
+        return out;
+      },
+      py::arg("ops"), "per head-gate pair of a program's records: the op of its first head conv, or -1");
+  m.def(
+      "head_marks_needed",
+      [](py::array_t<int, py::array::c_style | py::array::forcecast> marks, int H, int W, int th, int tw, int uh,
+         int uw, int halo) {
+        if (H <= 0 || W <= 0 || th <= 0 || tw <= 0 || uh <= 0 || uw <= 0 || halo < 0 || marks.ndim() != 2 ||
+            marks.shape(0) != head_mark_cells(H) || marks.shape(1) != head_mark_cells(W))
+          throw std::runtime_error("head_marks_needed: marks must be int32 [ceil(H / 8), ceil(W / 8)], sizes > 0");
+        const int nty = (H + th - 1) / th, ntx = (W + tw - 1) / tw;
+        py::array_t<bool> out({nty, ntx});
+        auto o = out.mutable_unchecked<2>();
+        for (int ty = 0; ty < nty; ++ty)
+          for (int tx = 0; tx < ntx; ++tx)
+            o(ty, tx) = head_marks_needed(marks.data(), H, W, ty, tx, th, tw, uh, uw, halo);
+        return out;
+      },
+      py::arg("marks"), py::arg("H"), py::arg("W"), py::arg("th"), py::arg("tw"), py::arg("uh"), py::arg("uw"),
+      py::arg("halo"),
+      "bool [tiles_y, tiles_x]: the th x tw producer tiles of one image that a continuing uh x uw consumer tile, "
+      "grown by halo pixels, reads (the host oracle of the x3hp mark gate)");
   m.attr("HEAD_BOX_CHANNELS") = kHeadBoxChannels;
   m.attr("HEAD_CLS_CHANNELS") = kHeadClsChannels;
   m.def("letterbox_s2d", &py_letterbox);
@@ -800,6 +866,9 @@
       .def("exec_order", &Executor::exec_order, py::arg("B"),
            "program op indices in the order bucket B's graphs launch them")
       .def("gated_ops", &Executor::gated_ops, py::arg("B"), "ops of bucket B that run with a tile gate")
+      .def("launch_order", &Executor::launch_order, py::arg("B"),
+           "every kernel launch of bucket B's graphs in order as (op, kind): 0 the whole op, 1 / 2 the class / "
+           "box window of a split first head conv, 3 the cell marks launched before op's box conv")
       .def("stream", &Executor::stream);
 
   py::class_<SplitInstance, std::shared_ptr<SplitInstance>>(m, "SplitInstance")
diff --git a/csrc/kernels/conv_f32.hip b/csrc/kernels/conv_f32.hip
--- a/csrc/kernels/conv_f32.hip
+++ b/csrc/kernels/conv_f32.hip
@@ -1412,17 +1412,16 @@
     throw std::runtime_error("conv2d_f32: unsupported geometry (Cin/xs/ys %4, Kpad %16, Cout_pad %16, Cout %4)");
   if (p.Cin < 16) throw std::runtime_error("conv2d_f32: Cin must be >= 16");
   if (p.Kpad < p.KH * p.KW * p.Cin) throw std::runtime_error("conv2d_f32: Kpad < KH*KW*Cin");
+  if ((p.n_lo != 0 || p.n_hi != 0 || p.marks != nullptr) &&
+      !(p.pw_w == nullptr && p.impl >= kF32X3HP && p.impl < kF32X3HP + kF32X3HPVariants))
+    throw std::runtime_error("conv2d_f32: an output-channel window or a mark gate needs an x3hp variant");
   if (p.pw_w != nullptr) {
     if (p.impl >= kF32X3HRPw && p.impl < kF32X3HRPw + kF32X3HRPwVariants) {
       if (!conv_x3hr_pw(p, s, p.impl - kF32X3HRPw))
         throw std::runtime_error("conv2d_f32: a fused pointwise epilogue needs an x3hr-pw variant that fits the conv");
       return;
     }
-    const int v = p.impl >= kF32X3HGPw && p.impl < kF32X3HGPw + kF32X3HGPwVariants ? p.impl - kF32X3HGPw
-                  : p.impl >= kF32X3HGPwSmall && p.impl < kF32X3HGPwSmall + kF32X3HGPwSmallVariants
-                      ? kF32X3HGPwVariants + p.impl - kF32X3HGPwSmall
-                  : p.impl == 0 ? (p.Cout_pad <= 64 ? 0 : 2)
-                                : -1;
+    const int v = x3hg_pw_variant(p.impl, p.Cout_pad);
     if (v < 0 || !conv_x3hg_pw(p, s, v))
       throw std::runtime_error("conv2d_f32: a fused pointwise epilogue needs an x3hg-pw variant that fits the conv");
     return;
diff --git a/csrc/kernels/halo_x3g.hip b/csrc/kernels/halo_x3g.hip
--- a/csrc/kernels/halo_x3g.hip
+++ b/csrc/kernels/halo_x3g.hip
@@ -580,6 +580,24 @@
          (p.gate == nullptr ||
           (p.gate_n > 0 && p.gate_n <= HG_GATE_MAX_N && p.gate_n % 4 == 0 && p.gate_n <= p.pw_ys &&
            (uintptr_t)p.gate % 16 == 0));
+}
+
+int x3hg_pw_variant(int impl, int cout_pad) {
+  return impl >= kF32X3HGPw && impl < kF32X3HGPw + kF32X3HGPwVariants ? impl - kF32X3HGPw
+         : impl >= kF32X3HGPwSmall && impl < kF32X3HGPwSmall + kF32X3HGPwSmallVariants
+             ? kF32X3HGPwVariants + impl - kF32X3HGPwSmall
+         : impl == 0 ? (cout_pad <= 64 ? 0 : 2)
+                     : -1;
+}
+
+bool x3hg_pw_tile(int impl, int cout_pad, int* th, int* tw) {
+  switch (x3hg_pw_variant(impl, cout_pad)) {
+#define HG_PW_TILE(V, TW, WM, TM, TN, PWN) \
+  case V: *th = hg_th(TW, WM, TM); *tw = TW; return true;
+    HG_PW_VARIANTS(HG_PW_TILE)
+#undef HG_PW_TILE
+    default: return false;
+  }
 }
 
 bool conv_x3hg_pw(const ConvParams& p, hipStream_t s, int v) {
diff --git a/csrc/kernels/halo_x3p.hip b/csrc/kernels/halo_x3p.hip
--- a/csrc/kernels/halo_x3p.hip
+++ b/csrc/kernels/halo_x3p.hip
@@ -1,6 +1,7 @@
 #include <stdexcept>
 #include <string>
 
+#include "../runtime/head_marks.h"
 #include "common.h"
 #include "launch.h"
 
@@ -49,8 +50,12 @@
   const int t = bx - b * tiles;
   const int ty = t / tiles_x, tx = t - ty * tiles_x;
   const int oy0 = ty * TH, ox0 = tx * HP_TW;
+  if (p.marks != nullptr) {
+    const int* m = p.marks + (size_t)b * head_mark_cells(p.Ho) * head_mark_cells(p.Wo);
+    if (!head_marks_needed(m, p.Ho, p.Wo, ty, tx, TH, HP_TW, p.mark_uh, p.mark_uw, p.mark_halo)) return;
+  }
   const int iy0 = oy0 - p.pad_t, ix0 = ox0 - p.pad_l;
-  const int n0 = blockIdx.y * BN;
+  const int n0 = p.n_lo + blockIdx.y * BN;
   const int H = p.H, W = p.W, Cin = p.Cin;
 
   const __amdgpu_buffer_rsrc_t xr = __builtin_amdgcn_make_buffer_rsrc(
@@ -176,7 +181,7 @@
 #pragma unroll
   for (int j = 0; j < NF; ++j) {
     const int cb = n0 + j * 16 + kq * 4;
-    if (cb >= p.Cout) continue;
+    if (cb >= p.n_hi) continue;
     const float4 bias = *(const float4*)(p.bias + cb);
 #pragma unroll
     for (int f = 0; f < MF; ++f) {
@@ -208,10 +213,14 @@
 namespace {
 
 template <int NF, int TH, int TS>
-void hp_launch(const ConvParams& p, hipStream_t s) {
+void hp_launch(const ConvParams& p0, hipStream_t s) {
   constexpr int BN = NF * 16;
+  ConvParams p = p0;
+  const bool whole = p.n_lo == 0 && p.n_hi == 0;
+  if (whole) p.n_hi = p.Cout;
   const int tiles = ((p.Wo + HP_TW - 1) / HP_TW) * ((p.Ho + TH - 1) / TH);
-  dim3 grid((unsigned)(p.B * tiles), (unsigned)((p.Cout_pad + BN - 1) / BN));
+  const int span = whole ? p.Cout_pad : p.n_hi - p.n_lo;
+  dim3 grid((unsigned)(p.B * tiles), (unsigned)((span + BN - 1) / BN));
   hipLaunchKernelGGL((conv_x3hp_kernel<NF, TH, TS>), grid, dim3(TH * 32), hp_lds_bytes(NF, TH, TS), s, p);
 }
 
@@ -224,7 +233,8 @@
   X(5, 3, 16, 3)   \
   X(6, 4, 16, 3)   \
   X(7, 9, 8, 1)    \
-  X(8, 9, 16, 1)
+  X(8, 9, 16, 1)   \
+  X(9, 5, 8, 1)
 
 }
 
@@ -234,7 +244,11 @@
   return p.w3 != nullptr && p.KH == 3 && p.KW == 3 && p.stride == 1 && p.Cin % 4 == 0 && p.xs % 4 == 0 &&
          x_bytes < (1u << 31) - (1u << 20) && w_bytes < (1u << 31) - (1u << 20) && p.Cout % 4 == 0 &&
          p.Cout_pad % 16 == 0 && p.ys % 4 == 0 && (p.res == nullptr || p.rs % 4 == 0) &&
-         (p.y2 == nullptr || p.y2s % 4 == 0) && p.lb_meta == nullptr && p.pw_w == nullptr;
+         (p.y2 == nullptr || p.y2s % 4 == 0) && p.lb_meta == nullptr && p.pw_w == nullptr &&
+         ((p.n_lo == 0 && p.n_hi == 0) ||
+          (p.n_lo >= 0 && p.n_lo % 16 == 0 && p.n_hi > p.n_lo && p.n_hi <= p.Cout && p.n_hi % 4 == 0)) &&
+         (p.marks == nullptr || ((uintptr_t)p.marks % 4 == 0 && p.mark_uh > 0 && p.mark_uw > 0 &&
+                                 p.mark_uh % kMarkCell == 0 && p.mark_uw % kMarkCell == 0 && p.mark_halo >= 0));
 }
 
 bool conv_x3hp(const ConvParams& p, hipStream_t s, int v) {
diff --git a/csrc/kernels/head_mark.hip b/csrc/kernels/head_mark.hip
--- /dev/null
+++ b/csrc/kernels/head_mark.hip
@@ -0,0 +1,71 @@
+#include <stdexcept>
+#include <string>
+
+#include "../runtime/head_marks.h"
+#include "common.h"
+#include "launch.h"
+
+namespace arena {
+
+namespace {
+constexpr int HM_WAVES = 4;
+}
+
+template <int NQ>
+__global__ __launch_bounds__(HM_WAVES * 64) void head_mark_kernel(const HeadMarkParams p) {
+  const int lane = threadIdx.x & 63, wave = threadIdx.x >> 6;
+  int g = blockIdx.x * HM_WAVES + wave;
+  const int live = live_batch(p.B, p.bdev);
+  int l = 0, ncy = 0, ncx = 0;
+  for (; l < p.n_levels; ++l) {
+    ncy = head_mark_cells(p.H[l]);
+    ncx = head_mark_cells(p.W[l]);
+    if (g < p.B * ncy * ncx) break;
+    g -= p.B * ncy * ncx;
+  }
+  if (l >= p.n_levels) return;
+  const float* logits = l == 0 ? p.logits[0] : l == 1 ? p.logits[1] : p.logits[2];
+  int* marks = l == 0 ? p.marks[0] : l == 1 ? p.marks[1] : p.marks[2];
+  const int H = l == 0 ? p.H[0] : l == 1 ? p.H[1] : p.H[2];
+  const int W = l == 0 ? p.W[0] : l == 1 ? p.W[1] : p.W[2];
+  const int ps = l == 0 ? p.ps[0] : l == 1 ? p.ps[1] : p.ps[2];
+  const int cells = ncy * ncx;
+  const int b = g / cells;
+  if (b >= live) return;
+  const int c = g - b * cells;
+  const int cy = c / ncx, cx = c - cy * ncx;
+  const float nan = __builtin_nanf("");
+  const float* img = logits + (size_t)b * H * W * ps;
+  float4 v[NQ];
+#pragma unroll
+  for (int j = 0; j < NQ; ++j) {
+    const int i = lane + 64 * j;
+    const int px = i / NQ, q = i - px * NQ;
+    const int y = cy * kMarkCell + (px >> 3), x = cx * kMarkCell + (px & 7);
+    v[j] = make_float4(nan, nan, nan, nan);
+    if (y < H && x < W) v[j] = *(const float4*)(img + ((size_t)y * W + x) * ps + 4 * q);
+  }
+  const float gm = p.gate_min;
+  int any = 0;
+#pragma unroll
+  for (int j = 0; j < NQ; ++j) any |= (v[j].x >= gm) | (v[j].y >= gm) | (v[j].z >= gm) | (v[j].w >= gm);
+  const int hot = __any(any);
+  if (lane == 0) marks[(size_t)b * cells + c] = hot ? 1 : 0;
+}
+
+void head_mark(const HeadMarkParams& p, hipStream_t s) {
+  if (p.n_levels <= 0 || p.n_levels > kMarkMaxLevels || p.B <= 0 || p.n != 80)
+    throw std::runtime_error("head_mark: 1..3 levels of 80 logits per pixel");
+  long total = 0;
+  for (int l = 0; l < p.n_levels; ++l) {
+    if (p.logits[l] == nullptr || p.marks[l] == nullptr || p.H[l] <= 0 || p.W[l] <= 0 || p.ps[l] < p.n ||
+        p.ps[l] % 4 != 0 || (uintptr_t)p.logits[l] % 16 != 0 || (uintptr_t)p.marks[l] % 4 != 0)
+      throw std::runtime_error("head_mark: level " + std::to_string(l) + ": pointers, map size or pixel stride");
+    total += (long)p.B * head_mark_cells(p.H[l]) * head_mark_cells(p.W[l]);
+  }
+  if (total > 0x7fffffffL - HM_WAVES) throw std::runtime_error("head_mark: too many cells");
+  const unsigned grid = (unsigned)((total + HM_WAVES - 1) / HM_WAVES);
+  hipLaunchKernelGGL((head_mark_kernel<20>), dim3(grid), dim3(HM_WAVES * 64), 0, s, p);
+}
+
+}
diff --git a/csrc/kernels/launch.h b/csrc/kernels/launch.h
--- a/csrc/kernels/launch.h
+++ b/csrc/kernels/launch.h
@@ -37,6 +37,9 @@
   const float* gate;
   int gate_n;
   float gate_min;
+  int n_lo, n_hi;
+  const int* marks;
+  int mark_uh, mark_uw, mark_halo;
   const uint8_t* lb_pool;
   const ImageMeta* lb_meta;
   const void* w3;
@@ -92,10 +95,23 @@
 constexpr int kF32X3HRPw = 161;
 constexpr int kF32X3HRPwVariants = 6;
 constexpr int kF32X3HP = 191;
-constexpr int kF32X3HPVariants = 9;
+constexpr int kF32X3HPVariants = 10;
 bool x3hp_supported(const ConvParams& p);
 bool conv_x3hp(const ConvParams& p, hipStream_t s, int v);
 void x3hp_prepare();
+int x3hg_pw_variant(int impl, int cout_pad);
+bool x3hg_pw_tile(int impl, int cout_pad, int* th, int* tw);
+struct HeadMarkParams {
+  int n_levels;
+  const float* logits[3];
+  int H[3], W[3], ps[3];
+  int* marks[3];
+  int n;
+  float gate_min;
+  int B;
+  const int* bdev;
+};
+void head_mark(const HeadMarkParams& p, hipStream_t s);
 bool conv_x3hr(const ConvParams& p, hipStream_t s, int v);
 bool conv_x3hr_pw(const ConvParams& p, hipStream_t s, int v);
 bool conv_fc_f32(const ConvParams& p, hipStream_t s);
diff --git a/csrc/runtime/executor.cpp b/csrc/runtime/executor.cpp
--- a/csrc/runtime/executor.cpp
+++ b/csrc/runtime/executor.cpp
@@ -37,10 +37,16 @@
   const char* e = std::getenv("ARENA_HEAD_GATE");
   return e == nullptr || std::atoi(e) != 0;
 }();
+int g_head_split = [] {
+  const char* e = std::getenv("ARENA_HEAD_SPLIT");
+  return e == nullptr ? 1 : std::max(0, std::min(2, std::atoi(e)));
+}();
 }
 
 void set_head_gate(bool v) { g_head_gate = v; }
 bool get_head_gate() { return g_head_gate; }
+void set_head_split(int v) { g_head_split = std::max(0, std::min(2, v)); }
+int get_head_split() { return g_head_split; }
 
 Executor::Executor(const ExecutorConfig& cfg) : cfg_(cfg) {
   if (cfg_.max_batch <= 0 || cfg_.max_batch > 1024) throw std::runtime_error("Executor: max_batch out of range");
@@ -277,6 +283,9 @@
   }
   if (has_raw_ && cfg_.raw_out_bytes <= 0) throw std::runtime_error("program exports raw outputs: raw_out_bytes = 0");
   gate_pairs_ = head_gate_pairs(prog_.empty() ? nullptr : prog_[0].data(), n_ops, kOpFields);
+  gate_first_.clear();
+  for (const HeadGatePair& gp : gate_pairs_)
+    gate_first_.push_back(head_gate_first_conv(prog_[0].data(), n_ops, kOpFields, gp));
 }
 
 int Executor::crop_cap_for(int B) const { return std::max(cfg_.min_crop_cap, B * cfg_.crop_cap_per_image); }
@@ -315,7 +324,20 @@
   bk.info.arena_bytes = arena_bytes;
   sync_slots();
   free_arenas(bk);
-  const size_t abytes = (size_t)std::max<int64_t>(arena_bytes, 256);
+  size_t abytes = align_up((size_t)std::max<int64_t>(arena_bytes, 256), 256);
+  bk.marks_off.assign(gate_pairs_.size(), -1);
+  for (size_t i = 0; i < gate_pairs_.size(); ++i) {
+    if (gate_first_[i] < 0) continue;
+    const OpRecord& f = prog_[gate_first_[i]];
+    const OpRecord& c = prog_[gate_pairs_[i].cls];
+    const int64_t cb = c[34] > 0 ? c[36] : c[10], cst = c[34] > 0 ? c[38] : c[12];
+    if (f[1] < 0 || f[1] >= n_buffers || cb < 0 || cb >= n_buffers) continue;
+    const int64_t in_lo = offsets[f[1]], in_hi = in_lo + (int64_t)B * f[4] * f[5] * f[3] * 4;
+    const int64_t w_lo = offsets[cb], w_hi = w_lo + (int64_t)B * c[13] * c[14] * cst * 4;
+    if (f[1] == cb || (in_lo < w_hi && w_lo < in_hi)) continue;
+    bk.marks_off[i] = (int64_t)abytes;
+    abytes += align_up((size_t)B * head_mark_cells((int)f[13]) * head_mark_cells((int)f[14]) * sizeof(int), 256);
+  }
   for (int s = 0; s < n_slots_; ++s) {
     ARENA_HIP_CHECK(hipMalloc(&bk.d_arena[s], abytes));
     ARENA_HIP_CHECK(hipMemset(bk.d_arena[s], 0, abytes));
@@ -474,6 +496,7 @@
   if (s == 0) {
     bk.exec_order.clear();
     bk.gated.clear();
+    bk.launches.clear();
   }
   auto capture_range = [&](size_t a, size_t b) {
     std::vector<OpRecord> part(prog_.begin() + a, prog_.begin() + b);
@@ -484,6 +507,7 @@
         bk.exec_order.push_back((int)(a + order[k]));
         if (gate[k] != nullptr) bk.gated.push_back((int)(a + order[k]));
       }
+      for (const Step& st : launch_plan(part, bk, (int)a, 0)) bk.launches.emplace_back((int)(a + st.pos), st.kind);
     }
     hipGraph_t g = nullptr;
     hipGraphExec_t ge = nullptr;
@@ -625,6 +649,37 @@
   return order;
 }
 
+std::vector<Executor::Step> Executor::launch_plan(const std::vector<OpRecord>& prog, const Bucket& bk, int op_offset,
+                                                  int force_impl) const {
+  std::vector<const HeadGatePair*> gate;
+  const std::vector<size_t> order = exec_plan(prog, bk, op_offset, force_impl, gate);
+  std::vector<Step> steps;
+  steps.reserve(order.size() + 6);
+  for (size_t k = 0; k < order.size(); ++k) steps.push_back(Step{order[k], LAUNCH_OP, gate[k]});
+  if (g_head_split == 0 || (g_head_split == 1 && bk.info.B < kHeadSplitMinBucket)) return steps;
+  for (size_t i = 0; i < gate_pairs_.size(); ++i) {
+    const HeadGatePair& gp = gate_pairs_[i];
+    const int fi = gate_first_[i];
+    const long lf = (long)fi - op_offset;
+    if (fi < 0 || lf < 0 || i >= bk.marks_off.size() || bk.marks_off[i] < 0) continue;
+    size_t k = 0;
+    while (k < steps.size() && !(steps[k].kind == LAUNCH_OP && steps[k].gate == &gp)) ++k;
+    if (k >= steps.size() || k < 2 || steps[k - 2].pos != (size_t)lf || steps[k - 2].kind != LAUNCH_OP) continue;
+    if (prog[lf] != prog_[fi] || prog_[fi][30] != BATCH_IMAGES) continue;
+    const int f_impl = fi < (int)bk.impl.size() ? bk.impl[fi] : 0;
+    if (!(f_impl >= kF32X3HP && f_impl < kF32X3HP + kF32X3HPVariants)) continue;
+    int uh = 0, uw = 0;
+    if (gp.box >= (int)bk.impl.size() || !x3hg_pw_tile(bk.impl[gp.box], (int)prog_[gp.box][16], &uh, &uw)) continue;
+    if (uh % kMarkCell != 0 || uw % kMarkCell != 0) continue;
+    const size_t box_pos = steps[k].pos;
+    steps[k - 2].kind = LAUNCH_CLS_WINDOW;
+    steps[k - 2].gate = &gp;
+    const Step extra[2] = {Step{box_pos, LAUNCH_MARK, &gp}, Step{(size_t)lf, LAUNCH_BOX_WINDOW, &gp}};
+    steps.insert(steps.begin() + (long)k, extra, extra + 2);
+  }
+  return steps;
+}
+
 void Executor::enqueue_program(const std::vector<OpRecord>& prog, Bucket& bk, Slot& sl, hipStream_t s_main,
                                int op_offset, int force_impl) {
   Ctrl* ctrl = (Ctrl*)resolve(bk, sl, BUF_CTRL, 0, 1);
@@ -635,12 +690,29 @@
   auto bdev = [&](int64_t kind) -> const int* { return kind == BATCH_CROPS ? &ctrl->n_crops : &ctrl->n_images; };
   const uint8_t* W = d_weights_;
 
-  std::vector<const HeadGatePair*> gate;
-  const std::vector<size_t> order = exec_plan(prog, bk, op_offset, force_impl, gate);
-  for (size_t k = 0; k < prog.size(); ++k) {
-    const size_t oi = order[k];
+  const std::vector<Step> steps = launch_plan(prog, bk, op_offset, force_impl);
+  auto marks_of = [&](const HeadGatePair* gp) {
+    return (int*)(bk.d_arena[sl.idx] + bk.marks_off[(size_t)(gp - gate_pairs_.data())]);
+  };
+  for (const Step& step : steps) {
+    const size_t oi = step.pos;
     const OpRecord& r = prog[oi];
     hipStream_t s = s_main;
+    if (step.kind == LAUNCH_MARK) {
+      HeadMarkParams m{};
+      m.n_levels = 1;
+      m.logits[0] = (const float*)resolve(bk, sl, r[36], r[37] + kHeadBoxChannels, 4);
+      m.H[0] = (int)r[13];
+      m.W[0] = (int)r[14];
+      m.ps[0] = (int)r[38];
+      m.marks[0] = marks_of(step.gate);
+      m.n = kHeadClsChannels;
+      head_gate_min(step.gate->conf_thr, &m.gate_min);
+      m.B = batch(r[30]);
+      m.bdev = bdev(r[30]);
+      head_mark(m, s);
+      continue;
+    }
     const bool f32 = r[kDtypeField] == 1;
     const int eb = f32 ? 4 : 2;
     switch (r[0]) {
@@ -698,11 +770,24 @@
           p.pw_ys = (int)r[38];
           p.pw_act = (int)r[39];
           if (!f32) p.impl = 2;
-          if (gate[k] != nullptr) {
+          if (step.gate != nullptr) {
             p.gate = (const float*)resolve(bk, sl, r[36], r[37] + kHeadBoxChannels, eb);
             p.gate_n = kHeadClsChannels;
-            head_gate_min(gate[k]->conf_thr, &p.gate_min);
+            head_gate_min(step.gate->conf_thr, &p.gate_min);
           }
+        }
+        if (step.kind == LAUNCH_CLS_WINDOW || step.kind == LAUNCH_BOX_WINDOW) {
+          const bool box = step.kind == LAUNCH_BOX_WINDOW;
+          p.n_lo = box ? 0 : kHeadBoxChannels;
+          p.n_hi = box ? kHeadBoxChannels : kHeadBoxChannels + kHeadClsChannels;
+          if (box) {
+            p.marks = marks_of(step.gate);
+            p.mark_halo = 1;
+            x3hg_pw_tile(bk.impl[step.gate->box], (int)prog_[step.gate->box][16], &p.mark_uh, &p.mark_uw);
+          }
+          if (!conv_x3hp(p, s, box ? kHeadSplitBoxVariant : kHeadSplitClsVariant))
+            throw std::runtime_error("executor: the split first head conv does not fit its x3hp window kernel");
+          break;
         }
         if (f32)
           conv2d_f32(p, s);
diff --git a/csrc/runtime/executor.h b/csrc/runtime/executor.h
--- a/csrc/runtime/executor.h
+++ b/csrc/runtime/executor.h
@@ -14,6 +14,7 @@
 
 #include "../kernels/launch.h"
 #include "head_gate.h"
+#include "head_marks.h"
 #include "instance.h"
 
 namespace arena {
@@ -29,6 +30,11 @@
 
 void set_head_gate(bool v);
 bool get_head_gate();
+void set_head_split(int v);
+int get_head_split();
+constexpr int kHeadSplitMinBucket = 32;
+constexpr int kHeadSplitBoxVariant = 2, kHeadSplitClsVariant = 9;
+enum LaunchKind : int { LAUNCH_OP = 0, LAUNCH_CLS_WINDOW = 1, LAUNCH_BOX_WINDOW = 2, LAUNCH_MARK = 3 };
 
 enum OpType : int64_t {
   OP_CONV = 1,
@@ -175,6 +181,13 @@
     std::vector<Seg> segs[kMaxSlots];
     std::vector<int16_t> impl;
     std::vector<int> exec_order, gated;
+    std::vector<std::pair<int, int>> launches;
+    std::vector<int64_t> marks_off;
+  };
+  struct Step {
+    size_t pos;
+    int kind;
+    const HeadGatePair* gate;
   };
 
   void alloc_slots();
@@ -195,6 +208,8 @@
   void autotune(Bucket& bk);
   std::vector<size_t> exec_plan(const std::vector<OpRecord>& prog, const Bucket& bk, int op_offset, int force_impl,
                                 std::vector<const HeadGatePair*>& gate) const;
+  std::vector<Step> launch_plan(const std::vector<OpRecord>& prog, const Bucket& bk, int op_offset,
+                                int force_impl) const;
 
  public:
   std::vector<int> exec_order(int B) const {
@@ -204,6 +219,10 @@
   std::vector<int> gated_ops(int B) const {
     auto it = buckets_.find(B);
     return it == buckets_.end() ? std::vector<int>{} : it->second.gated;
+  }
+  std::vector<std::pair<int, int>> launch_order(int B) const {
+    auto it = buckets_.find(B);
+    return it == buckets_.end() ? std::vector<std::pair<int, int>>{} : it->second.launches;
   }
   std::vector<int> conv_choices(int B) const {
     auto it = buckets_.find(B);
@@ -235,6 +254,7 @@
   size_t weights_bytes_ = 0;
   std::vector<OpRecord> prog_, cls_prog_;
   std::vector<HeadGatePair> gate_pairs_;
+  std::vector<int> gate_first_;
   std::map<int, Bucket> buckets_;
   Slot slots_[kMaxSlots];
   int n_slots_ = 2;
diff --git a/csrc/runtime/head_gate.h b/csrc/runtime/head_gate.h
--- a/csrc/runtime/head_gate.h
+++ b/csrc/runtime/head_gate.h
@@ -68,4 +68,29 @@
   return out;
 }
 
+constexpr int64_t kHgOpYoloRaw = 13;
+inline int head_gate_first_conv(const int64_t* ops, int n, int fields, const HeadGatePair& gp) {
+  if (ops == nullptr || fields <= kHgDtypeField || gp.box < 1 || gp.cls != gp.box + 1 || gp.cls >= n) return -1;
+  auto rec = [&](int i) { return ops + (size_t)i * fields; };
+  const int fi = gp.box - 1;
+  const int64_t *f = rec(fi), *a = rec(gp.box), *c = rec(gp.cls);
+  constexpr int kN = kHeadBoxChannels + kHeadClsChannels;
+  if (!(f[0] == kHgOpConv && f[kHgDtypeField] == 1 && f[17] == 3 && f[18] == 3 && f[19] == 1 && f[15] == kN &&
+        f[34] == 0 && f[22] < 0 && f[25] < 0 && f[10] >= 0))
+    return -1;
+  if (!(f[13] == a[4] && f[14] == a[5] && f[13] == a[13] && f[14] == a[14] && f[30] == a[30])) return -1;
+  if (!(a[1] == f[10] && a[2] == f[11] && a[6] == kHeadBoxChannels && a[3] == f[12])) return -1;
+  if (!(c[1] == f[10] && c[2] == f[11] + kHeadBoxChannels && c[6] == kHeadClsChannels && c[3] == f[12])) return -1;
+  const int64_t buf = f[10];
+  for (int i = 0; i < n; ++i) {
+    if (i == fi || i == gp.box || i == gp.cls) continue;
+    const int64_t* r = rec(i);
+    bool reads = r[1] == buf;
+    if (r[0] == kHgOpConv) reads |= r[22] == buf;
+    if (r[0] == kHgOpDecode || r[0] == kHgOpYoloRaw) reads |= r[5] == buf || r[9] == buf;
+    if (reads) return -1;
+  }
+  return fi;
 }
+
+}
diff --git a/csrc/runtime/head_marks.h b/csrc/runtime/head_marks.h
--- /dev/null
+++ b/csrc/runtime/head_marks.h
@@ -0,0 +1,41 @@
+#pragma once
+
+#if defined(__HIPCC__) || defined(__HIP__)
+#define ARENA_MARKS_HD __host__ __device__
+#else
+#define ARENA_MARKS_HD
+#endif
+
+namespace arena {
+
+constexpr int kMarkCell = 8;
+constexpr int kMarkMaxLevels = 3;
+
+ARENA_MARKS_HD inline int head_mark_cells(int extent) { return (extent + kMarkCell - 1) / kMarkCell; }
+
+ARENA_MARKS_HD inline bool head_marks_continues(const int* m, int H, int W, int uy, int ux, int uh, int uw) {
+  const int y0 = uy * uh, x0 = ux * uw;
+  const int y1 = (y0 + uh < H ? y0 + uh : H) - 1, x1 = (x0 + uw < W ? x0 + uw : W) - 1;
+  const int ncx = head_mark_cells(W);
+  for (int cy = y0 / kMarkCell; cy <= y1 / kMarkCell; ++cy)
+    for (int cx = x0 / kMarkCell; cx <= x1 / kMarkCell; ++cx)
+      if (m[cy * ncx + cx] != 0) return true;
+  return false;
+}
+
+ARENA_MARKS_HD inline bool head_marks_needed(const int* m, int H, int W, int ty, int tx, int th, int tw, int uh,
+                                             int uw, int halo) {
+  const int ty0 = ty * th, tx0 = tx * tw;
+  const int ty1 = ty0 + th < H ? ty0 + th : H, tx1 = tx0 + tw < W ? tx0 + tw : W;
+  const int nuy = (H + uh - 1) / uh, nux = (W + uw - 1) / uw;
+  const int uy_lo = ty0 > halo ? (ty0 - halo) / uh : 0, ux_lo = tx0 > halo ? (tx0 - halo) / uw : 0;
+  int uy_hi = (ty1 + halo - 1) / uh, ux_hi = (tx1 + halo - 1) / uw;
+  if (uy_hi > nuy - 1) uy_hi = nuy - 1;
+  if (ux_hi > nux - 1) ux_hi = nux - 1;
+  for (int uy = uy_lo; uy <= uy_hi; ++uy)
+    for (int ux = ux_lo; ux <= ux_hi; ++ux)
+      if (head_marks_continues(m, H, W, uy, ux, uh, uw)) return true;
+  return false;
+}
+
+}
diff --git a/inference_arena_amd/engine/plans.py b/inference_arena_amd/engine/plans.py
--- a/inference_arena_amd/engine/plans.py
+++ b/inference_arena_amd/engine/plans.py
@@ -189,6 +189,8 @@
                     pw=(*fold_conv_bn(d.cv2[lvl][2], None), View(D, 0, 4 * d.reg_max), None))
             pb.conv(View(H1, c2, c3), View(BUF_NONE, 0, c3), *fold(d.cv3[lvl][1]),
                     pw=(*fold_conv_bn(d.cv3[lvl][2], None), View(D, 4 * d.reg_max, nc), None))
+            if pb.f32:
+                P.last = max(P.last, len(pb.ops) - 1)
         else:
             pb.conv(View(H1, 0, c2), View(H2, 0, c2), *fold(d.cv2[lvl][1]))
             pb.conv(View(H1, c2, c3), View(H2, c2, c3), *fold(d.cv3[lvl][1]))
diff --git a/inference_arena_amd/ops/functional.py b/inference_arena_amd/ops/functional.py
--- a/inference_arena_amd/ops/functional.py
+++ b/inference_arena_amd/ops/functional.py
@@ -37,7 +37,7 @@
                 res: torch.Tensor | None = None, res_coff: int = 0, out2: torch.Tensor | None = None,
                 out2_coff: int = 0, f32out: bool = False, out_hw=None, bdev: torch.Tensor | None = None,
                 packed=None, impl: int = 0, pw=None, pw_out: torch.Tensor | None = None, pw_out_coff: int = 0,
-                gate=None) -> torch.Tensor:
+                gate=None, window=None, marks=None) -> torch.Tensor:
     f32 = x.dtype == torch.float32
     B, H, W, Cx = x.shape
     cout, cin_w, kh, kw = w.shape
@@ -86,6 +86,14 @@
             pwd.update({"gate": _ptr(gt, gcoff), "gate_n": int(gn), "gate_min": float(gmin)})
     elif gate is not None or pw_out is not None:
         raise ValueError("conv2d_nhwc: gate / pw_out need pw")
+    if window is not None:
+        pwd.update({"n_lo": int(window[0]), "n_hi": int(window[1])})
+    if marks is not None:
+        mt, uh, uw, halo = marks
+        if (mt.dtype != torch.int32 or mt.device != x.device or not mt.is_contiguous()
+                or tuple(mt.shape) != (B, (Ho + 7) // 8, (Wo + 7) // 8)):
+            raise ValueError("conv2d_nhwc: marks must be contiguous int32 [B, ceil(Ho / 8), ceil(Wo / 8)]")
+        pwd.update({"marks": _ptr(mt), "mark_uh": int(uh), "mark_uw": int(uw), "mark_halo": int(halo)})
     skd = {}
     if 171 <= int(impl) < 180:
         ws = torch.empty(8 * B * Ho * Wo * cpad, dtype=torch.float32, device=x.device)
@@ -103,6 +111,27 @@
     if pw is not None:
         torch.cuda.synchronize(x.device)
     return out
+
+
+def head_mark(logits: torch.Tensor, coff: int, n: int, gate_min: float, marks: torch.Tensor | None = None,
+              bdev: torch.Tensor | None = None, levels=None) -> torch.Tensor | list:
+    lv = [(logits, marks)] + list(levels or [])
+    out = []
+    for lg, mk in lv:
+        B, H, W, C = lg.shape
+        if lg.dtype != torch.float32 or not lg.is_contiguous() or coff < 0 or coff + n > C:
+            raise ValueError("head_mark: logits must be contiguous float32 [B, H, W, >= coff + n]")
+        if mk is None:
+            mk = torch.zeros(B, (H + 7) // 8, (W + 7) // 8, dtype=torch.int32, device=lg.device)
+        if (mk.dtype != torch.int32 or mk.device != lg.device or not mk.is_contiguous()
+                or tuple(mk.shape) != (B, (H + 7) // 8, (W + 7) // 8) or B != lv[0][0].shape[0]):
+            raise ValueError("head_mark: marks must be contiguous int32 [B, ceil(H / 8), ceil(W / 8)]")
+        out.append(mk)
+    native().head_mark({"logits": [_ptr(lg, coff) for lg, _ in lv], "marks": [_ptr(mk) for mk in out],
+                        "H": [lg.shape[1] for lg, _ in lv], "W": [lg.shape[2] for lg, _ in lv],
+                        "ps": [lg.shape[3] for lg, _ in lv], "n": int(n), "gate_min": float(gate_min),
+                        "B": lv[0][0].shape[0], "bdev": _ptr(bdev), "stream": _stream()})
+    return out if levels else out[0]
 
 
 def dwconv3x3_nhwc(x: torch.Tensor, w: torch.Tensor, b: torch.Tensor, *, stride: int = 1, act="relu6",
diff --git a/inference_arena_amd/utils/settings.py b/inference_arena_amd/utils/settings.py
--- a/inference_arena_amd/utils/settings.py
+++ b/inference_arena_amd/utils/settings.py
@@ -54,6 +54,7 @@
     ARENA_INFER_SERVICE: int = 0
     ARENA_IR_S2K16: int = 1
     ARENA_HEAD_GATE: int = 1
+    ARENA_HEAD_SPLIT: int = 1
 
     @classmethod
     def from_env(cls, env_file: str | Path = ".env", **overrides) -> "Settings":
```

New measurement: 11120, median of 6. 1.01x the previous value.
